# moabarar/nemar

Hardware: AMD Instinct MI355X
Metric: train images/sec (256x256 A/B pairs) (higher is better)
Workload: dtype f32

## Files before the change

### include/nemar_hip.h

```cpp
#ifndef NEMAR_HIP_H
#define NEMAR_HIP_H
#include <stddef.h>

#ifdef __cplusplus
extern "C" {
#endif

#define NEMAR_OK 0
#define NEMAR_EINVAL (-1)
#define NEMAR_ELAUNCH (-2)
#define NEMAR_EWORKSPACE (-3)

int nemar_version(void);
const char* nemar_last_error(void);

#define NEMAR_GRID_EXPLICIT 0
#define NEMAR_GRID_UNET 1
#define NEMAR_GRID_AFFINE 2
int nemar_grid_sample_fwd(const float* in, const float* grid_src, int grid_mode, float* out,
                          int N, int C, int H, int W, int Ho, int Wo, void* stream);
size_t nemar_grid_sample_bwd_workspace(int N, int C, int H, int W);
size_t nemar_grid_sample_bwd_zeroed_bytes(int N, int C, int H, int W);
int nemar_grid_sample_bwd(const float* in, const float* grid_src, int grid_mode, const float* gout,
                          float* gin, int accum_gin, float* ggrid, int accum_ggrid,
                          int N, int C, int H, int W, int Ho, int Wo, void* workspace, size_t ws_bytes, void* stream);

size_t nemar_smoothness_workspace(int N, int H, int W);
int nemar_smoothness_fwd(const float* d, const float* img, int Ci, float alpha, float factor,
                         float* loss, int accumulate, void* workspace, size_t ws_bytes,
                         int N, int H, int W, void* stream);
int nemar_smoothness_bwd(const float* d, const float* img, int Ci, float alpha, const float* gscale,
                         float factor, float* gd, int accumulate, int N, int H, int W, void* stream);

#define NEMAR_PAD_ZERO 0
#define NEMAR_PAD_REFLECT 1
#define NEMAR_ACT_NONE 0
#define NEMAR_ACT_RELU 1
#define NEMAR_ACT_LRELU 2
#define NEMAR_ACT_TANH 3
size_t nemar_conv2d_fwd_workspace(int N, int H, int W, int K, int C, int R, int S, int stride, int pad);
int nemar_conv2d_fwd(const float* x0, int C0, const float* x1, int C1, const float* w, const float* bias,
                     float* y, int N, int H, int W, int K, int R, int S, int stride, int pad, int pad_mode,
                     int act, float slope, void* workspace, size_t ws_bytes, int prepacked, void* stream);
size_t nemar_conv2d_bwd_data_workspace(int N, int C, int H, int W, int K, int R, int S, int stride, int pad,
                                       int pad_mode);
int nemar_conv2d_bwd_data(const float* gy, const float* w, const float* bias, int act, float slope,
                          float* gx0, int C0, float* gx1, int C1, int N, int H, int W, int K, int OH, int OW,
                          int R, int S, int stride, int pad, int pad_mode, void* workspace, size_t ws_bytes,
                          int prepacked, void* stream);
size_t nemar_conv2d_bwd_weight_workspace(int N, int C, int H, int W, int K, int OH, int OW, int R, int S, int stride,
                                         int pad);
int nemar_conv2d_bwd_weight(const float* x0, int C0, const float* x1, int C1, const float* gy, float* gw, float* gb,
                            int N, int H, int W, int K, int OH, int OW, int R, int S, int stride, int pad,
                            int pad_mode, void* workspace, size_t ws_bytes, void* stream);
typedef struct nemar_conv_extras {
    void* scratch;
    size_t scratch_bytes;
    const void* src_max_words;
    int src_max_count;
    const void* src2_max_words;
    int src2_max_count;
    const void* src_planes;
    void* gy_planes_out;
    size_t gy_planes_bytes;
    const void* src2_planes;
    const float* addend;
    void* out_max_words;
    const float* bias_partials;
} nemar_conv_extras;
int nemar_conv2d_bwd_data_fusable(int N, int C, int H, int W, int K, int R, int S, int stride, int pad, int pad_mode);
int nemar_conv2d_bwd_data_addend_ok(int N, int C, int H, int W, int K, int R, int S, int stride, int pad, int pad_mode);
size_t nemar_conv2d_x_planes_bytes(int N, int C, int H, int W, int KS);
size_t nemar_conv2d_gy_planes_bytes(int N, int C, int H, int W, int K, int R, int S, int stride, int pad, int pad_mode);
int nemar_last_gy_planes(void);
int nemar_conv2d_fwd_ex(const float* x0, int C0, const float* x1, int C1, const float* w, const float* bias, float* y, int N,
                        int H, int W, int K, int R, int S, int stride, int pad, int pad_mode, int act, float slope,
                        void* workspace, size_t ws_bytes, int prepacked, void* stream, const nemar_conv_extras* extras);
int nemar_conv2d_bwd_data_ex(const float* gy, const float* w, const float* bias, int act, float slope, float* gx0, int C0,
                             float* gx1, int C1, int N, int H, int W, int K, int OH, int OW, int R, int S, int stride, int pad,
                             int pad_mode, void* workspace, size_t ws_bytes, int prepacked, void* stream,
                             const nemar_conv_extras* extras);
int nemar_conv2d_bwd_weight_ex(const float* x0, int C0, const float* x1, int C1, const float* gy, float* gw, float* gb, int N,
                               int H, int W, int K, int OH, int OW, int R, int S, int stride, int pad, int pad_mode,
                               void* workspace, size_t ws_bytes, void* stream, const nemar_conv_extras* extras);
int nemar_pack_plan_record(int plan);
int nemar_pack_plan_jobs(int plan);
size_t nemar_pack_plan_bytes(int plan);
int nemar_pack_plan_dirty(int plan);
int nemar_pack_plan_commit(int plan, void* device_buffer, size_t bytes, void* stream);
int nemar_pack_plan_run(int plan, void* stream);
int nemar_pack_plan_reset(int plan);
int nemar_last_route(void);
int nemar_config_epoch(void);
int nemar_set_max_words_lazy(int on);
int nemar_max_words_finalize(void* max_words, int samples, void* stream);
size_t nemar_conv2d_scratch(int N, int H, int W, int K, int C, int R, int S, int stride, int pad);
int nemar_absmax(const float* t, long long n, void* out_word, void* stream);
int nemar_absmax_samples(const float* t, int samples, long long per_sample, void* out_words, void* stream);
int nemar_kernel_timer(int enable);
int nemar_kernel_timer_read(double* total_ms, double* total_flop, int* launches);
size_t nemar_bias_grad_workspace(int N, int C, int HW);
int nemar_bias_grad(const float* g, float* gb, int N, int C, int HW, void* workspace, size_t ws_bytes, void* stream);

int nemar_instnorm_fwd(const float* x, const float* residual, float* y, float* stats, int planes, int HW,
                       float eps, int act, float slope, void* stream);
int nemar_instnorm_bwd(const float* x, const float* stats, const float* gy, float* gx, int planes, int HW,
                       int act, float slope, void* stream);
#define NEMAR_MAX_PARTIALS 2048
#define NEMAR_MAX_WORDS(samples) ((size_t)(samples) * (1 + NEMAR_MAX_PARTIALS))
int nemar_instnorm_fwd_max(const float* x, const float* residual, float* y, float* stats, int planes, int HW,
                           float eps, int act, float slope, void* max_words, int planes_per_sample, void* stream);
int nemar_instnorm_bwd_max(const float* x, const float* stats, const float* gy, float* gx, int planes, int HW,
                           int act, float slope, void* max_words, int planes_per_sample, void* stream);

int nemar_instnorm_fwd_planes(const float* x, const float* residual, const void* residual_max_words, float* y, float* stats,
                              int N, int C, int H, int W, float eps, int act, float slope, float dropout_p,
                              unsigned long long seed, unsigned offset, void* planes, void* scale_words, void* max_words,
                              void* wgrad_planes, void* stream);
int nemar_instnorm_bwd_planes(const float* x, const float* stats, const float* gy, const void* gy_max_words, int N, int C,
                              int H, int W, int act, float slope, float dropout_p, unsigned long long seed, unsigned offset,
                              int pad_mode, float* gx, void* dgrad_planes, void* wgrad_planes, void* scale_words,
                              float* bias_partials, void* stream);
int nemar_bias_from_partials(const float* bias_partials, int N, int C, float* gb, void* stream);
size_t nemar_batchnorm_workspace(int N, int C, int HW, int segments);
int nemar_batchnorm_fwd_train(const float* x, const float* residual, float* y, const float* weight, const float* bias,
                              float* running_mean, float* running_var, long long* num_batches_tracked, float* saved,
                              int N, int C, int HW, int segments, float eps, float momentum, int act, float slope,
                              float dropout_p, unsigned long long seed, unsigned offset, void* max_words,
                              void* workspace, size_t workspace_bytes, void* stream);
int nemar_batchnorm_fwd_eval(const float* x, const float* residual, float* y, const float* weight, const float* bias,
                             const float* running_mean, const float* running_var, float* saved, int N, int C, int HW, float eps,
                             int act, float slope, float dropout_p, unsigned long long seed, unsigned offset, void* max_words,
                             void* stream);
int nemar_batchnorm_bwd(const float* x, const float* gy, float* gx, const float* weight, const float* bias, const float* saved,
                        float* grad_weight, float* grad_bias, int N, int C, int HW, int segments, int training, int act,
                        float slope, float dropout_p, unsigned long long seed, unsigned offset, void* workspace,
                        size_t workspace_bytes, void* stream);

int nemar_act_bwd(const float* gy, const float* y, float* gx, long long n, int act, float slope, void* stream);
int nemar_act_fwd(const float* x, float* y, long long n, int act, float slope, void* stream);
int nemar_concat_pieces(const float* const* pieces, const long long* counts, int k, float* dst, void* stream);
int nemar_add2(const float* a, const float* b, float* out, long long n, void* stream);
int nemar_maxpool2_fwd(const float* x, float* y, int planes, int H, int W, void* stream);
int nemar_maxpool2_bwd(const float* x, const float* gy, const float* addend, float* gx, int planes, int H, int W,
                       void* stream);
int nemar_bilinear_fwd(const float* x, float* y, int planes, int H, int W, int Ho, int Wo, void* stream);
int nemar_bilinear_bwd(const float* gy, float* gx, int planes, int H, int W, int Ho, int Wo, void* stream);
int nemar_dropout(const float* x, float* y, long long n, float p, unsigned long long seed, unsigned offset,
                  void* stream);
int nemar_dropout_max(const float* x, float* y, int samples, long long per_sample, float p, unsigned long long seed,
                      unsigned offset, void* max_words, void* stream);

int nemar_set_dropout_base(const void* device_word);
int nemar_store_words(void* dst, const void* host_words, int n, void* stream);
int nemar_adam_step_dev(float* p, const float* g, float* m, float* v, long long n, const float* hyper, double beta1,
                        double beta2, double eps, void* stream);

int nemar_crop_flip_normalize(const float* pool, const int* params, float* y, int M, int B, int C, int H, int W,
                              int Hc, int Wc, float scale, void* stream);

int nemar_deform_field(const float* params, float* g, int B, int Hc, int Wc, int gh, int gw, void* stream);
int nemar_crop_flip_deform_normalize(const float* pool, const int* params, const float* g, float* y, int M, int B, int C,
                                     int H, int W, int Hc, int Wc, float scale, void* stream);
size_t nemar_registration_error_workspace(int N, int H, int W);
int nemar_registration_error(const float* pred, int grid_mode, const float* g, float* out, void* workspace, size_t ws_bytes,
                             int N, int H, int W, void* stream);

#define NEMAR_SAMPLE_BILINEAR 0
#define NEMAR_SAMPLE_NEAREST 1
int nemar_warp_resampled_fwd(const float* in, const float* pred, int grid_mode, int sample_mode, float* out,
                             int N, int C, int Hs, int Ws, int hf, int wf, int Ho, int Wo, void* stream);

int nemar_label_overlap(const float* labels_moving, const float* labels_fixed, const float* pred, int grid_mode, unsigned* counts,
                        int N, int K, int Hs, int Ws, int hf, int wf, int Ho, int Wo, void* stream);
int nemar_map_points(const float* pts, const float* pred, int grid_mode, float* out, int N, int P, int Hs, int Ws, int hf, int wf,
                     int Ho, int Wo, void* stream);

int nemar_compose_pred(const float* first, int first_mode, int h1, int w1, const float* second, int second_mode, int h2, int w2,
                       float* out_field, const float* img, float* out_img, int C, int N, int H, int W, void* stream);

#define NEMAR_GAN_VANILLA 0
#define NEMAR_GAN_LSGAN 1
#define NEMAR_GAN_WGANGP 2
size_t nemar_loss_workspace(void);
int nemar_l1_loss_fwd(const float* a, const float* b, long long n, float weight, float* loss, int accumulate,
                      void* workspace, size_t ws_bytes, void* stream);
int nemar_l1_loss_bwd(const float* a, const float* b, long long n, const float* gscale, float weight, float* ga,
                      int accumulate, void* stream);
int nemar_gan_loss_fwd(const float* x, long long n, int mode, int target_is_real, float weight, float* loss,
                       int accumulate, void* workspace, size_t ws_bytes, void* stream);
int nemar_gan_loss_bwd(const float* x, long long n, int mode, int target_is_real, const float* gscale,
                       float weight, float* gx, void* stream);

int nemar_adam_step(float* p, const float* g, float* m, float* v, long long n, double lr, double beta1,
                    double beta2, double eps, int step, void* stream);

#ifdef __cplusplus
}
#endif
#endif
```

### nemar_amd/_lib.py

```python
import ctypes as C
import os

import torch

_HERE = os.path.dirname(os.path.abspath(__file__))
PRODUCT_PATH = os.path.join(_HERE, "lib", "libnemar_hip.so")
AB_PATH = os.path.join(_HERE, "lib", "libnemar_hip_ab.so")
DEFAULT_PATH = AB_PATH if (os.environ.get("NEMAR_AB_LIBRARY") == "1" or os.environ.get("NEMAR_TUNE")) else PRODUCT_PATH

_f = C.POINTER(C.c_float)
_vp = C.c_void_p
_i = C.c_int
_fl = C.c_float
_sz = C.c_size_t
_ll = C.c_longlong
_db = C.c_double
_u64 = C.c_ulonglong
_u32 = C.c_uint

SIGNATURES = {
    "nemar_version": (_i, []),
    "nemar_last_error": (C.c_char_p, []),
    "nemar_grid_sample_fwd": (_i, [_vp, _vp, _i, _vp, _i, _i, _i, _i, _i, _i, _vp]),
    "nemar_grid_sample_bwd_workspace": (_sz, [_i, _i, _i, _i]),
    "nemar_grid_sample_bwd_zeroed_bytes": (_sz, [_i, _i, _i, _i]),
    "nemar_grid_sample_bwd": (_i, [_vp, _vp, _i, _vp, _vp, _i, _vp, _i, _i, _i, _i, _i, _i, _i, _vp, _sz, _vp]),
    "nemar_smoothness_workspace": (_sz, [_i, _i, _i]),
    "nemar_smoothness_fwd": (_i, [_vp, _vp, _i, _fl, _fl, _vp, _i, _vp, _sz, _i, _i, _i, _vp]),
    "nemar_smoothness_bwd": (_i, [_vp, _vp, _i, _fl, _vp, _fl, _vp, _i, _i, _i, _i, _vp]),
    "nemar_conv2d_fwd_workspace": (_sz, [_i] * 9),
    "nemar_conv2d_fwd": (_i, [_vp, _i, _vp, _i, _vp, _vp, _vp, _i, _i, _i, _i, _i, _i, _i, _i, _i, _i, _fl, _vp, _sz, _i, _vp]),
    "nemar_conv2d_bwd_data_workspace": (_sz, [_i] * 10),
    "nemar_conv2d_bwd_data": (_i, [_vp, _vp, _vp, _i, _fl, _vp, _i, _vp, _i, _i, _i, _i, _i, _i, _i, _i, _i, _i, _i,
                                   _i, _vp, _sz, _i, _vp]),
    "nemar_conv2d_bwd_weight_workspace": (_sz, [_i] * 11),
    "nemar_conv2d_bwd_weight": (_i, [_vp, _i, _vp, _i, _vp, _vp, _vp, _i, _i, _i, _i, _i, _i, _i, _i, _i, _i, _i, _vp, _sz,
                                     _vp]),
    "nemar_conv2d_scratch": (_sz, [_i] * 9),
    "nemar_conv2d_gy_planes_bytes": (_sz, [_i] * 10),
    "nemar_absmax": (_i, [_vp, _ll, _vp, _vp]),
    "nemar_absmax_samples": (_i, [_vp, _i, _ll, _vp, _vp]),
    "nemar_kernel_timer": (_i, [_i]),
    "nemar_kernel_timer_read": (_i, [C.POINTER(C.c_double), C.POINTER(C.c_double), C.POINTER(_i)]),
    "nemar_bias_grad_workspace": (_sz, [_i, _i, _i]),
    "nemar_bias_grad": (_i, [_vp, _vp, _i, _i, _i, _vp, _sz, _vp]),
    "nemar_last_route": (_i, []),
    "nemar_last_gy_planes": (_i, []),
    "nemar_config_epoch": (_i, []),
    "nemar_set_max_words_lazy": (_i, [_i]),
    "nemar_instnorm_fwd": (_i, [_vp, _vp, _vp, _vp, _i, _i, _fl, _i, _fl, _vp]),
    "nemar_instnorm_bwd": (_i, [_vp, _vp, _vp, _vp, _i, _i, _i, _fl, _vp]),
    "nemar_instnorm_fwd_max": (_i, [_vp, _vp, _vp, _vp, _i, _i, _fl, _i, _fl, _vp, _i, _vp]),
    "nemar_instnorm_fwd_planes": (_i, [_vp, _vp, _vp, _vp, _vp, _i, _i, _i, _i, _fl, _i, _fl, _fl, _u64, _u32, _vp, _vp, _vp, _vp, _vp]),
    "nemar_instnorm_bwd_planes": (_i, [_vp, _vp, _vp, _vp, _i, _i, _i, _i, _i, _fl, _fl, _u64, _u32, _i, _vp, _vp, _vp, _vp, _vp, _vp]),
    "nemar_bias_from_partials": (_i, [_vp, _i, _i, _vp, _vp]),
    "nemar_conv2d_bwd_data_fusable": (_i, [_i] * 10),
    "nemar_conv2d_x_planes_bytes": (_sz, [_i] * 5),
    "nemar_set_dropout_base": (_i, [_vp]),
    "nemar_store_words": (_i, [_vp, _vp, _i, _vp]),
    "nemar_pack_plan_record": (_i, [_i]),
    "nemar_pack_plan_jobs": (_i, [_i]),
    "nemar_pack_plan_bytes": (_sz, [_i]),
    "nemar_pack_plan_dirty": (_i, [_i]),
    "nemar_pack_plan_commit": (_i, [_i, _vp, _sz, _vp]),
    "nemar_pack_plan_run": (_i, [_i, _vp]),
    "nemar_pack_plan_reset": (_i, [_i]),
    "nemar_adam_step_dev": (_i, [_vp, _vp, _vp, _vp, _ll, _vp, C.c_double, C.c_double, C.c_double, _vp]),
    "nemar_conv2d_fwd_ex": (_i, [_vp, _i, _vp, _i, _vp, _vp, _vp, _i, _i, _i, _i, _i, _i, _i, _i, _i, _i, _fl, _vp, _sz, _i, _vp, _vp]),
    "nemar_conv2d_bwd_data_ex": (_i, [_vp, _vp, _vp, _i, _fl, _vp, _i, _vp, _i, _i, _i, _i, _i, _i, _i, _i, _i, _i, _i, _i, _vp, _sz, _i, _vp, _vp]),
    "nemar_conv2d_bwd_weight_ex": (_i, [_vp, _i, _vp, _i, _vp, _vp, _vp, _i, _i, _i, _i, _i, _i, _i, _i, _i, _i, _i, _vp, _sz, _vp, _vp]),
    "nemar_instnorm_bwd_max": (_i, [_vp, _vp, _vp, _vp, _i, _i, _i, _fl, _vp, _i, _vp]),
    "nemar_act_bwd": (_i, [_vp, _vp, _vp, _ll, _i, _fl, _vp]),
    "nemar_act_fwd": (_i, [_vp, _vp, _ll, _i, _fl, _vp]),
    "nemar_conv2d_bwd_data_addend_ok": (_i, [_i] * 10),
    "nemar_max_words_finalize": (_i, [_vp, _i, _vp]),
    "nemar_concat_pieces": (_i, [_vp, _vp, _i, _vp, _vp]),
    "nemar_add2": (_i, [_vp, _vp, _vp, _ll, _vp]),
    "nemar_maxpool2_fwd": (_i, [_vp, _vp, _i, _i, _i, _vp]),
    "nemar_maxpool2_bwd": (_i, [_vp, _vp, _vp, _vp, _i, _i, _i, _vp]),
    "nemar_bilinear_fwd": (_i, [_vp, _vp, _i, _i, _i, _i, _i, _vp]),
    "nemar_bilinear_bwd": (_i, [_vp, _vp, _i, _i, _i, _i, _i, _vp]),
    "nemar_crop_flip_normalize": (_i, [_vp, _vp, _vp, _i, _i, _i, _i, _i, _i, _i, _fl, _vp]),
    "nemar_deform_field": (_i, [_vp, _vp, _i, _i, _i, _i, _i, _vp]),
    "nemar_crop_flip_deform_normalize": (_i, [_vp, _vp, _vp, _vp, _i, _i, _i, _i, _i, _i, _i, _fl, _vp]),
    "nemar_registration_error_workspace": (_sz, [_i, _i, _i]),
    "nemar_registration_error": (_i, [_vp, _i, _vp, _vp, _vp, _sz, _i, _i, _i, _vp]),
    "nemar_warp_resampled_fwd": (_i, [_vp, _vp, _i, _i, _vp, _i, _i, _i, _i, _i, _i, _i, _i, _vp]),
    "nemar_label_overlap": (_i, [_vp, _vp, _vp, _i, _vp, _i, _i, _i, _i, _i, _i, _i, _i, _vp]),
    "nemar_map_points": (_i, [_vp, _vp, _i, _vp, _i, _i, _i, _i, _i, _i, _i, _i, _vp]),
    "nemar_compose_pred": (_i, [_vp, _i, _i, _i, _vp, _i, _i, _i, _vp, _vp, _vp, _i, _i, _i, _i, _vp]),
    "nemar_dropout": (_i, [_vp, _vp, _ll, _fl, _u64, _u32, _vp]),
    "nemar_dropout_max": (_i, [_vp, _vp, _i, _ll, _fl, _u64, _u32, _vp, _vp]),
    "nemar_loss_workspace": (_sz, []),
    "nemar_l1_loss_fwd": (_i, [_vp, _vp, _ll, _fl, _vp, _i, _vp, _sz, _vp]),
    "nemar_l1_loss_bwd": (_i, [_vp, _vp, _ll, _vp, _fl, _vp, _i, _vp]),
    "nemar_gan_loss_fwd": (_i, [_vp, _ll, _i, _i, _fl, _vp, _i, _vp, _sz, _vp]),
    "nemar_gan_loss_bwd": (_i, [_vp, _ll, _i, _i, _vp, _fl, _vp, _vp]),
    "nemar_adam_step": (_i, [_vp, _vp, _vp, _vp, _ll, _db, _db, _db, _db, _i, _vp]),
    "nemar_batchnorm_workspace": (_sz, [_i, _i, _i, _i]),
    "nemar_batchnorm_fwd_train": (_i, [_vp, _vp, _vp, _vp, _vp, _vp, _vp, _vp, _vp, _i, _i, _i, _i, _fl, _fl, _i, _fl, _fl, _u64, _u32,
                                       _vp, _vp, _sz, _vp]),
    "nemar_batchnorm_fwd_eval": (_i, [_vp, _vp, _vp, _vp, _vp, _vp, _vp, _vp, _i, _i, _i, _fl, _i, _fl, _fl, _u64, _u32, _vp, _vp]),
    "nemar_batchnorm_bwd": (_i, [_vp, _vp, _vp, _vp, _vp, _vp, _vp, _vp, _i, _i, _i, _i, _i, _i, _fl, _fl, _u64, _u32, _vp, _sz, _vp]),
}


AB_SIGNATURES = {
    "nemar_tune": (_i, [_i, _i]),
    "nemar_grid_sample_tune": (_i, [_i]),
    "nemar_tune_ptr": (_i, [_vp]),
}


class NemarHipError(RuntimeError):
    pass


class ConvExtras(C.Structure):
    _fields_ = [("scratch", C.c_void_p), ("scratch_bytes", C.c_size_t), ("src_max_words", C.c_void_p), ("src_max_count", C.c_int),
                ("src2_max_words", C.c_void_p), ("src2_max_count", C.c_int), ("src_planes", C.c_void_p),
                ("gy_planes_out", C.c_void_p), ("gy_planes_bytes", C.c_size_t), ("src2_planes", C.c_void_p),
                ("addend", C.c_void_p), ("out_max_words", C.c_void_p), ("bias_partials", C.c_void_p)]


class Library:

    def __init__(self, path):
        if not os.path.exists(path):
            raise NemarHipError(
                "gfx950 operator library not found at %s — build it with `python -m nemar_amd.csrc.build` "
                "(there is no CPU/PyTorch fallback for the NeMAR hot path)" % path)
        self.path = path
        self._dll = C.CDLL(path)
        self._fns = {}
        for name, (res, args) in SIGNATURES.items():
            try:
                fn = getattr(self._dll, name)
            except AttributeError as e:
                raise NemarHipError("%s does not export %s" % (path, name)) from e
            fn.restype = res
            fn.argtypes = args
            self._fns[name] = fn
        self.has_switches = all(hasattr(self._dll, name) for name in AB_SIGNATURES)
        if self.has_switches:
            for name, (res, args) in AB_SIGNATURES.items():
                fn = getattr(self._dll, name)
                fn.restype = res
                fn.argtypes = args
                self._fns[name] = fn

    def raw(self, name):
        return self._fns[name]

    def last_error(self):
        return self._fns["nemar_last_error"]().decode("utf-8", "replace")

    def __getattr__(self, name):
        fns = self.__dict__.get("_fns", {})
        full = name if name.startswith("nemar_") else "nemar_" + name
        if full not in fns:
            if full in AB_SIGNATURES:
                raise NemarHipError("%s has no %s: the measurement switches exist only in the -DNEMAR_AB build "
                                    "(libnemar_hip_ab.so; set NEMAR_AB_LIBRARY=1 before nemar_amd is imported)" % (self.__dict__.get("path"), full))
            raise AttributeError(name)
        fn = fns[full]
        if {**SIGNATURES, **AB_SIGNATURES}[full][0] is not _i or full in ("nemar_version", "nemar_last_route", "nemar_last_gy_planes", "nemar_config_epoch", "nemar_set_max_words_lazy", "nemar_pack_plan_jobs", "nemar_pack_plan_dirty", "nemar_conv2d_bwd_data_fusable", "nemar_conv2d_bwd_data_addend_ok"):
            return fn

        if os.environ.get("NEMAR_DEBUG_SYNC"):
            def checked(*a):
                import sys
                sys.stderr.write("[nemar] %s %s\n" % (full, [x for x in a if isinstance(x, (int, float))]))
                sys.stderr.flush()
                rc = fn(*a)
                torch.cuda.synchronize()
                if rc != 0:
                    raise NemarHipError("%s failed (%d): %s" % (full, rc, self.last_error()))
                return rc
            checked.__name__ = full
            self.__dict__[name] = checked
            return checked

        def checked(*a):
            rc = fn(*a)
            if rc != 0:
                raise NemarHipError("%s failed (%d): %s" % (full, rc, self.last_error()))
            return rc

        checked.__name__ = full
        self.__dict__[name] = checked
        return checked


_default = None


def load(path=None):
    global _default
    if path is not None:
        return Library(path)
    if _default is None:
        _default = Library(DEFAULT_PATH)
        for kv in os.environ.get("NEMAR_TUNE", "").split(","):
            if "=" in kv:
                k, v = kv.split("=")
                _default.tune(int(k), int(v))
    return _default
```

### nemar_amd/csrc/common.h

```cpp
#pragma once
#include <hip/hip_runtime.h>
#include <stdint.h>
#include <stdio.h>

#define NEMAR_OK 0
#define NEMAR_EINVAL (-1)
#define NEMAR_ELAUNCH (-2)
#define NEMAR_EWORKSPACE (-3)

#define NEMAR_API extern "C" __attribute__((visibility("default")))

#ifdef NEMAR_AB
#define NEMAR_SWITCH(type, name, def) type name = def
#define NEMAR_AB_ONLY(...) __VA_ARGS__
#else
#define NEMAR_SWITCH(type, name, def) __attribute__((unused)) constexpr type name = def
#define NEMAR_AB_ONLY(...)
#endif

size_t nemar_lds_bytes(const void* kernel, size_t need, bool claim);
#define NEMAR_LDS_CLAIM_DEFAULT 1
#ifdef NEMAR_AB
extern int g_lds_claim;
#else
constexpr int g_lds_claim = NEMAR_LDS_CLAIM_DEFAULT;
#endif

struct nemar_conv_extras {
    void* scratch;
    size_t scratch_bytes;
    const void* src_max_words;
    int src_max_count;
    const void* src2_max_words;
    int src2_max_count;
    const void* src_planes;
    void* gy_planes_out;
    size_t gy_planes_bytes;
    const void* src2_planes;
    const float* addend;
    void* out_max_words;
    const float* bias_partials;
};

void nemar_set_error(const char* fmt, ...);

#define NEMAR_REQUIRE(cond, ...)                 \
    do {                                         \
        if (!(cond)) {                           \
            nemar_set_error(__VA_ARGS__);        \
            return NEMAR_EINVAL;                 \
        }                                        \
    } while (0)

#define NEMAR_CLEAR_HIP_ERROR() ((void)hipGetLastError())

#define NEMAR_CHECK_LAUNCH(what)                                              \
    do {                                                                      \
        hipError_t e__ = hipGetLastError();                                   \
        if (e__ != hipSuccess) {                                              \
            nemar_set_error("%s: %s", what, hipGetErrorString(e__));          \
            return NEMAR_ELAUNCH;                                             \
        }                                                                     \
    } while (0)

#define NEMAR_HIP_CALL(expr)                                                 \
    do {                                                                      \
        hipError_t e__ = (expr);                                              \
        if (e__ != hipSuccess) {                                              \
            nemar_set_error("%s: %s", #expr, hipGetErrorString(e__));         \
            return NEMAR_ELAUNCH;                                             \
        }                                                                     \
    } while (0)

static inline int nemar_cdiv(long long a, long long b) { return (int)((a + b - 1) / b); }

static inline int nemar_stream_grid(long long work_items, int per_block) {
    long long b = (work_items + per_block - 1) / per_block;
    if (b < 1) b = 1;
    if (b > 256 * 8) b = 256 * 8;
    return (int)b;
}

struct FastDiv {
    unsigned d;
    unsigned long long m;
};
static inline FastDiv make_fastdiv(unsigned d) {
    FastDiv f;
    f.d = d ? d : 1;
    f.m = ((1ull << 40) + f.d - 1) / f.d;
    return f;
}
__device__ __forceinline__ unsigned fd_div(unsigned n, const FastDiv& f) {
    return (unsigned)(((unsigned long long)n * f.m) >> 40);
}

__device__ __forceinline__ void glds_b128(const float* g, float* lds) {
    __builtin_amdgcn_global_load_lds((const __attribute__((address_space(1))) void*)g,
                                     (__attribute__((address_space(3))) void*)lds, 16, 0, 0);
}
__device__ __forceinline__ void glds_b32(const float* g, float* lds) {
    __builtin_amdgcn_global_load_lds((const __attribute__((address_space(1))) void*)g,
                                     (__attribute__((address_space(3))) void*)lds, 4, 0, 0);
}
__device__ __forceinline__ void wait_vmem() { __builtin_amdgcn_s_waitcnt(0x0F70); }

__device__ __forceinline__ float uniform_f(float v) {
#ifdef NEMAR_HOST_EMULATION
    return v;
#else
    return __builtin_bit_cast(float, __builtin_amdgcn_readfirstlane(__builtin_bit_cast(int, v)));
#endif
}

__device__ __forceinline__ float wave_sum(float v) {
#pragma unroll
    for (int o = 32; o > 0; o >>= 1) v += __shfl_xor(v, o, 64);
    return v;
}
__device__ __forceinline__ float wave_max(float v) {
#pragma unroll
    for (int o = 32; o > 0; o >>= 1) v = fmaxf(v, __shfl_xor(v, o, 64));
    return v;
}
// ... 12 lines not shown
```

### nemar_amd/csrc/conv.hip

```cpp
#define NEMAR_CONV_HIP
#include "common.h"
#include "conv_exact.h"
#include "conv_call.h"
#include "conv_route.h"
#include "pack_plan.h"

#ifdef NEMAR_AB
extern int g_split16_ring3;
extern int g_split16_ksplit_cap;
extern int g_narrow_fwd4;
extern int g_wg_xreg;
extern int g_register_vec4;
extern int g_overlap_per_lane;
void nemar_norm_planes_debug(int bits);
#endif

int nemar_narrow_fwd(const float* x, const float* w, const float* bias, float* y, int N, int C, int H, int W, int K, int R,
                     int pad, int border, int act, float slope, float* part, size_t part_floats, hipStream_t st);
int nemar_narrow_wgrad(const float* x, const float* gy, float* gw, int N, int C, int H, int W, int K, int R, int pad,
                       int border, float* part, hipStream_t st);
void nemar_wgrad2_launch(const float* x0, int C0, const float* x1, int C1, const float* gy, float* gw, float* gb, int N,
                         int H, int W, int K, int OH, int OW, int R, int S, int stride, int pad, int pad_mode,
                         int target_blocks, bool vec_ok, int dbg, float* part, hipStream_t st);
void nemar_sum_partials_pair(const float* part_a, long long stride_a, int splits_a, float* dst_a, long long n_a,
// ... 414 lines not shown
            v = at(y, x);
        } else {
            const int y0 = y + 3, x0 = x + 3;
            const int y1 = (y >= 1 && y <= 3) ? 3 - y : -1, y2 = (y <= H - 2 && y >= H - 4) ? 2 * (H - 1) - y + 3 : -1;
            const int x1 = (x >= 1 && x <= 3) ? 3 - x : -1, x2 = (x <= W - 2 && x >= W - 4) ? 2 * (W - 1) - x + 3 : -1;
            auto row = [&](int Y) {
                float s = at(Y, x0);
                if (x1 >= 0) s += at(Y, x1);
                if (x2 >= 0) s += at(Y, x2);
                return s;
            };
            v = row(y0);
            if (y1 >= 0) v += row(y1);
            if (y2 >= 0) v += row(y2);
        }
        if (bias) v += bias[k];
        out[idx] = apply_act(v, act, slope);
    }
}

void k7_mf_run(const K7MfPlan& m_, const float* src, const float* w, int Ks, int Cb, int dgrad, const float* bias, float* out, int N, int H, int W,
               int fold, int act, float slope, float* wsf, int prepacked, hipStream_t st) {
    K7MfPlan m = m_;
    float* wt = wsf + m.wt_off;
    void* packed = wsf + m.pack_off;
    float* P = wsf + m.p_off;
    if (!prepacked) {
        K7MfWtArgs a{w, wt, Ks, Cb, dgrad, nemar_stream_grid(32 * Cb * 7, 256), 1};
        if (nemar_pack_recording()) nemar_pack_record_job(PACK_FAM_PRE, &a, a.gx, 1);
        hipLaunchKernelGGL(k7_mf_weights_kernel, dim3(a.gx), dim3(256), 0, st, w, wt, Ks, Cb, dgrad);
        nemar_s16g_pack(m.q, m.pl, wt, (long long)Cb * 7, 7, packed, st);
    }
    m.q.src0 = src; m.q.src1 = nullptr; m.q.dst0 = P; m.q.dst1 = nullptr; m.q.bias = nullptr; m.q.dbg = 0; m.q.tl = nullptr;
    nemar_s16g_conv(m.q, m.pl, packed, st);
    const long long total = (long long)N * Ks * H * W;
    hipLaunchKernelGGL(k7_mf_sum_kernel, dim3(nemar_stream_grid(total, 256)), dim3(256), 0, st, (const float*)P, bias, out, Ks, H, W, m.PH, m.PW, fold,
                       act, slope, total);
}

__global__ __launch_bounds__(256) void pad_planes_kernel(const float* __restrict__ src, float* __restrict__ dst, int plane,
                                                         int plane_padded, long long total) {
    for (long long idx = (long long)blockIdx.x * blockDim.x + threadIdx.x; idx < total;
         idx += (long long)gridDim.x * blockDim.x) {
        const long long pl = idx / plane_padded;
        const int r = (int)(idx - pl * plane_padded);
        dst[idx] = r < plane ? src[pl * plane + r] : 0.f;
    }
}

}

static ConvFacts facts_of(const ConvCall& call, const float* bias, int act, float slope) {
    ConvFacts f;
    f.bias = bias != nullptr; f.act = act; f.slope = slope; f.scratch_bytes = call.scratch ? call.scratch_bytes : 0;
    return f;
}

NEMAR_API size_t nemar_conv2d_fwd_workspace(int N, int H, int W, int K, int C, int R, int S, int stride, int pad) {
    if (N <= 0 || H <= 0 || W <= 0 || K <= 0 || C <= 0 || R <= 0 || S <= 0 || stride < 1) return 0;
    return sizeof(float) * plan_fwd({N, C, 0, H, W, K, R, S, stride, pad, BORDER_ZERO}, ConvFacts::canonical()).total;
}

static int conv2d_fwd(ConvCall& call, const float* x0, int C0, const float* x1, int C1, const float* w, const float* bias,
                      float* y, int N, int H, int W, int K, int R, int S, int stride, int pad, int pad_mode,
                      int act, float slope, void* workspace, size_t ws_bytes, int prepacked, void* stream) {
    NEMAR_CLEAR_HIP_ERROR();
    NEMAR_REQUIRE(x0 && w && y && workspace, "conv2d_fwd: null pointer");
    NEMAR_REQUIRE(C0 > 0 && C1 >= 0 && (C1 == 0 || x1), "conv2d_fwd: bad channel split %d+%d", C0, C1);
    NEMAR_REQUIRE(N > 0 && H > 0 && W > 0 && K > 0 && R > 0 && S > 0 && R * S <= MAX_TAPS, "conv2d_fwd: bad shape");
    NEMAR_REQUIRE(stride >= 1 && pad >= 0 && pad < 32768, "conv2d_fwd: bad stride/pad");
    NEMAR_REQUIRE(pad_mode == BORDER_ZERO || (pad_mode == BORDER_REFLECT && pad < H && pad < W),
                  "conv2d_fwd: reflect pad %d needs pad < H,W (%d,%d)", pad, H, W);
    const int C = C0 + C1;
    const int OH = (H + 2 * pad - R) / stride + 1, OW = (W + 2 * pad - S) / stride + 1;
    NEMAR_REQUIRE(OH > 0 && OW > 0, "conv2d_fwd: empty output");
    NEMAR_REQUIRE((long long)N * OH * OW < (1ll << 31) && (long long)C * H * W < (1ll << 31) && (long long)C * R * S < (1 << 20),
                  "conv2d_fwd: problem too large for 32-bit tile indexing");
    ConvFacts f = facts_of(call, bias, act, slope);
    FwdPlan P = plan_fwd({N, C0, C1, H, W, K, R, S, stride, pad, pad_mode}, f);
    if (ws_bytes < sizeof(float) * P.total) {
        nemar_set_error("conv2d_fwd: workspace %zu < %zu", ws_bytes, sizeof(float) * P.total);
        return NEMAR_EWORKSPACE;
    }
    hipStream_t st = (hipStream_t)stream;
    const char* what = "conv2d_fwd";
    g_last_route = P.route;
    switch (P.route) {
    case ROUTE_K7:
        if (P.sub == FwdPlan::K7_MANY_FEW) {
            k7_mf_run(P.k7, x0, w, K, C, 0, bias, y, N, H, W, 0, act, slope, (float*)workspace, prepacked, st);
            what = "conv2d_fwd (7x7 many -> few, 16-bit pipe)";
        } else {
            if (!prepacked) nemar_k7_fm_pack(w, (long long)C * 49, 49, 0, K, C, workspace, st);
            nemar_k7_fm_conv(x0, C, H, W, 3, pad_mode == BORDER_REFLECT, workspace, bias, y, K, N, H, W, act, slope, 0, st);
            what = "conv2d_fwd (7x7, 16-bit pipe)";
        }
        break;
    case ROUTE_NARROW:
        nemar_narrow_fwd(x0, w, bias, y, N, C, H, W, K, R, pad, pad_mode, act, slope,
                         g_deterministic ? (float*)workspace : nullptr, ws_bytes / sizeof(float), st);
        what = "conv2d_fwd (narrow)";
        break;
    case ROUTE_SPLIT16: {
        const int mode = pad_mode == BORDER_REFLECT ? SPLIT16_REFLECT : SPLIT16_ZERO;
        if (!prepacked) nemar_split16_pack(w, workspace, K, C, R, 0, g_split16_variant, st);
        nemar_split16_conv(x0, workspace, bias, y, N, H, W, K, C, R, 1, H, W, OH, OW, mode, call.scratch, g_xcd_map, g_split16_variant,
                           g_tl, nullptr, call.src_max, call.src_planes, call.src_planes_kind, nullptr, nullptr, st);
        what = "conv2d_fwd (split-16)";
        break;
    }
    case ROUTE_S16G: {
        S16gProblem& q = P.q;
        q.src0 = x0; q.src1 = x1; q.dst0 = y; q.dst1 = nullptr; q.bias = bias; q.dbg = g_dbg; q.tl = g_tl;
        if (!prepacked) nemar_s16g_pack(q, P.pl, w, (long long)C * R * S, (long long)R * S, workspace, st);
        nemar_s16g_conv(q, P.pl, workspace, st);
        what = "conv2d_fwd (16-bit pipe, in-kernel split)";
        break;
    }
    default: {
        IgemmParams p;
        fwd_taps(p.taps, R, S, pad);
        if (!prepacked) launch_pack(w, (float*)workspace, K, C, C * R * S, R * S, p.taps, st);
        p.src0 = x0; p.src1 = x1; p.C0 = C0; p.C1 = C1; p.Hs = H; p.Ws = W;
        p.wp = (const float*)workspace; p.M = K; p.Mpad = igemm_mpad(K); p.Kred = C * R * S;
        p.zero = p.wp + packed_core_floats(K, C * R * S);
        p.dbg = g_dbg; p.tl = g_tl;
        p.ring_p = 0; p.ring_H = 0; p.ring_W = 0; p.ksplit = 1; p.part = nullptr; p.part_stride = 0;
        p.rf = 0; p.rf_row = nullptr; p.rf_col = nullptr; p.xcd = 0;
        p.bias = bias;
        p.dst0 = y; p.dst1 = nullptr; p.M0 = K;
        p.OH = OH; p.OW = OW; p.OHf = OH; p.OWf = OW; p.osy = 1; p.ooy = 0; p.osx = 1; p.oox = 0;
        p.N = N; p.P = N * OH * OW;
        p.sy = stride; p.sx = stride; p.border = pad_mode; p.act = act; p.slope = slope; p.pad = pad;
        p.fd_ohw = make_fastdiv(OH * OW); p.fd_ow = make_fastdiv(OW); p.fd_cs = make_fastdiv(C);
        if (P.sub != FwdPlan::PLAIN) {
            p.ksplit = P.ksplit;
            p.part = (float*)workspace + P.slab_off;
            p.part_stride = (long long)N * K * OH * OW;
            p.act = ACT_NONE;
        }
        launch_igemm(p, st);
        if (P.sub == FwdPlan::SPLIT_ACT) nemar_sum_partials_act(p.part, p.part_stride, p.ksplit, y, p.part_stride, act == ACT_RELU ? 1 : 2, slope, st);
        else if (P.sub == FwdPlan::SPLIT) nemar_sum_partials(p.part, p.part_stride, p.ksplit, y, p.part_stride, false, st);
    }
    }
    NEMAR_CHECK_LAUNCH(what);
    return NEMAR_OK;
}

NEMAR_API size_t nemar_conv2d_bwd_data_workspace(int N, int C, int H, int W, int K, int R, int S, int stride, int pad, int pad_mode) {
    if (N <= 0 || C <= 0 || K <= 0 || R <= 0 || S <= 0 || stride < 1) return 0;
    return sizeof(float) * plan_dgrad({N, C, 0, H, W, K, R, S, stride, pad, pad_mode}, ConvFacts::canonical()).total;
}

static int conv2d_bwd_data(ConvCall& call, const float* gy, const float* w, const float* bias, int act, float slope,
                           float* gx0, int C0, float* gx1, int C1, int N, int H, int W, int K, int OH, int OW,
                           int R, int S, int stride, int pad, int pad_mode, void* workspace, size_t ws_bytes,
                           int prepacked, void* stream) {
    NEMAR_CLEAR_HIP_ERROR();
    NEMAR_REQUIRE(gy && w && workspace && (gx0 || gx1), "conv2d_bwd_data: null pointer");
    NEMAR_REQUIRE(C0 >= 0 && C1 >= 0 && C0 + C1 > 0 && (C1 == 0 || gx1), "conv2d_bwd_data: bad channel split");
    NEMAR_REQUIRE(N > 0 && H > 0 && W > 0 && K > 0 && OH > 0 && OW > 0 && R * S <= MAX_TAPS && R > 0 && S > 0,
                  "conv2d_bwd_data: bad shape");
    NEMAR_REQUIRE(stride >= 1 && stride <= 4 && pad >= 0, "conv2d_bwd_data: bad stride/pad");
    NEMAR_REQUIRE((H + 2 * pad - R) / stride + 1 == OH && (W + 2 * pad - S) / stride + 1 == OW,
                  "conv2d_bwd_data: gy %dx%d inconsistent with x %dx%d k%d s%d p%d", OH, OW, H, W, R, stride, pad);
    const int C = C0 + C1;
    const bool refl = pad_mode == BORDER_REFLECT && pad > 0;
    NEMAR_REQUIRE(pad_mode != BORDER_REFLECT || (pad < H && pad < W), "conv2d_bwd_data: reflect pad too large");
    NEMAR_REQUIRE(!refl || (!bias && act == ACT_NONE && gx1 == nullptr),
                  "conv2d_bwd_data: reflect mode supports a single destination without bias/activation");
    NEMAR_REQUIRE(!refl || stride > 1 || pad <= 4, "conv2d_bwd_data: reflect pad %d > 4 unsupported", pad);
    ConvFacts f = facts_of(call, bias, act, slope);
    f.gx0 = gx0 != nullptr; f.gx1 = gx1 != nullptr;
    f.gy_planes_bytes = call.gy_planes_out ? call.gy_planes_bytes : 0;
    DgradPlan L = plan_dgrad({N, C0, C1, H, W, K, R, S, stride, pad, pad_mode}, f);
    if (ws_bytes < sizeof(float) * L.total) {
        nemar_set_error("conv2d_bwd_data: workspace %zu < %zu", ws_bytes, sizeof(float) * L.total);
        return NEMAR_EWORKSPACE;
    }
    NEMAR_REQUIRE((long long)N * (H + 2 * pad) * (W + 2 * pad) < (1ll << 31) && (long long)K * OH * OW < (1ll << 31) && (long long)K * R * S < (1 << 20),
                  "conv2d_bwd_data: problem too large for 32-bit tile indexing");
    hipStream_t st = (hipStream_t)stream;
    float* wsf = (float*)workspace;
    const long long total = (long long)N * C * H * W;
    const int mskip = L.mskip;
    const char* what = "conv2d_bwd_data";
    g_last_route = L.route;
    switch (L.sub) {
    case DgradPlan::K7_MANY_FEW:
        k7_mf_run(L.k7, gy, w, C, K, 1, nullptr, gx0, N, H, W, L.k7_fold, ACT_NONE, 0.f, wsf, prepacked, st);
        what = "conv2d_bwd_data (7x7 many -> few, 16-bit pipe)";
        break;
    case DgradPlan::K7_FEW_MANY:
        if (!prepacked) nemar_k7_fm_pack(w, 49, (long long)C * 49, 1, C, K, workspace, st);
        if (L.k7_fold == 2) {
            float* padded = wsf + ((nemar_k7_fm_pack_floats(C) + 3) & ~(size_t)3);
            nemar_k7_fm_conv(gy, K, OH, OW, 6, 0, workspace, nullptr, padded, C, N, H + 6, W + 6, ACT_NONE, 0.f, 0, st);
            fold_padded(padded, gx0, H, W, pad, total, nullptr, st);
        } else {
            nemar_k7_fm_conv(gy, K, OH, OW, L.k7_fold ? 6 : 3, 0, workspace, nullptr, gx0, C, N, H, W, ACT_NONE, 0.f, L.k7_fold, st);
        }
        what = "conv2d_bwd_data (7x7, 16-bit pipe)";
        break;
    case DgradPlan::SPLIT16: {
        if (!prepacked) nemar_split16_pack(w, workspace, K, C, R, 1, g_split16_variant, st);
        const Split16Done done = nemar_split16_conv(gy, workspace, nullptr, gx0, N, H, W, C, K, R, R - 1 - pad, OH, OW, H, W,
                                                    refl ? SPLIT16_DGRAD_REFLECT : SPLIT16_ZERO, call.scratch, g_xcd_map, g_split16_variant, g_tl,
                                                    L.want_gy_planes ? call.gy_planes_out : nullptr, call.src_max, call.src_planes,
                                                    call.src_planes_kind, call.addend, call.out_max, st);
        call.gy_planes_written = done.dual_written;
        call.epilogue_fused = done.epilogue_fused;
        what = "conv2d_bwd_data (split-16)";
        break;
    }
    case DgradPlan::S16G:
    case DgradPlan::S16G_FOLD: {
        const bool fold16 = L.sub == DgradPlan::S16G_FOLD;
        S16gProblem& q = L.q;
        q.src0 = gy; q.src1 = nullptr; q.bias = bias ? bias + mskip : nullptr;
        if (fold16) { q.dst0 = wsf + L.padded_off; q.dst1 = nullptr; q.M0 = q.M; }
        else if (mskip) { q.dst0 = gx1; q.dst1 = nullptr; q.M0 = q.M; }
        else { q.dst0 = gx0; q.dst1 = gx1; q.M0 = C0; }
        if (!prepacked) nemar_s16g_pack(q, L.pl, w + (size_t)mskip * R * S, (long long)R * S, (long long)C * R * S, workspace, st);
        nemar_s16g_conv(q, L.pl, workspace, st);
        if (fold16) fold_padded(q.dst0, gx0, H, W, pad, total, call.addend, st);
        if (fold16 && call.addend) call.addend_done = true;
        what = fold16 ? "conv2d_bwd_data (16-bit pipe on the padded domain + fold)" : "conv2d_bwd_data (16-bit pipe, in-kernel split)";
        break;
    }
    case DgradPlan::EXACT: {
    const bool ring = L.ring, fold = L.fold;
    bool folded = false;
    const int Hd = fold ? H + 2 * pad : H, Wd = fold ? W + 2 * pad : W;
    const int padd = fold ? 0 : pad;
    float* padded = fold ? wsf + L.padded_off : nullptr;
    int cls = 0;
    for (int ph = 0; ph < stride; ++ph)
        for (int pw = 0; pw < stride; ++pw, ++cls) {
            IgemmParams p;
            dgrad_taps(p.taps, R, S, padd, stride, ph, pw);
            const int OHc = (Hd - ph + stride - 1) / stride, OWc = (Wd - pw + stride - 1) / stride;
            if (OHc <= 0 || OWc <= 0) continue;
            const int Mc = C - mskip;
            p.src0 = gy; p.src1 = nullptr; p.C0 = K; p.C1 = 0; p.Hs = OH; p.Ws = OW;
            p.M = Mc; p.Mpad = igemm_mpad(Mc); p.Kred = p.taps.n * K;
            p.bias = bias ? bias + mskip : nullptr;
            if (fold) { p.dst0 = padded; p.dst1 = nullptr; p.M0 = Mc; }
            else if (mskip) { p.dst0 = gx1; p.dst1 = nullptr; p.M0 = Mc; }
            else { p.dst0 = gx0; p.dst1 = gx1; p.M0 = C0; }
            p.OH = OHc; p.OW = OWc; p.OHf = Hd; p.OWf = Wd; p.osy = stride; p.ooy = ph; p.osx = stride; p.oox = pw;
            p.N = N; p.P = N * OHc * OWc;
            p.sy = 1; p.sx = 1; p.border = BORDER_ZERO; p.act = act; p.slope = slope;
            p.pad = pad;
            p.ring_p = 0; p.ring_H = 0; p.ring_W = 0; p.ksplit = 1; p.part = nullptr; p.part_stride = 0;
            p.rf = 0; p.rf_row = nullptr; p.rf_col = nullptr; p.xcd = 0;
            p.fd_ohw = make_fastdiv(OHc * OWc); p.fd_ow = make_fastdiv(OWc); p.fd_cs = make_fastdiv(K);
            float* wp = wsf + L.pack_stride * (size_t)cls;
            p.wp = wp;
            p.zero = wp + packed_core_floats(Mc, K * (p.taps.n > 0 ? p.taps.n : 1));
            p.dbg = g_dbg; p.tl = nullptr;
            if (p.taps.n == 0) {
                p.taps.n = 1; p.taps.dy[0] = -32000; p.taps.dx[0] = -32000; p.taps.wofs[0] = 0; p.Kred = K;
                p.taps.dyx[0] = (int)(((unsigned)-32000 << 16) | ((unsigned)-32000 & 0xffffu));
            }
            if (!prepacked) launch_pack(w + (size_t)mskip * R * S, wp, Mc, K, R * S, C * R * S, p.taps, st);
            bool ring_done = false;
            if (L.narrow) {
                float* w2 = wsf + L.w2_off;
                if (!prepacked) {
                    if (nemar_pack_recording()) {
                        FlipTArgs a{w, w2, K, C, R, S, nemar_stream_grid((long long)K * C * R * S, 256), 1};
                        nemar_pack_record_job(PACK_FAM_FLIPT, &a, a.gx, 1);
                    }
                    hipLaunchKernelGGL(flip_transpose_kernel, dim3(nemar_stream_grid((long long)K * C * R * S, 256)),
                                       dim3(256), 0, st, w, w2, K, C, R, S);
                }
                nemar_narrow_fwd(gy, w2, nullptr, gx0, N, K, OH, OW, C, R, R - 1 - pad, BORDER_ZERO, ACT_NONE, 0.f, nullptr, 0, st);
            } else {
                if (L.split) {
                    p.ksplit = L.ksplit;
                    p.part = wsf + L.slab_off;
                    p.part_stride = (long long)N * C * Hd * Wd;
                    if (gx1) { p.M0 = C; p.dst1 = nullptr; }
                }
                bool vec = false;
                if (L.aux_rows && route_ws2(p, &vec) && vec) {
                    float* rows = wsf + L.aux_rows_off, * cols = wsf + L.aux_cols_off;
                    hipLaunchKernelGGL(reflect_aux_kernel, dim3(nemar_stream_grid(6ll * N * K * W + 8ll * N * K * H, 256)),
                                       dim3(256), 0, st, gy, rows, cols, N, K, H, W);
                    p.rf = 1; p.rf_row = rows; p.rf_col = cols;
                    ring_done = true;
                }
// ... 124 lines not shown
        p.dbg = g_dbg;
        p.pix_per_split = P.pix_per_split;
        p.part = part;
        p.partb = part ? part + P.bias_off : nullptr;
        const bool wide = K > 32;
        dim3 grid(nemar_cdiv(K, wide ? 128 : 32), nemar_cdiv(J, wide ? 128 : 256), P.splits), block(256);
        if (wide) hipLaunchKernelGGL((wgrad_kernel<2, 2, 2, 2>), grid, block, 0, st, p);
        else hipLaunchKernelGGL((wgrad_kernel<1, 4, 1, 2>), grid, block, 0, st, p);
        if (part) nemar_sum_partials_pair(part, (long long)K * J, P.splits, gw, (long long)K * J, gb ? p.partb : nullptr, K, P.splits, gb, K, true, st);
    }
    }
    NEMAR_CHECK_LAUNCH(what);
    return NEMAR_OK;
}

NEMAR_API int nemar_last_route(void) { return g_last_route; }
NEMAR_API int nemar_config_epoch(void) { return g_config_epoch; }

#ifdef NEMAR_AB
NEMAR_API int nemar_tune_ptr(void* p) { g_tl = (long long*)p; return NEMAR_OK; }

NEMAR_API int nemar_tune(int key, int value) {
    ++g_config_epoch;
    if (key == 0) { g_cfg128 = value; return NEMAR_OK; }
    if (key == 1) { g_lds_pad = value; return NEMAR_OK; }
    if (key == 2) { g_dbg = value; return NEMAR_OK; }
    if (key == 3) { g_narrow = value; return NEMAR_OK; }
    if (key == 4) { g_wgrad = value; return NEMAR_OK; }
    if (key == 6) { g_min_blocks = value > 0 ? value : 384; return NEMAR_OK; }
    if (key == 14) { g_deterministic = value != 0; return NEMAR_OK; }
    if (key == 8) { g_reflect_aux = value != 0; return NEMAR_OK; }
    if (key == 15) { g_xcd_map = value != 0; return NEMAR_OK; }
    if (key == 20) { g_split16 = value != 0; return NEMAR_OK; }
    if (key == 24) { g_s16g = value != 0; return NEMAR_OK; }
    if (key == 25) { g_s16g_min_mmac = value < 0 ? 0 : value; return NEMAR_OK; }
    if (key == 26) { g_s16g_wgrad_first = value != 0; return NEMAR_OK; }
    if (key == 27) { nemar_s16g_tune(0, value); return NEMAR_OK; }
    if (key == 29) { g_s16g_wgrad = value != 0; return NEMAR_OK; }
    if (key == 31) { nemar_norm_planes_debug(value); return NEMAR_OK; }
    if (key == 32) { g_split16_ring3 = value != 0; return NEMAR_OK; }
    if (key == 33) { g_k7 = value != 0; return NEMAR_OK; }
    if (key == 36) { g_split_act = value != 0; return NEMAR_OK; }
    if (key == 43) { g_fold_small = value != 0; return NEMAR_OK; }
    if (key == 37) { g_lds_claim = value; return NEMAR_OK; }
    if (key == 38) { g_wg_xreg = value != 0; return NEMAR_OK; }
    if (key == 39) { g_split16_ksplit_cap = value < 1 ? 1 : (value > 8 ? 8 : value); return NEMAR_OK; }
    if (key == 45) { g_overlap_per_lane = value != 0; return NEMAR_OK; }
    if (key == 44) { g_register_vec4 = value != 0; return NEMAR_OK; }
    if (key == 35) { g_dual_gy = value != 0; return NEMAR_OK; }
    if (key == 34) { nemar_split16_wgrad_tune(value); return NEMAR_OK; }
    if (key == 30) { g_s16g_fold = value != 0; return NEMAR_OK; }
    if (key == 28) { nemar_s16g_tune(1, value); return NEMAR_OK; }
    if (key == 40) { nemar_s16g_tune(2, value); return NEMAR_OK; }
    if (key == 42) { nemar_s16g_tune(4, value); return NEMAR_OK; }
    if (key == 41) { nemar_s16g_tune(3, value); return NEMAR_OK; }
    if (key == 23) { g_split16_min_mmac = value < 0 ? 0 : value; return NEMAR_OK; }
    if (key == 21) { g_split16_variant = value == 3 ? 3 : 4; return NEMAR_OK; }
    if (key == 16) { g_adir = value != 0; return NEMAR_OK; }
    if (key == 17) { g_mt8 = value; return NEMAR_OK; }
    if (key == 19) { g_narrow_fwd4 = value != 0; return NEMAR_OK; }
    if (key == 18) { g_ring = (value == 4 || value == 5) ? value : 3; return NEMAR_OK; }
    if (key == 12) { g_ksplit = value != 0; return NEMAR_OK; }
    if (key == 11) { g_nl4_scalar = value != 0; return NEMAR_OK; }
    if (key == 10) { g_deep64 = value != 0; return NEMAR_OK; }
    if (key == 7) { g_ws2_mt = (value == 1 || value == 2 || value == 4) ? value : 0; return NEMAR_OK; }
    if (key == 5) { g_wgrad_blocks = value > 0 ? value : 512; return NEMAR_OK; }
    nemar_set_error("nemar_tune: unknown key %d", key);
    return NEMAR_EINVAL;
}
#endif

static DgradPlan usual_dgrad(int N, int C, int H, int W, int K, int R, int S, int stride, int pad, int pad_mode) {
    DgradPlan P{};
    if (N <= 0 || C <= 0 || H <= 0 || W <= 0 || K <= 0 || R <= 0 || S <= 0 || stride < 1) return P;
    return plan_dgrad({N, C, 0, H, W, K, R, S, stride, pad, pad_mode}, ConvFacts::canonical());
}
static bool fusable(const DgradPlan& P) { return P.gy_planes_need != 0 && P.split16_ksplit == 1; }

NEMAR_API size_t nemar_conv2d_scratch(int N, int H, int W, int K, int C, int R, int S, int stride, int pad) {
    if (N <= 0 || H <= 0 || W <= 0 || K <= 0 || C <= 0) return 0;
    return plan_arena_bytes({N, C, 0, H, W, K, R, S, stride, pad, BORDER_ZERO});
}

NEMAR_API size_t nemar_conv2d_gy_planes_bytes(int N, int C, int H, int W, int K, int R, int S, int stride, int pad, int pad_mode) {
    return usual_dgrad(N, C, H, W, K, R, S, stride, pad, pad_mode).gy_planes_need;
}

NEMAR_API int nemar_conv2d_bwd_data_fusable(int N, int C, int H, int W, int K, int R, int S, int stride, int pad, int pad_mode) {
    return fusable(usual_dgrad(N, C, H, W, K, R, S, stride, pad, pad_mode)) ? 1 : 0;
}

NEMAR_API int nemar_conv2d_bwd_data_addend_ok(int N, int C, int H, int W, int K, int R, int S, int stride, int pad, int pad_mode) {
    const DgradPlan P = usual_dgrad(N, C, H, W, K, R, S, stride, pad, pad_mode);
    if (fusable(P)) return 1;
    if (pad_mode != BORDER_REFLECT || pad <= 0 || stride != 1 || pad >= H || pad >= W || R != S || R == 7) return 0;
    return (P.fold16 || P.fold) && plan_arena_bytes({N, C, 0, H, W, K, R, S, stride, pad, BORDER_ZERO}) == 0 ? 1 : 0;
}

NEMAR_API int nemar_last_gy_planes(void) { return g_last_gy_planes; }

namespace {
ConvCall call_from(const nemar_conv_extras* ex) {
    ConvCall call;
    if (!ex) return call;
    if (ex->scratch && ex->scratch_bytes) { call.scratch = ex->scratch; call.scratch_bytes = ex->scratch_bytes; }
    if (ex->src_max_words && ex->src_max_count > 0) call.src_max = {(const unsigned*)ex->src_max_words, ex->src_max_count};
    return call;
}
}

NEMAR_API int nemar_conv2d_fwd(const float* x0, int C0, const float* x1, int C1, const float* w, const float* bias,
                               float* y, int N, int H, int W, int K, int R, int S, int stride, int pad, int pad_mode,
                               int act, float slope, void* workspace, size_t ws_bytes, int prepacked, void* stream) {
    ConvCall call;
    return conv2d_fwd(call, x0, C0, x1, C1, w, bias, y, N, H, W, K, R, S, stride, pad, pad_mode, act, slope, workspace, ws_bytes, prepacked, stream);
}

NEMAR_API int nemar_conv2d_fwd_ex(const float* x0, int C0, const float* x1, int C1, const float* w, const float* bias, float* y, int N,
                                  int H, int W, int K, int R, int S, int stride, int pad, int pad_mode, int act, float slope,
                                  void* workspace, size_t ws_bytes, int prepacked, void* stream, const nemar_conv_extras* extras) {
    ConvCall call = call_from(extras);
    if (extras) { call.src_planes = extras->src_planes; call.src_planes_kind = SPLIT16_REFLECT; }
    return conv2d_fwd(call, x0, C0, x1, C1, w, bias, y, N, H, W, K, R, S, stride, pad, pad_mode, act, slope, workspace, ws_bytes, prepacked, stream);
}

NEMAR_API int nemar_conv2d_bwd_data(const float* gy, const float* w, const float* bias, int act, float slope,
                                    float* gx0, int C0, float* gx1, int C1, int N, int H, int W, int K, int OH, int OW,
                                    int R, int S, int stride, int pad, int pad_mode, void* workspace, size_t ws_bytes,
                                    int prepacked, void* stream) {
    ConvCall call;
    return conv2d_bwd_data(call, gy, w, bias, act, slope, gx0, C0, gx1, C1, N, H, W, K, OH, OW, R, S, stride, pad, pad_mode, workspace, ws_bytes,
                           prepacked, stream);
}

NEMAR_API int nemar_conv2d_bwd_data_ex(const float* gy, const float* w, const float* bias, int act, float slope, float* gx0, int C0,
                                       float* gx1, int C1, int N, int H, int W, int K, int OH, int OW, int R, int S, int stride, int pad,
                                       int pad_mode, void* workspace, size_t ws_bytes, int prepacked, void* stream,
                                       const nemar_conv_extras* extras) {
    ConvCall call = call_from(extras);
    if (extras) {
        call.src_planes = extras->src_planes;
        call.src_planes_kind = pad_mode == BORDER_REFLECT ? SPLIT16_DGRAD_REFLECT : SPLIT16_ZERO;
        call.gy_planes_out = extras->gy_planes_out; call.gy_planes_bytes = extras->gy_planes_bytes;
        call.addend = extras->addend; call.out_max = extras->out_max_words;
    }
    const int rc = conv2d_bwd_data(call, gy, w, bias, act, slope, gx0, C0, gx1, C1, N, H, W, K, OH, OW, R, S, stride, pad, pad_mode, workspace,
                                   ws_bytes, prepacked, stream);
    g_last_gy_planes = call.gy_planes_written ? 1 : 0;
    if (rc == NEMAR_OK && ((call.addend && !call.epilogue_fused && !call.addend_done) || (call.out_max && !call.epilogue_fused))) {
        nemar_set_error("conv2d_bwd_data_ex: this layer's route has no fused epilogue (addend / out_max_words): ask nemar_conv2d_bwd_data_fusable / "
                        "nemar_conv2d_bwd_data_addend_ok first");
        return NEMAR_EINVAL;
    }
    return rc;
}

NEMAR_API int nemar_conv2d_bwd_weight(const float* x0, int C0, const float* x1, int C1, const float* gy, float* gw,
                                      float* gb, int N, int H, int W, int K, int OH, int OW, int R, int S, int stride,
                                      int pad, int pad_mode, void* workspace, size_t ws_bytes, void* stream) {
    ConvCall call;
    return conv2d_bwd_weight(call, x0, C0, x1, C1, gy, gw, gb, N, H, W, K, OH, OW, R, S, stride, pad, pad_mode, workspace, ws_bytes, stream);
}

NEMAR_API int nemar_conv2d_bwd_weight_ex(const float* x0, int C0, const float* x1, int C1, const float* gy, float* gw, float* gb, int N,
                                         int H, int W, int K, int OH, int OW, int R, int S, int stride, int pad, int pad_mode,
                                         void* workspace, size_t ws_bytes, void* stream, const nemar_conv_extras* extras) {
    ConvCall call = call_from(extras);
    if (extras) {
        if (extras->src2_max_words && extras->src2_max_count > 0) call.src2_max = {(const unsigned*)extras->src2_max_words, extras->src2_max_count};
        call.x_planes = extras->src_planes;
        call.src2_planes = extras->src2_planes;
        call.bias_partials = extras->bias_partials;
    }
    const int rc = conv2d_bwd_weight(call, x0, C0, x1, C1, gy, gw, gb, N, H, W, K, OH, OW, R, S, stride, pad, pad_mode, workspace, ws_bytes, stream);
    if (rc == NEMAR_OK && call.bias_partials && gb && !call.bias_rode) {
        nemar_set_error("conv2d_bwd_weight_ex: bias_partials are only taken on the wide route (nemar_conv2d_bwd_data_fusable); gb was reduced from gy");
        return NEMAR_EINVAL;
    }
    return rc;
}

NEMAR_API int nemar_absmax(const float* t, long long n, void* out_word, void* stream) {
    NEMAR_CLEAR_HIP_ERROR();
    NEMAR_REQUIRE(t && out_word && n > 0, "absmax: null pointer");
    nemar_split16_absmax(t, 1, n, out_word, (hipStream_t)stream);
    NEMAR_CHECK_LAUNCH("absmax");
    return NEMAR_OK;
}

NEMAR_API int nemar_absmax_samples(const float* t, int samples, long long per_sample, void* out_words, void* stream) {
    NEMAR_CLEAR_HIP_ERROR();
    NEMAR_REQUIRE(t && out_words && samples > 0 && samples <= 65535 && per_sample > 0, "absmax_samples: bad arguments");
    nemar_split16_absmax(t, samples, per_sample, out_words, (hipStream_t)stream);
    NEMAR_CHECK_LAUNCH("absmax_samples");
    return NEMAR_OK;
}

NEMAR_API int nemar_kernel_timer(int enable) {
    nemar_split16_timer(enable);
    return NEMAR_OK;
}

NEMAR_API int nemar_kernel_timer_read(double* total_ms, double* total_flop, int* launches) {
    NEMAR_REQUIRE(total_ms && total_flop && launches, "kernel_timer_read: null pointer");
    *launches = nemar_split16_timer_read(total_ms, total_flop);
// ... 21 lines not shown
```

### nemar_amd/csrc/conv_call.h

```cpp
#pragma once
#include <stddef.h>

struct MaxWords {
    const unsigned* words = nullptr;
    int count = 0;
};

struct ConvCall {
    void* scratch = nullptr;
    size_t scratch_bytes = 0;
    MaxWords src_max;
    MaxWords src2_max;
    const void* src_planes = nullptr;
    int src_planes_kind = -1;
    const void* x_planes = nullptr;
    void* gy_planes_out = nullptr;
    size_t gy_planes_bytes = 0;
    const void* src2_planes = nullptr;
    const float* addend = nullptr;
    void* out_max = nullptr;
    const float* bias_partials = nullptr;
    bool gy_planes_written = false;
    bool epilogue_fused = false;
    bool addend_done = false;
    bool bias_rode = false;
};
```

### nemar_amd/csrc/conv_route.h

```cpp
#pragma once
#ifndef NEMAR_CONV_HIP
#error "conv_route.h holds conv.hip's own switches: include it from conv.hip only"
#endif
#include "common.h"
#include "conv_exact.h"
#include "conv_split16.h"
#include "conv_s16g.h"
#include "conv_k7.h"

bool nemar_narrow_eligible(int K, int C1, int R, int S, int stride, int N, int OH, int OW);
int nemar_narrow_wgrad_splits(int N, int C, int OH, int OW);
bool nemar_wgrad2_eligible(int K, int OH, int OW, bool gy_aligned16);
void nemar_wgrad2_plan(int K, int J, int P, int target_blocks, int* splits_out, int* pix_per_split_out);

using namespace nemar_exact;

namespace {

static NEMAR_SWITCH(int, g_split16, 1);
static NEMAR_SWITCH(long long, g_split16_min_mmac, 2000);
static NEMAR_SWITCH(int, g_split16_variant, 4);
static NEMAR_SWITCH(int, g_k7, 1);
static NEMAR_SWITCH(int, g_s16g, 1);
static NEMAR_SWITCH(long long, g_s16g_min_mmac, 30);
// ... 94 lines not shown
void s16g_set_class(S16gProblem& q, int c, const TapTable& t, int OHc, int OWc, int ooy, int oox) {
    q.ntaps[c] = t.n;
    for (int i = 0; i < t.n && i < S16G_MAX_TAPS; ++i) { q.dy[c][i] = t.dy[i]; q.dx[c][i] = t.dx[i]; q.wofs[c][i] = t.wofs[i]; }
    q.OH[c] = OHc; q.OW[c] = OWc; q.ooy[c] = ooy; q.oox[c] = oox;
}
bool s16g_worth_it(long long macs) { return g_s16g && macs >= g_s16g_min_mmac * 1000000ll; }

bool s16g_fwd_problem(S16gProblem& q, S16gPlan& pl, int N, int C0, int C1, int H, int W, int K, int R, int S, int stride, int pad,
                      int pad_mode, int act, float slope) {
    const int C = C0 + C1;
    if (R * S > S16G_MAX_TAPS || stride > 2 || stride < 1) return false;
    const int OH = (H + 2 * pad - R) / stride + 1, OW = (W + 2 * pad - S) / stride + 1;
    if (OH <= 0 || OW <= 0 || !s16g_worth_it((long long)N * OH * OW * K * C * R * S)) return false;
    q = S16gProblem();
    q.C0 = C0; q.C1 = C1; q.Hs = H; q.Ws = W; q.N = N; q.M = K; q.M0 = K;
    q.act = act; q.slope = slope; q.border = pad_mode; q.sstride = stride;
    q.OHf = OH; q.OWf = OW; q.osy = 1; q.osx = 1; q.ncls = 1;
    TapTable t;
    fwd_taps(t, R, S, pad);
    s16g_set_class(q, 0, t, OH, OW, 0, 0);
    pl = nemar_s16g_plan(q);
    return pl.ok != 0;
}

bool s16g_dgrad_problem(S16gProblem& q, S16gPlan& pl, int N, int C, int mskip, int H, int W, int K, int OH, int OW, int R, int S,
                        int stride, int pad, int act, float slope) {
    if (R * S > S16G_MAX_TAPS || stride > 2 || stride < 1) return false;
    if (!s16g_worth_it((long long)N * OH * OW * K * (C - mskip) * R * S)) return false;
    q = S16gProblem();
    q.C0 = K; q.C1 = 0; q.Hs = OH; q.Ws = OW; q.N = N; q.M = C - mskip;
    q.act = act; q.slope = slope; q.border = BORDER_ZERO; q.sstride = 1;
    q.OHf = H; q.OWf = W; q.osy = stride; q.osx = stride; q.ncls = 0;
    for (int ph = 0; ph < stride; ++ph)
        for (int pw = 0; pw < stride; ++pw) {
            TapTable t;
            dgrad_taps(t, R, S, pad, stride, ph, pw);
            const int OHc = (H - ph + stride - 1) / stride, OWc = (W - pw + stride - 1) / stride;
            if (t.n == 0 || OHc <= 0 || OWc <= 0 || t.n > (stride > 1 ? S16G_CLS_TAPS : S16G_MAX_TAPS)) return false;
            s16g_set_class(q, q.ncls++, t, OHc, OWc, ph, pw);
        }
    pl = nemar_s16g_plan(q);
    return pl.ok != 0;
}

struct K7MfPlan {
    S16gProblem q;
    S16gPlan pl;
    size_t wt_off, pack_off, p_off, total;
    int PH, PW;
    bool ok;
};
K7MfPlan k7_mf_plan(int N, int Cb, int Hs, int Ws, int spad, int border) {
    K7MfPlan m;
    m.ok = false;
    m.PH = Hs + 2 * spad - 6;
    m.PW = Ws + 2 * spad;
    S16gProblem& q = m.q;
    q = S16gProblem();
    q.C0 = Cb; q.C1 = 0; q.Hs = Hs; q.Ws = Ws; q.N = N; q.M = 32; q.M0 = 32;
    q.act = ACT_NONE; q.slope = 0.f; q.border = border; q.sstride = 1;
    q.OHf = m.PH; q.OWf = m.PW; q.osy = 1; q.osx = 1; q.ncls = 1;
    TapTable t;
    t.n = 7;
    for (int i = 0; i < 7; ++i) { t.dy[i] = (short)(i - spad); t.dx[i] = (short)(-spad); t.dyx[i] = ((i - spad) << 16) | ((-spad) & 0xffff); t.wofs[i] = i; }
    s16g_set_class(q, 0, t, m.PH, m.PW, 0, 0);
    m.pl = nemar_s16g_plan(q);
    if (!m.pl.ok) return m;
    m.wt_off = 0;
    m.pack_off = ((size_t)32 * Cb * 7 + 3) & ~(size_t)3;
    m.p_off = (m.pack_off + (nemar_s16g_pack_bytes(q, m.pl) + 3) / 4 + 3) & ~(size_t)3;
    m.total = m.p_off + (size_t)N * 32 * m.PH * m.PW;
    m.ok = true;
    return m;
}
bool k7_mf_eligible(int Cb, int Ks, int R, int S, int stride, int pad) {
    return g_k7 && R == 7 && S == 7 && stride == 1 && pad == 3 && Ks >= 1 && Ks <= 4 && Cb >= 16 && Cb % 16 == 0;
}

struct FwdPlan {
    int route;
    enum Sub { PLAIN, K7_MANY_FEW, K7_FEW_MANY, SPLIT, SPLIT_ACT } sub;
    size_t pack, slab_off, total;
    int ksplit;
    K7MfPlan k7;
    S16gProblem q; S16gPlan pl;
};
FwdPlan plan_fwd(const ConvShape& s, const ConvFacts& f) {
    FwdPlan P;
    const int N = s.N, H = s.H, W = s.W, K = s.K, C = s.C(), R = s.R, S = s.S, stride = s.stride, pad = s.pad, OH = s.OH(), OW = s.OW();
    P.pack = packed_floats(K, C * R * S);
    if (wide_candidates(s).fwd)
        grow(P.pack, (nemar_split16_pack_bytes(K, C, R) + 3) / 4);
    if (s16g_fwd_problem(P.q, P.pl, N, C, 0, H, W, K, R, S, stride, pad, BORDER_ZERO, ACT_NONE, 0.f))
        grow(P.pack, (nemar_s16g_pack_bytes(P.q, P.pl) + 3) / 4);
    const bool k7_fm = nemar_k7_fm_eligible(C, K, R, S, stride, pad);
    if (k7_fm) grow(P.pack, nemar_k7_fm_pack_floats(K));
    P.ksplit = 1;
    if (g_ksplit && OH > 0 && OW > 0 && K > 4) P.ksplit = normalize_ksplit(C * R * S, small_problem_split(K, N * OH * OW, C * R * S));
    P.slab_off = (P.pack + 3) & ~(size_t)3;
    P.total = P.slab_off + (P.ksplit > 1 ? (size_t)P.ksplit * N * K * OH * OW : 0);
    P.k7.ok = false;
    if (k7_mf_eligible(C, K, R, S, stride, pad)) {
        P.k7 = k7_mf_plan(N, C, H, W, 3, BORDER_ZERO);
        if (P.k7.ok) grow(P.total, P.k7.total);
        if (s.pad_mode != BORDER_ZERO) P.k7 = k7_mf_plan(N, C, H, W, 3, s.pad_mode);
    }
    const int mode = s.pad_mode == BORDER_REFLECT ? SPLIT16_REFLECT : SPLIT16_ZERO;
    P.sub = FwdPlan::PLAIN;
    if (s.C1 == 0 && P.k7.ok) { P.route = ROUTE_K7; P.sub = FwdPlan::K7_MANY_FEW; }
    else if (g_k7 && s.C1 == 0 && f.act != ACT_TANH && k7_fm) { P.route = ROUTE_K7; P.sub = FwdPlan::K7_FEW_MANY; }
    else if (nemar_narrow_eligible(K, s.C1, R, S, stride, N, OH, OW) && g_narrow) P.route = ROUTE_NARROW;
    else if (g_split16 && s.C1 == 0 && f.act == ACT_NONE && split16_worth_it(N, OH, OW, K, C, R, S) &&
             nemar_split16_eligible(N, H, W, K, C, R, S, stride, pad, mode, g_split16_variant) &&
             f.scratch_bytes && f.scratch_bytes >= nemar_split16_scratch_total(N, H, W, K, C, OH, OW)) P.route = ROUTE_SPLIT16;
    else if (s16g_fwd_problem(P.q, P.pl, N, s.C0, s.C1, H, W, K, R, S, stride, pad, s.pad_mode, f.act, f.slope)) P.route = ROUTE_S16G;
    else {
        const bool split_act = g_split_act && (f.act == ACT_RELU || f.act == ACT_LRELU);
        P.route = ROUTE_EXACT;
        if (P.ksplit > 1 && (f.act == ACT_NONE || split_act)) P.sub = split_act ? FwdPlan::SPLIT_ACT : FwdPlan::SPLIT;
    }
    return P;
}

struct DgradPlan {
    int route;
    enum Sub { K7_MANY_FEW, K7_FEW_MANY, SPLIT16, S16G, S16G_FOLD, EXACT } sub;
    size_t pack_stride, padded_off, w2_off, ring_off, ring_slab_off, slab_off, aux_rows_off, aux_cols_off, total;
    int ring_len, ksplit, ring_ksplit;
    bool ring, fold, fold16, fold_small;
    int k7_fold;
    bool want_gy_planes;
    size_t gy_planes_need;
    int split16_ksplit;
    int mskip;
    bool narrow;
    bool split;
    bool aux_rows;
    K7MfPlan k7;
    S16gProblem q; S16gPlan pl;
};
DgradPlan plan_dgrad(const ConvShape& s, const ConvFacts& f) {
    DgradPlan L;
    const int N = s.N, C = s.C(), H = s.H, W = s.W, K = s.K, R = s.R, S = s.S, stride = s.stride, pad = s.pad, OH = s.OH(), OW = s.OW();
    const bool refl = s.refl();
    L.ring = refl && stride == 1;
    L.fold = refl && !L.ring;
    L.pack_stride = packed_floats(C, K * R * S);
    if (wide_candidates(s).dgrad)
        grow(L.pack_stride, (nemar_split16_pack_bytes(C, K, R) + 3) / 4);
    bool s16g = false;
    L.fold16 = false;
    if (!refl && OH > 0 && OW > 0 && s16g_dgrad_problem(L.q, L.pl, N, C, 0, H, W, K, OH, OW, R, S, stride, pad, ACT_NONE, 0.f)) {
        s16g = true;
        grow(L.pack_stride, ((nemar_s16g_pack_bytes(L.q, L.pl) + 3) / 4 + stride * stride - 1) / (stride * stride));
    } else if (L.ring && g_s16g_fold && R * S <= 9 && OH > 0 && OW > 0 &&
               s16g_dgrad_problem(L.q, L.pl, N, C, 0, H + 2 * pad, W + 2 * pad, K, OH, OW, R, S, 1, 0, ACT_NONE, 0.f)) {
        L.fold16 = true;
        grow(L.pack_stride, (nemar_s16g_pack_bytes(L.q, L.pl) + 3) / 4);
    }
    L.fold_small = L.ring && !L.fold16 && g_fold_small && g_ksplit && C > 4 && (H + 2 * pad) * (W + 2 * pad) <= 1296;
    if (L.fold_small) { L.ring = false; L.fold = true; }
    size_t o = L.pack_stride * (size_t)(stride * stride);
    L.padded_off = o;
    if (L.fold || L.fold16) o += (size_t)N * C * (H + 2 * pad) * (W + 2 * pad);
    L.w2_off = o;
    if (C <= 4) o += (size_t)C * K * R * S;
    L.ring_off = o;
    L.ring_len = L.ring ? 2 * pad * (W + 2 * pad) + 2 * pad * H : 0;
    o += (size_t)N * C * L.ring_len;
    L.ring_ksplit = 1;
    L.ring_slab_off = o;
    if (L.ring) {
        const int tiles = nemar_cdiv(N * L.ring_len, 64) * nemar_cdiv(C, 64), stages = nemar_cdiv(K * R * S, BK);
        int ks = nemar_cdiv(384, tiles);
        if (ks > nemar_cdiv(stages, 8)) ks = nemar_cdiv(stages, 8);
        L.ring_ksplit = normalize_ksplit(K * R * S, ks < 1 ? 1 : ks);
        if (L.ring_ksplit > 1) o += (size_t)L.ring_ksplit * N * C * L.ring_len;
    }
    L.ksplit = 1;
    const int Hs = L.fold_small ? H + 2 * pad : H, Wsl = L.fold_small ? W + 2 * pad : W;
    if (g_ksplit && stride == 1 && (!L.fold || L.fold_small) && C > 4) {
        const int P = N * Hs * Wsl, Kred = K * R * S, stages = nemar_cdiv(Kred, BK);
        if (g_cfg128 == 0 && C > 64 && K % BK == 0) {
            const long long tiles = (long long)nemar_cdiv(C, 128) * nemar_cdiv(P, 128);
            if (tiles < 200 && stages >= 256) {
                int ks = nemar_cdiv(256, (int)tiles);
                if (ks > stages / 128) ks = stages / 128;
                if (ks > 1) L.ksplit = ks;
            }
        }
        if (L.ksplit == 1) L.ksplit = small_problem_split(C, P, Kred);
        L.ksplit = normalize_ksplit(Kred, L.ksplit);
    }
    L.slab_off = o;
    if (L.ksplit > 1) o += (size_t)L.ksplit * N * C * Hs * Wsl;
    const bool aux = L.ring && pad == 1 && R == 3 && S == 3;
    L.aux_rows_off = o;
    if (aux) o += 6ull * N * K * W;
    L.aux_cols_off = o;
    if (aux) o += 8ull * N * K * H;
    L.total = o;
    L.k7.ok = false;
    if (k7_mf_eligible(K, C, R, S, stride, pad)) {
// ... 123 lines not shown
```

### nemar_amd/csrc/conv_split16.h

```cpp
#pragma once
#include <hip/hip_runtime.h>
#include <stddef.h>
#include "conv_call.h"

enum { SPLIT16_ZERO = 0, SPLIT16_REFLECT = 1, SPLIT16_DGRAD_REFLECT = 2 };

bool nemar_split16_eligible(int N, int H, int W, int M, int Cred, int R, int S, int stride, int pad, int mode, int variant);
size_t nemar_split16_scratch_bytes(int N, int Cred, int H, int W);
int nemar_split16_ksplit(int N, int H, int W, int M, int Cred);
size_t nemar_split16_scratch_total(int N, int H, int W, int M, int Cred, int OH, int OW);
size_t nemar_split16_pack_bytes(int M, int Cred, int KS);
void nemar_split16_pack(const float* w, void* packed, int K, int C, int KS, int dgrad, int variant, hipStream_t st);
struct Split16Done {
    bool dual_written;
    bool epilogue_fused;
};
Split16Done nemar_split16_conv(const float* src, const void* packed, const float* bias, float* dst, int N, int H, int W, int M, int Cred,
                               int KS, int src_pad, int Hs, int Ws_src, int OH, int OW, int mode, void* scratch, int xcd_map, int variant,
                               long long* tl, void* dual_g_out, MaxWords src_max, const void* ready_planes, int ready_kind,
                               const float* addend, void* out_max, hipStream_t st);

bool nemar_split16_wgrad_eligible(int N, int C, int H, int W, int K, int R, int S, int stride, int pad);
size_t nemar_split16_wgrad_scratch_bytes(int N, int C, int H, int W, int K, int KS);
int nemar_split16_wgrad_splits(int N, int C, int H, int W, int K, int KS);
#ifdef NEMAR_AB
void nemar_split16_wgrad_tune(int one_copy);
#endif
void nemar_sum_partials_pair(const float* part_a, long long stride_a, int splits_a, float* dst_a, long long n_a,
                             const float* part_b, long long stride_b, int splits_b, float* dst_b, long long n_b, bool accumulate, hipStream_t st);
void nemar_split16_wgrad(const float* x, const float* gy, float* gw, int N, int C, int H, int W, int K, int KS, int reflect,
                         void* scratch, float* part, int xcd_map, const void* g_planes, const void* x_planes, MaxWords x_max,
                         MaxWords gy_max, const float* bias_partials, float* gb, hipStream_t st);
size_t nemar_split16_wgrad_g_bytes(int N, int H, int W, int K, int KS);
void nemar_split16_dual_split(const float* gy, void* dplanes, void* gplanes, int N, int K, int H, int W, int mode, const unsigned* maxbits,
                              int mstride, hipStream_t st);
void nemar_sum_partials(const float* part, long long stride, int splits, float* dst, long long n, bool accumulate, hipStream_t st);
void nemar_sum_partials_two(const float* part, long long stride, int splits, float* d0, float* d1, int N, int C0, int C1, int HW, hipStream_t st);
void nemar_sum_partials_act(const float* part, long long stride, int splits, float* dst, long long n, int act, float slope, hipStream_t st);

void nemar_split16_absmax(const float* x, int samples, long long per, void* out, hipStream_t st);
const unsigned* nemar_split16_source_max(const float* src, int N, long long per, MaxWords hint, unsigned* own, int* stride, hipStream_t st);

void nemar_split16_timer(int on);
int nemar_split16_timer_read(double* total_ms, double* total_flop);
```

### nemar_amd/csrc/conv_split16.hip

```cpp
#include "common.h"
#include "conv_split16.h"
#include "pack_plan.h"
#include "max_words.h"

namespace {

typedef float f32x16 __attribute__((ext_vector_type(16)));
typedef __bf16 bf16x8 __attribute__((ext_vector_type(8)));
typedef unsigned u32x4 __attribute__((ext_vector_type(4)));
typedef unsigned short u16x8 __attribute__((ext_vector_type(8)));

__device__ __forceinline__ unsigned short bf16_rn(float v) {
    const __bf16 h = (__bf16)v;
    return __builtin_bit_cast(unsigned short, h);
}
__device__ __forceinline__ float bf16_val(unsigned short b) { return __builtin_bit_cast(float, (unsigned)b << 16); }

__device__ __forceinline__ void split3(float v, unsigned short& b0, unsigned short& b1, unsigned short& b2) {
    b0 = bf16_rn(v);
    const float r1 = v - bf16_val(b0);
    b1 = bf16_rn(r1);
    const float r2 = r1 - bf16_val(b1);
    b2 = bf16_rn(r2);
}
// ... 126 lines not shown
        const int tap = (int)(q % NT), chunk = (int)(q / NT);
        const int mg = mblk * 128 + m;
        unsigned short b0[8], b1[8], b2[8];
#pragma unroll
        for (int j = 0; j < 8; ++j) {
            const int cr = chunk * 16 + kg * 8 + j;
            const float v = dgrad ? w[((size_t)cr * M + mg) * NT + (NT - 1 - tap)] : w[((size_t)mg * Cred + cr) * NT + tap];
            if (NPL == 3) split3(v, b0[j], b1[j], b2[j]);
            else split2_f16(v * scale, b0[j], b1[j]);
        }
        u32x4* o = out + (((size_t)(chunk * NT + tap) * mblks + mblk) * NPL) * 256 + kg * 128 + m;
        o[0] = pack8(b0);
        o[256] = pack8(b1);
        if (NPL == 3) o[512] = pack8(b2);
    }
}

struct Split16PackArgs {
    const float* w; u32x4* out;
    int M, Cred, dgrad, NT;
    const unsigned* parts; unsigned* maxword;
    int gx, gy;
};
__device__ __forceinline__ void split16_pack_body(const Split16PackArgs& a, int bx, int, int gx) {
    unsigned mb = 0;
#pragma unroll
    for (int i = 0; i < NEMAR_PACK_MAX_PARTS; ++i) mb = max(mb, a.parts[i]);
    if (bx == 0 && threadIdx.x == 0) *a.maxword = mb;
    const int mblks = a.M >> 7, NT = a.NT, M = a.M, Cred = a.Cred;
    const long long total = (long long)(Cred >> 4) * NT * mblks * 256;
    const float scale = pow2_scale(mb);
    for (long long t = (long long)bx * 256 + threadIdx.x; t < total; t += (long long)gx * 256) {
        const int m = (int)(t & 127), kg = (int)((t >> 7) & 1);
        long long q = t >> 8;
        const int mblk = (int)(q % mblks);
        q /= mblks;
        const int tap = (int)(q % NT), chunk = (int)(q / NT);
        const int mg = mblk * 128 + m;
        unsigned short b0[8], b1[8];
#pragma unroll
        for (int j = 0; j < 8; ++j) {
            const int cr = chunk * 16 + kg * 8 + j;
            const float v = a.dgrad ? a.w[((size_t)cr * M + mg) * NT + (NT - 1 - tap)] : a.w[((size_t)mg * Cred + cr) * NT + tap];
            split2_f16(v * scale, b0[j], b1[j]);
        }
        u32x4* o = a.out + (((size_t)(chunk * NT + tap) * mblks + mblk) * 2) * 256 + kg * 128 + m;
        o[0] = pack8(b0);
        o[256] = pack8(b1);
    }
}
NEMAR_PACK_MULTI(split16_pack_multi_kernel, Split16PackArgs, split16_pack_body, 256)
void split16_pack_multi(const void* jobs, int njobs, int gx, int gy, hipStream_t st) {
    hipLaunchKernelGGL(split16_pack_multi_kernel, dim3(gx, gy, njobs), dim3(256), 0, st, (const Split16PackArgs*)jobs);
}
struct RegSplit16Pack {
    RegSplit16Pack() { nemar_pack_register(PACK_FAM_SPLIT16, sizeof(Split16PackArgs), split16_pack_multi); }
} g_reg_split16_pack;

struct Split16Params {
    const u32x4* planes;
    const u32x4* wp;
    const float* bias;
    int bias_al;
    float* dst;
    int N, H, W, M, Cred;
    int Ws, HpWs;
    int wshift, RT;
    int tiles_per_img, mblks;
    int halo_instr, aux_instr;
    int halo16, aux16;
    int fold;
    int xcd;
    long long plane16;
    int ksplit;
    long long slab_stride;
    int OH, OW;
    const unsigned* xmax;
    const unsigned* wmax;
    int xstride;
    long long* tl;
    const float* addend;
    unsigned* maxw;
    int maxw_lazy;
};

__device__ __forceinline__ void glds16(const u32x4* g, u32x4* lds) {
    __builtin_amdgcn_global_load_lds((const __attribute__((address_space(1))) void*)g,
                                     (__attribute__((address_space(3))) void*)lds, 16, 0, 0);
}

__device__ __forceinline__ void glds16u(const u32x4* ubase, unsigned lane_bytes, u32x4* lds) {
    glds16(reinterpret_cast<const u32x4*>(reinterpret_cast<const char*>(ubase) + lane_bytes), lds);
}

template <int NBW, int NPL, int KS = 3, int RING = 4, int EPI = 0>
__global__ __launch_bounds__(256) void igemm_split16_kernel(Split16Params p) {
    constexpr int NT = KS * KS;
    constexpr int ASTAGE16 = 256 * NPL, KB = (NT - 3) * NBW, NREG = 2 * NPL, NP = NPL == 3 ? 6 : 3, NMFMA = 8 * NP;
    constexpr int ACOPY = NPL;
    static_assert(RING == 4 || (RING == 3 && NT % 3 == 0), "ring slot of a tap must be a compile-time constant");
#define S16_SLOTOF(stage_, tap_) (RING == 4 ? ((stage_) & 3) : ((tap_) % 3))
#ifdef NEMAR_HOST_EMULATION
    __shared__ __attribute__((aligned(16))) u32x4 smem[9728];
#else
    extern __shared__ __attribute__((aligned(16))) u32x4 smem[];
#endif
    u32x4* const As = smem;
    u32x4* const Bs = smem + RING * ASTAGE16;
    const int region16 = p.halo16 + p.aux16, bbuf16 = NREG * region16;

    const int tid = threadIdx.x, wid = __builtin_amdgcn_readfirstlane(tid >> 6), lane = tid & 63;
    int t = blockIdx.x;
    if (p.xcd) t = (t & 7) * ((int)gridDim.x >> 3) + (t >> 3);
    const int zsplit = t % p.ksplit;
    t /= p.ksplit;
    const int ptile = t / p.mblks, mblk = t - ptile * p.mblks;
    const int n = ptile / p.tiles_per_img, y0 = (ptile - n * p.tiles_per_img) * p.RT;
    const int nchunks = (p.Cred >> 4) / p.ksplit, nstage = nchunks * NT;
    const int chunk0 = zsplit * nchunks;
    const int CG = p.Cred >> 3;

    const int hi = (p.halo16 + 63) >> 6, ai = (p.aux16 + 63) >> 6, ipr = hi + ai, ncopies = NREG * ipr;
    const size_t wstage = (size_t)p.mblks * ASTAGE16;
    const u32x4* const wsrc0 = p.wp + (size_t)mblk * ASTAGE16 + wid * (64 * ACOPY) + (size_t)chunk0 * NT * wstage;
    const u32x4* const bsrc0 = p.planes + ((size_t)n * CG + 2 * chunk0) * p.HpWs;
    const int halo_off = y0 * p.Ws, aux_off = (p.H + 2) * p.Ws;
    unsigned goff[KB], blds[KB];
    int blim[KB];
    int share = 0;
    {
        int breg = 0, bin = wid;
        while (bin >= ipr) { bin -= ipr; ++breg; }
        unsigned g = 0, l = 0;
        int lim = 0;
#pragma unroll
        for (int k = 0; k < KB; ++k) {
            if (wid + 4 * k < ncopies) {
                const bool aux = bin >= hi;
                const int j = aux ? bin - hi : bin;
                const int pl = breg >> 1, kg = breg & 1;
                g = (unsigned)((size_t)pl * p.plane16 + (size_t)kg * p.HpWs + (aux ? aux_off : halo_off) + j * 64);
                l = (unsigned)(breg * region16 + (aux ? p.halo16 : 0) + j * 64);
                lim = (aux ? p.aux16 : p.halo16) - j * 64;
                share = k + 1;
                bin += 4;
                while (bin >= ipr) { bin -= ipr; ++breg; }
            }
            goff[k] = g + lane;
            blds[k] = l;
            blim[k] = lim;
        }
    }
#define S16_COPIES(stage_, ti_, ci_)                                                                                   \
    {                                                                                                                   \
        const int st_ = min((stage_), nstage - 1);                      \
        const u32x4* const a_ = wsrc0 + (size_t)st_ * wstage + lane;                                                    \
        u32x4* const ad_ = As + S16_SLOTOF(stage_, ti_) * ASTAGE16 + wid * (64 * ACOPY);                                \
        _Pragma("unroll") for (int q = 0; q < ACOPY; ++q) glds16(a_ + 64 * q, ad_ + 64 * q);                            \
        if ((ti_) >= 3) {                                                                                               \
            const int hc_ = min((ci_) + 1, nchunks - 1);                  \
            const u32x4* const bb_ = bsrc0 + (size_t)(2 * hc_) * p.HpWs;                                                \
            u32x4* const bd_ = Bs + (((ci_) + 1) & 1) * bbuf16;                                                         \
            _Pragma("unroll") for (int q = 0; q < NBW; ++q) {                                                           \
                const int k_ = ((ti_) - 3) * NBW + q;                                                                   \
                if (lane < blim[k_]) glds16(bb_ + goff[k_], bd_ + blds[k_]);                                            \
            }                                                                                                           \
        }                                                                                                               \
// ... 97 lines not shown
                    else                                                                                                \
                        acc[mt_][nt_] = __builtin_amdgcn_mfma_f32_32x32x16_f16(__builtin_bit_cast(f16x8, af[cur][mt_][PA[q_]]), \
                                                                               __builtin_bit_cast(f16x8, bf[cur][nt_][PB[q_]]), \
                                                                               acc[mt_][nt_], 0, 0, 0);                 \
                }                                                                                                       \
                __builtin_amdgcn_sched_barrier(0);
                constexpr int NSLOT = 1 + 6 * NPL + ACOPY + NBW;
#define S16_SLOT(i_) S16_MFMAS((i_) * NMFMA / NSLOT, ((i_) + 1) * NMFMA / NSLOT)
                int baddr[2];
#pragma unroll
                for (int nt = 0; nt < 2; ++nt) {
                    int ra_ = (row[nt] + nr + z) * p.Ws;
                    if (KS == 3 && nr == 2) ra_ = top[nt] ? auxoff : ra_;
                    if (KS == 3 && nr == 0) ra_ = bot[nt] ? auxoff + p.Ws : ra_;
                    int sl_ = col[nt] + nsx;
                    if (KS == 3 && nsx == 2) sl_ = lft[nt] ? p.W + 2 : sl_;
                    if (KS == 3 && nsx == 0) sl_ = rgt[nt] ? p.W + 3 : sl_;
                    baddr[nt] = ra_ + sl_;
                }
                const u32x4* const Bn_ = Bs + nhb * bbuf16 + lhi * region16;
                const u32x4* const An_ = As + S16_SLOTOF(T + 1, tap + 1) * ASTAGE16 + lhi * 128 + l31;
                S16_SLOT(0)
#pragma unroll
                for (int i = 0; i < 2 * NPL; ++i) {
                    bf[nxt][i / NPL][i % NPL] = Bn_[(i % NPL) * 2 * region16 + baddr[i / NPL]];
                    S16_SLOT(1 + i)
                }
#pragma unroll
                for (int i = 0; i < 4 * NPL; ++i) {
                    af[nxt][i / NPL][i % NPL] = An_[(i % NPL) * 256 + (i / NPL) * 32];
                    S16_SLOT(1 + 2 * NPL + i)
                }
                {
                    const int st_ = min(T + RING, nstage - 1);
                    const u32x4* const a_ = wsrc0 + (size_t)st_ * wstage + lane;
                    u32x4* const ad_ = As + S16_SLOTOF(T, tap) * ASTAGE16 + wid * (64 * ACOPY);
#pragma unroll
                    for (int q = 0; q < ACOPY; ++q) {
                        glds16(a_ + 64 * q, ad_ + 64 * q);
                        S16_SLOT(1 + 6 * NPL + q)
                    }
                    if (iti >= 3) {
                        const int hc_ = min(ici + 1, nchunks - 1);
                        const u32x4* const bb_ = bsrc0 + (size_t)(2 * hc_) * p.HpWs;
                        u32x4* const bd_ = Bs + ((ici + 1) & 1) * bbuf16;
#pragma unroll
                        for (int q = 0; q < NBW; ++q) {
                            const int k_ = (iti - 3) * NBW + q;
                            if (lane < blim[k_]) glds16(bb_ + goff[k_], bd_ + blds[k_]);
                            S16_SLOT(1 + 6 * NPL + ACOPY + q)
                        }
                    } else {
                        S16_MFMAS((1 + 6 * NPL + ACOPY) * NMFMA / NSLOT, NMFMA)
                    }
                }
#undef S16_SLOT
#undef S16_MFMAS
                const int t3 = tap + 3 >= NT ? tap + 3 - NT : tap + 3;
                const int nfl = RING == 4 ? S16_COUNT(t3) + S16_COUNT(iti) : S16_COUNT(iti);
                S16_STAMP(1)
                if (nfl == ACOPY) S16_VMCNT(ACOPY)
                else if (nfl == ACOPY + NBW) S16_VMCNT(ACOPY + NBW)
                else if (nfl == 2 * ACOPY) S16_VMCNT(2 * ACOPY)
                else if (nfl == 2 * ACOPY + NBW) S16_VMCNT(2 * ACOPY + NBW)
                else S16_VMCNT(2 * ACOPY + 2 * NBW)
                S16_STAMP(2)
                __builtin_amdgcn_s_waitcnt(0xC07F);
                S16_STAMP(3)
                __builtin_amdgcn_s_barrier();
                S16_STAMP(4)
#undef S16_STAMP
            }
        }
    }
    wait_vmem();
#undef S16_READ
#undef S16_VMCNT
#undef S16_COUNT
#undef S16_COPIES
#undef S16_SLOTOF

    const size_t HW = (size_t)p.OH * p.OW;
    const float unscale = NPL == 2 ? 1.f / (pow2_scale(p.xmax[n * p.xstride]) * pow2_scale(*p.wmax)) : 1.f;
    if (!EPI) {
        const bool with_bias = p.bias != nullptr && zsplit == 0;
        float* d0[2];
        bool ok[2];
#pragma unroll
        for (int nt = 0; nt < 2; ++nt) {
            ok[nt] = KS == 3 || (y0 + row[nt] < p.OH && col[nt] < p.OW);
            d0[nt] = p.dst + (size_t)zsplit * p.slab_stride + (size_t)n * p.M * HW + (size_t)(y0 + row[nt]) * p.OW + col[nt] +
                     (size_t)(mblk * 128 + 4 * lhi) * HW;
        }
#pragma unroll
        for (int mt = 0; mt < 4; ++mt) {
            float bv[16];
#pragma unroll
            for (int q = 0; q < 4; ++q) {
                float4 b4 = make_float4(0.f, 0.f, 0.f, 0.f);
                if (with_bias) {
                    const float* const bp = p.bias + mblk * 128 + 4 * lhi + mt * 32 + 8 * q;
                    b4 = p.bias_al ? *reinterpret_cast<const float4*>(bp) : make_float4(bp[0], bp[1], bp[2], bp[3]);
                }
                bv[4 * q] = b4.x; bv[4 * q + 1] = b4.y; bv[4 * q + 2] = b4.z; bv[4 * q + 3] = b4.w;
            }
#pragma unroll
            for (int r = 0; r < 16; ++r) {
#pragma unroll
                for (int nt = 0; nt < 2; ++nt) {
                    float v = acc[mt][nt][r];
                    if (NPL == 2) v *= unscale;
                    v += bv[r];
                    if (ok[nt]) d0[nt][(size_t)(mt * 32 + (r & 3) + 8 * (r >> 2)) * HW] = v;
                }
            }
            __builtin_amdgcn_sched_barrier(0);
        }
        return;
    }
    unsigned omax = 0;
    size_t o0[2];
#pragma unroll
    for (int nt = 0; nt < 2; ++nt)
        o0[nt] = (size_t)n * p.M * HW + (size_t)(y0 + row[nt]) * p.OW + col[nt] + (size_t)(mblk * 128 + 4 * lhi) * HW;
#pragma unroll
    for (int mt = 0; mt < 4; ++mt) {
        float ad[2][16];
        if (EPI == 2) {
#pragma unroll
            for (int r = 0; r < 16; ++r)
#pragma unroll
                for (int nt = 0; nt < 2; ++nt) ad[nt][r] = p.addend[o0[nt] + (size_t)(mt * 32 + (r & 3) + 8 * (r >> 2)) * HW];
            __builtin_amdgcn_sched_barrier(0);
        }
#pragma unroll
        for (int r = 0; r < 16; ++r)
#pragma unroll
            for (int nt = 0; nt < 2; ++nt) {
                float v = acc[mt][nt][r] * unscale;
                if (EPI == 2) v += ad[nt][r];
                p.dst[o0[nt] + (size_t)(mt * 32 + (r & 3) + 8 * (r >> 2)) * HW] = v;
                omax = max(omax, finite_bits(__builtin_bit_cast(unsigned, v)));
            }
        __builtin_amdgcn_sched_barrier(0);
    }
    if (p.maxw) {
        __shared__ unsigned mred[4];
#pragma unroll
        for (int o = 32; o > 0; o >>= 1) omax = max(omax, (unsigned)__shfl_xor((int)omax, o, 64));
        if (lane == 0) mred[wid] = omax;
        __syncthreads();
        if (tid == 0) {
            const int parts = p.tiles_per_img * p.mblks;
            p.maxw[p.N + (size_t)n * parts + (ptile - n * p.tiles_per_img) * p.mblks + mblk] = max(max(mred[0], mred[1]), max(mred[2], mred[3]));
            if (p.maxw_lazy && ptile == n * p.tiles_per_img && mblk == 0) p.maxw[n] = NEMAR_MAX_LAZY_MARK | (unsigned)parts;
        }
    }
}

int ilog2(int v) {
    int s = 0;
    while ((1 << s) < v) ++s;
    return s;
}

}

bool nemar_split16_eligible(int N, int H, int W, int M, int Cred, int R, int S, int stride, int pad, int mode, int variant) {
    if (R != S || (R != 3 && R != 4) || stride != 1 || pad != 1) return false;
    if (M % 128 != 0 || Cred % 16 != 0 || M <= 0 || Cred <= 0) return false;
    if (!(W == 32 || W == 64 || W == 128 || W == 256)) return false;
    const int RT = 256 / W;
    if (H % RT != 0 || H < 4) return false;
    if ((long long)N * Cred * (H + 4) * (W + 4) >= (1ll << 31) || N > 256) return false;
    if (R == 4 && (mode != SPLIT16_ZERO || variant == 0)) return false;
    if (variant == 0) return false;
    const int npl = variant == 3 ? 3 : 2;
    const int region16 = (RT + R - 1) * (W + 4) + (mode == SPLIT16_DGRAD_REFLECT ? 2 * (W + 4) : 0);
    return 2 * 2 * npl * region16 + 4 * 256 * npl <= 9728;
}

NEMAR_SWITCH(int, g_split16_ksplit_cap, 8);
int nemar_split16_ksplit(int N, int H, int W, int M, int Cred) {
    const int tiles = N * (H / (256 / W)) * (M / 128), nchunks = Cred / 16;
    int ks = 1;
    while (tiles * ks * 2 <= 256 && nchunks % (ks * 2) == 0 && nchunks / (ks * 2) >= 4 && ks < g_split16_ksplit_cap) ks *= 2;
    return ks;
}

size_t nemar_split16_scratch_total(int N, int H, int W, int M, int Cred, int OH, int OW) {
    const int ks = nemar_split16_ksplit(N, H, W, M, Cred);
    return nemar_split16_scratch_bytes(N, Cred, H, W) + (ks > 1 ? (size_t)ks * N * M * OH * OW * sizeof(float) : 0);
}

size_t nemar_split16_scratch_bytes(int N, int Cred, int H, int W) {
    return (size_t)3 * N * (Cred / 8) * (H + 4) * (W + 4) * 16 + 16384;
}

size_t nemar_split16_pack_bytes(int M, int Cred, int KS) { return (size_t)(Cred / 16) * KS * KS * (M / 128) * 768 * 16 + 16384; }

namespace {
unsigned* scratch_max_word(void* scratch, int N, int Cred, int H, int W) {
    return (unsigned*)((char*)scratch + nemar_split16_scratch_bytes(N, Cred, H, W) - 1024);
}
unsigned* pack_max_word(void* packed, int M, int Cred, int KS) {
    return (unsigned*)((char*)packed + nemar_split16_pack_bytes(M, Cred, KS) - 64);
}

}

void nemar_split16_absmax(const float* x, int samples, long long per, void* out, hipStream_t st) {
    int grid = nemar_stream_grid(per, 256 * 16);
    if (grid * samples > 2048) grid = (2048 + samples - 1) / samples;
    hipLaunchKernelGGL(absmax_kernel, dim3(grid, samples), dim3(256), 0, st, x, per, (unsigned*)out);
}

const unsigned* nemar_split16_source_max(const float* src, int N, long long per, MaxWords hint, unsigned* own, int* stride, hipStream_t st) {
    if (hint.words && (hint.count == N || hint.count == 1)) {
        *stride = hint.count == N && N > 1 ? 1 : 0;
        return hint.words;
    }
    (void)hipMemsetAsync(own, 0, sizeof(unsigned) * N, st);
    nemar_split16_absmax(src, N, per, own, st);
    *stride = N > 1 ? 1 : 0;
    return own;
}

namespace {
constexpr int MAX_TIMED = 1024;
hipEvent_t g_tev[MAX_TIMED][2];
int g_tev_made = 0, g_tev_used = 0;
double g_tev_flop = 0.0;
bool g_timing = false;
}

void nemar_split16_timer(int on) {
    g_timing = on != 0;
    if (on) { g_tev_used = 0; g_tev_flop = 0.0; }
}

int nemar_split16_timer_read(double* total_ms, double* total_flop) {
    double t = 0.0;
    for (int i = 0; i < g_tev_used; ++i) {
        float ms = 0.f;
        (void)hipEventSynchronize(g_tev[i][1]);
        (void)hipEventElapsedTime(&ms, g_tev[i][0], g_tev[i][1]);
        t += ms;
    }
    *total_ms = t;
    *total_flop = g_tev_flop;
    const int n = g_tev_used;
    g_tev_used = 0;
    g_tev_flop = 0.0;
    return n;
}

#define S16_TIMED_LAUNCH(launch_)                                              \
    {                                                                          \
        const bool tm_ = g_timing && KS == 3 && g_tev_used < MAX_TIMED;        \
        if (tm_) {                                                             \
            while (g_tev_made <= g_tev_used) {                                 \
                (void)hipEventCreate(&g_tev[g_tev_made][0]);                   \
                (void)hipEventCreate(&g_tev[g_tev_made][1]);                   \
                ++g_tev_made;                                                  \
            }                                                                  \
            (void)hipEventRecord(g_tev[g_tev_used][0], st);                    \
        }                                                                      \
        launch_;                                                               \
        if (tm_) {                                                             \
            (void)hipEventRecord(g_tev[g_tev_used++][1], st);                  \
            g_tev_flop += 2.0 * N * OH * OW * (double)M * Cred * KS * KS;      \
        }                                                                      \
    }

void nemar_split16_pack(const float* w, void* packed, int K, int C, int KS, int dgrad, int variant, hipStream_t st) {
    const int M = dgrad ? C : K, Cred = dgrad ? K : C, NT = KS * KS;
    const long long total = (long long)(Cred / 16) * NT * (M / 128) * 256;
    if (variant == 4) {
        unsigned* mw = pack_max_word(packed, M, Cred, KS);
        if (nemar_pack_recording()) {
            unsigned* parts = (unsigned*)((char*)packed + nemar_split16_pack_bytes(M, Cred, KS) - 1024);
            NemarPackMaxArgs ma{w, (long long)K * C * NT, parts, NEMAR_PACK_MAX_PARTS, 1};
            nemar_pack_record_job(PACK_FAM_MAX, &ma, ma.gx, 1);
            Split16PackArgs a{w, (u32x4*)packed, M, Cred, dgrad, NT, parts, mw, nemar_stream_grid(total, 256), 1};
            nemar_pack_record_job(PACK_FAM_SPLIT16, &a, a.gx, 1);
        }
        (void)hipMemsetAsync(mw, 0, sizeof(unsigned), st);
        nemar_split16_absmax(w, 1, (long long)K * C * NT, mw, st);
        hipLaunchKernelGGL((split16_pack_kernel<2>), dim3(nemar_stream_grid(total, 256)), dim3(256), 0, st, w, (u32x4*)packed, M, Cred, dgrad, mw,
                           NT);
        return;
    }
    hipLaunchKernelGGL((split16_pack_kernel<3>), dim3(nemar_stream_grid(total, 256)), dim3(256), 0, st, w, (u32x4*)packed, M, Cred, dgrad,
                       (const unsigned*)nullptr, NT);
}

NEMAR_SWITCH(int, g_split16_ring3, 0);

Split16Done nemar_split16_conv(const float* src, const void* packed, const float* bias, float* dst, int N, int H, int W, int M, int Cred,
                               int KS, int src_pad, int Hs, int Ws_src, int OH, int OW, int mode, void* scratch, int xcd_map, int variant,
                               long long* tl, void* dual_g_out, MaxWords src_max, const void* ready_planes, int ready_kind,
                               const float* addend, void* out_max, hipStream_t st) {
    bool dual_written = false;
    const long long total = (long long)N * (Cred / 8) * (H + 4) * (W + 4);
    unsigned* const xmw = scratch_max_word(scratch, N, Cred, H, W);
    const unsigned* xmax = xmw;
    int xstride = 0;
    const void* const ready = (variant == 4 && KS == 3 && src_pad == 1 && Hs == H && Ws_src == W && ready_kind == mode &&
                               src_max.words && src_max.count == N) ? ready_planes : nullptr;
    if (variant == 4) {
        xmax = nemar_split16_source_max(src, N, (long long)Cred * Hs * Ws_src, src_max, xmw, &xstride, st);
        if (!ready && dual_g_out && KS == 3 && src_pad == 1 && Hs == H && Ws_src == W && Cred % 64 == 0 &&
            (mode == SPLIT16_DGRAD_REFLECT || mode == SPLIT16_ZERO))
        {
            nemar_split16_dual_split(src, scratch, dual_g_out, N, Cred, H, W, mode, xmax, xstride, st);
            dual_written = true;
        } else if (!ready)
            hipLaunchKernelGGL((split_planes_kernel<2>), dim3(nemar_cdiv(total, 256)), dim3(256), 0, st, src, (u32x4*)scratch, N, Cred, H, W,
                               mode, total, xmax, xstride, src_pad, Hs, Ws_src);
    } else {
        hipLaunchKernelGGL((split_planes_kernel<3>), dim3(nemar_cdiv(total, 256)), dim3(256), 0, st, src, (u32x4*)scratch, N, Cred, H, W,
                           mode, total, (const unsigned*)nullptr, 0, src_pad, Hs, Ws_src);
    }
    Split16Params p;
    p.planes = ready ? (const u32x4*)ready : (const u32x4*)scratch;
    p.wp = (const u32x4*)packed;
    p.bias = bias;
    p.bias_al = (((uintptr_t)bias) & 15) == 0 ? 1 : 0;
    p.dst = dst;
    p.N = N; p.H = H; p.W = W; p.M = M; p.Cred = Cred;
    p.Ws = W + 4;
    p.HpWs = (H + 4) * (W + 4);
    p.wshift = ilog2(W);
    p.RT = 256 / W;
    p.tiles_per_img = H / p.RT;
    p.mblks = M / 128;
    p.halo_instr = nemar_cdiv((long long)(p.RT + KS - 1) * p.Ws * 16, 1024);
    p.fold = mode == SPLIT16_DGRAD_REFLECT;
    p.aux_instr = p.fold ? nemar_cdiv((long long)2 * p.Ws * 16, 1024) : 0;
    p.plane16 = total;
    p.tl = tl;
    p.xmax = xmax;
    p.xstride = xstride;
    p.wmax = pack_max_word(const_cast<void*>(packed), M, Cred, KS);
    p.OH = OH; p.OW = OW;
    p.halo16 = (p.RT + KS - 1) * p.Ws;
    p.aux16 = p.fold ? 2 * p.Ws : 0;
    const int tiles = N * p.tiles_per_img * p.mblks;
    p.ksplit = nemar_split16_ksplit(N, H, W, M, Cred);
    p.slab_stride = (long long)N * M * OH * OW;
    const bool fuse = p.ksplit == 1 && variant == 4 && KS == 3 && !bias && (addend || out_max);
    p.addend = fuse ? addend : nullptr;
    p.maxw = fuse ? (unsigned*)out_max : nullptr;
    p.maxw_lazy = (p.maxw && nemar_max_words_lazy() && p.tiles_per_img * p.mblks <= 0xFFFF) ? 1 : 0;
    float* const final_dst = dst;
    if (p.ksplit > 1) p.dst = (float*)((char*)scratch + nemar_split16_scratch_bytes(N, Cred, H, W));
    const int grid = tiles * p.ksplit;
    p.xcd = (xcd_map && grid % 8 == 0 && (grid / 8) % (p.mblks * p.ksplit) == 0) ? 1 : 0;
    const int region = p.halo_instr + p.aux_instr;
    const dim3 g(grid);
#ifdef NEMAR_HOST_EMULATION
#define S16_GO_(NBW_, NPL_, KS_, RING_, EPI_) { hipLaunchKernelGGL((igemm_split16_kernel<NBW_, NPL_, KS_, RING_, EPI_>), g, dim3(256), 0, st, p); }
#else
#define S16_GO_(NBW_, NPL_, KS_, RING_, EPI_)                                                                           \
    {                                                                                                                   \
        const size_t need_ = ((size_t)(RING_) * 256 * (NPL_) + (size_t)2 * 2 * (NPL_) * (p.halo16 + p.aux16)) * 16;     \
        const size_t lds_ = nemar_lds_bytes(reinterpret_cast<const void*>(&igemm_split16_kernel<NBW_, NPL_, KS_, RING_, EPI_>), need_,      \
                                            (g_lds_claim & 2) != 0);                    \
        hipLaunchKernelGGL((igemm_split16_kernel<NBW_, NPL_, KS_, RING_, EPI_>), g, dim3(256), lds_, st, p);            \
    }
#endif
#define S16_GO(NBW_, NPL_, KS_, RING_) S16_GO_(NBW_, NPL_, KS_, RING_, 0)
    if (variant == 4) {
        const int ipr = nemar_cdiv(p.halo16, 64) + nemar_cdiv(p.aux16, 64);
        const int nbw = nemar_cdiv(nemar_cdiv(4 * ipr, 4), KS * KS - 3);
        NEMAR_AB_ONLY(const bool ring3 = g_split16_ring3 && KS == 3 && ((size_t)3 * 512 + (size_t)8 * (p.halo16 + p.aux16)) * 16 <= 80 * 1024 - 512;)
        S16_TIMED_LAUNCH(
            if (KS == 4) {
                if (nbw <= 1) S16_GO(1, 2, 4, 4)
                else S16_GO(2, 2, 4, 4)
            }
            NEMAR_AB_ONLY(else if (ring3) {
                if (nbw <= 1) S16_GO(1, 2, 3, 3)
                else if (nbw == 2) S16_GO(2, 2, 3, 3)
                else S16_GO(3, 2, 3, 3)
            })
            else if (fuse && p.addend && nbw <= 1) S16_GO_(1, 2, 3, 4, 2)
            else if (fuse && p.addend && nbw == 2) S16_GO_(2, 2, 3, 4, 2)
            else if (fuse && p.addend) S16_GO_(3, 2, 3, 4, 2)
            else if (fuse && nbw <= 1) S16_GO_(1, 2, 3, 4, 1)
            else if (fuse && nbw == 2) S16_GO_(2, 2, 3, 4, 1)
            else if (fuse) S16_GO_(3, 2, 3, 4, 1)
            else if (nbw <= 1) S16_GO(1, 2, 3, 4)
            else if (nbw == 2) S16_GO(2, 2, 3, 4)
            else S16_GO(3, 2, 3, 4))
        if (p.ksplit > 1) nemar_sum_partials(p.dst, p.slab_stride, p.ksplit, final_dst, p.slab_stride, false, st);
        if (p.maxw && !p.maxw_lazy) max_words_finalize(p.maxw, N, p.tiles_per_img * p.mblks, st);
        return {dual_written, fuse};
    }
#ifdef NEMAR_AB
    if (variant == 3) {
        const int ipr = nemar_cdiv(p.halo16, 64) + nemar_cdiv(p.aux16, 64);
        const int nbw = nemar_cdiv(nemar_cdiv(6 * ipr, 4), KS * KS - 3);
        if (KS == 4) {
            if (nbw <= 1) S16_GO(1, 3, 4, 4)
            else S16_GO(2, 3, 4, 4)
        } else if (nbw <= 2) S16_GO(2, 3, 3, 4)
        else S16_GO(3, 3, 3, 4)
        if (p.ksplit > 1) nemar_sum_partials(p.dst, p.slab_stride, p.ksplit, final_dst, p.slab_stride, false, st);
        return {dual_written, fuse};
    }
#endif
#undef S16_GO
#undef S16_GO_
    (void)region;
    return {dual_written, fuse};
}
```

### nemar_amd/csrc/core.hip

```cpp
#include "common.h"
#include <stdarg.h>
#include <mutex>
#include <unordered_map>

#ifdef NEMAR_AB
int g_lds_claim = NEMAR_LDS_CLAIM_DEFAULT;
#endif

size_t nemar_lds_bytes(const void* kernel, size_t need, bool claim) {
#ifdef NEMAR_HOST_EMULATION
    (void)kernel; (void)claim;
    return need;
#else
    static std::mutex mu;
    static std::unordered_map<unsigned long long, size_t> fill_of;
    size_t fill;
    {
        std::lock_guard<std::mutex> lock(mu);
        int dev = 0;
        (void)hipGetDevice(&dev);
        const unsigned long long key = (unsigned long long)(uintptr_t)kernel ^ ((unsigned long long)(dev + 1) << 56);
        auto it = fill_of.find(key);
        if (it == fill_of.end()) {
            hipFuncAttributes fa;
            size_t stat = 0;
            if (hipFuncGetAttributes(&fa, kernel) == hipSuccess) stat = fa.sharedSizeBytes;
            int cu = 0;
            if (hipDeviceGetAttribute(&cu, hipDeviceAttributeMaxSharedMemoryPerMultiprocessor, dev) != hipSuccess || cu < 160 * 1024) cu = 160 * 1024;
            fill = (size_t)cu > stat ? (size_t)cu - stat : 0;
            if (fill < need) fill = need;
            const hipError_t e = hipFuncSetAttribute(kernel, hipFuncAttributeMaxDynamicSharedMemorySize, (int)fill);
            if (e != hipSuccess) nemar_set_error("hipFuncSetAttribute(MaxDynamicSharedMemorySize = %zu): %s", fill, hipGetErrorString(e));
            (void)hipGetLastError();
            it = fill_of.emplace(key, fill).first;
        } else if (it->second < need) {
            const hipError_t e = hipFuncSetAttribute(kernel, hipFuncAttributeMaxDynamicSharedMemorySize, (int)need);
            if (e != hipSuccess) nemar_set_error("hipFuncSetAttribute(MaxDynamicSharedMemorySize = %zu): %s", need, hipGetErrorString(e));
            (void)hipGetLastError();
            it->second = need;
        }
        fill = it->second;
    }
    return (claim && fill > need) ? fill : need;
#endif
}

#define NEMAR_HIP_VERSION 607

static thread_local char g_err[512] = "";
static thread_local int g_max_words_lazy = 0;
bool nemar_max_words_lazy() { return g_max_words_lazy != 0; }
NEMAR_API int nemar_set_max_words_lazy(int on) {
    const int prev = g_max_words_lazy;
    g_max_words_lazy = on ? 1 : 0;
    return prev;
}

void nemar_set_error(const char* fmt, ...) {
    va_list ap;
    va_start(ap, fmt);
    vsnprintf(g_err, sizeof(g_err), fmt, ap);
    va_end(ap);
}

NEMAR_API int nemar_version(void) { return NEMAR_HIP_VERSION; }

NEMAR_API const char* nemar_last_error(void) { return g_err; }
```

### nemar_amd/csrc/norm_planes.hip

```cpp
#include "common.h"
#include "max_words.h"
#include "conv_split16.h"

namespace {

typedef unsigned u32x4 __attribute__((ext_vector_type(4)));
typedef _Float16 f16x2 __attribute__((ext_vector_type(2)));
constexpr int ACT_NONE = 0, ACT_RELU = 1, ACT_LRELU = 2;

__device__ __forceinline__ float np_act(float v, int act, float slope) {
    if (act == ACT_RELU) return fmaxf(v, 0.f);
    if (act == ACT_LRELU) return v > 0.f ? v : v * slope;
    return v;
}
__device__ __forceinline__ float np_pow2_scale(unsigned maxbits) {
    const int e = (int)((maxbits >> 23) & 255u);
    if (e == 0 || e == 255) return 1.f;
    const int se = 127 + 11 - (e - 127);
    if (se < 1 || se > 254) return 1.f;
    return __builtin_bit_cast(float, (unsigned)se << 23);
}
__device__ __forceinline__ unsigned np_f16(float v) {
    const _Float16 h = (_Float16)v;
    return (unsigned)__builtin_bit_cast(unsigned short, h);
}
__device__ __forceinline__ void np_split(float v, unsigned& h, unsigned& l) {
    h = np_f16(v);
    l = np_f16(v - (float)__builtin_bit_cast(_Float16, (unsigned short)h));
}
__device__ __forceinline__ unsigned np_finite_mag(float v) {
    const unsigned u = __builtin_bit_cast(unsigned, v) & 0x7fffffffu;
    return u < 0x7f800000u ? u : 0u;
}
__device__ __forceinline__ void np_philox(unsigned c0, unsigned c1, unsigned c2, unsigned c3, unsigned k0, unsigned k1, unsigned* out) {
#pragma unroll
    for (int r = 0; r < 10; ++r) {
        const unsigned hi0 = __umulhi(0xD2511F53u, c0), lo0 = 0xD2511F53u * c0;
        const unsigned hi1 = __umulhi(0xCD9E8D57u, c2), lo1 = 0xCD9E8D57u * c2;
        const unsigned n0 = hi1 ^ c1 ^ k0, n1 = lo1, n2 = hi0 ^ c3 ^ k1, n3 = lo0;
        c0 = n0; c1 = n1; c2 = n2; c3 = n3;
        k0 += 0x9E3779B9u;
        k1 += 0xBB67AE85u;
    }
    out[0] = c0; out[1] = c1; out[2] = c2; out[3] = c3;
}

struct NormPlanesParams {
    const float* x;
    const float* residual;
    const unsigned* resmax;
    float* y;
    float* stats;
    u32x4* planes;
    unsigned* scale_words;
    unsigned* maxw;
    long long plane16;
    int N, C, H, W;
    float eps, slope, bound0;
    int act;
    int dropout;
    unsigned thresh;
    float dscale;
    unsigned seed_lo, seed_hi, offset;
    const unsigned* obase;
    int lazy;
    int dbg;
    u32x4* xw;
    long long xplane16;
    int CPR, Hx;
};

constexpr int XT_MAX = 64 * 72;
constexpr int NP_LDS_BYTES = 8 * (XT_MAX + 8) * 2 > 16 * 256 * 16 ? 8 * (XT_MAX + 8) * 2 : 16 * 256 * 16;

__device__ __forceinline__ void block_sum8(float* s, float* red, float* tot) {
    const int lane = threadIdx.x & 63, wid = threadIdx.x >> 6;
#pragma unroll
    for (int j = 0; j < 8; ++j) s[j] = wave_sum(s[j]);
    __syncthreads();
    if (lane == 0) {
#pragma unroll
        for (int j = 0; j < 8; ++j) red[wid * 8 + j] = s[j];
    }
    __syncthreads();
    if (threadIdx.x < 8) {
        float t = 0.f;
        for (int w = 0; w < 16; ++w) t += red[w * 8 + threadIdx.x];
        red[128 + threadIdx.x] = t;
    }
    __syncthreads();
#pragma unroll
    for (int j = 0; j < 8; ++j) tot[j] = uniform_f(red[128 + j]);
}

__device__ __forceinline__ int np_unit_of_block(int b, int total) {
    if (total & 63) return b;
    const int x = b & 7, r = b >> 3;
    return (((r >> 3) << 3) + x) * 8 + (r & 7);
}

#ifdef NEMAR_NP_FWD_OCC2
__global__ __launch_bounds__(1024, 8) void instnorm_planes_kernel(NormPlanesParams p) {
#else
__global__ __launch_bounds__(1024) void instnorm_planes_kernel(NormPlanesParams p) {
#endif
    __shared__ float red[136];
    __shared__ unsigned mred[16];
    __shared__ __attribute__((aligned(16))) unsigned char np_lds[NP_LDS_BYTES];
    u32x4 (*const xpose)[256] = reinterpret_cast<u32x4 (*)[256]>(np_lds);
    const int CG = p.C >> 3;
    const int unit = np_unit_of_block((int)blockIdx.x, (int)gridDim.x);
    const int n = unit / CG, cg = unit - n * CG;
    const int HW = p.H * p.W, W = p.W, H = p.H;
    const int t = threadIdx.x;
    const bool active = 4 * t < HW;
    const size_t cbase = ((size_t)n * p.C + (size_t)cg * 8) * HW;
    float v[8][4];
    float s[8], tot[8], mean[8], rstd[8];
#pragma unroll
    for (int j = 0; j < 8; ++j) {
        float4 q = make_float4(0.f, 0.f, 0.f, 0.f);
        if (active) q = *reinterpret_cast<const float4*>(p.x + cbase + (size_t)j * HW + 4 * t);
        v[j][0] = q.x; v[j][1] = q.y; v[j][2] = q.z; v[j][3] = q.w;
        s[j] = (q.x + q.y) + (q.z + q.w);
    }
    const float inv = 1.f / (float)HW;
    if (!(p.dbg & 4)) block_sum8(s, red, tot); else { for (int j = 0; j < 8; ++j) tot[j] = s[j] * 1024.f; }
#pragma unroll
    for (int j = 0; j < 8; ++j) {
        mean[j] = tot[j] * inv;
        float q = 0.f;
#pragma unroll
        for (int e = 0; e < 4; ++e) {
            const float d = active ? v[j][e] - mean[j] : 0.f;
            v[j][e] = d;
            q += d * d;
        }
        s[j] = q;
    }
    if (!(p.dbg & 4)) block_sum8(s, red, tot); else { for (int j = 0; j < 8; ++j) tot[j] = s[j] * 1024.f; }
    float corr[8];
#pragma unroll
    for (int j = 0; j < 8; ++j) s[j] = (v[j][0] + v[j][1]) + (v[j][2] + v[j][3]);
    if (!(p.dbg & 4)) block_sum8(s, red, corr); else { for (int j = 0; j < 8; ++j) corr[j] = s[j] * 1024.f; }
#pragma unroll
    for (int j = 0; j < 8; ++j) {
        const float c = corr[j] * inv;
        rstd[j] = 1.f / sqrtf(tot[j] * inv + p.eps);
        if (fabsf(c) * rstd[j] > 7.62939453125e-6f) {
            mean[j] += c;
            rstd[j] = 1.f / sqrtf(fmaxf(tot[j] * inv - c * c, 0.f) + p.eps);
#pragma unroll
// ... 58 lines not shown
#pragma unroll
        for (int pl = 0; pl < 2; ++pl) {
            if (p.dbg & 1) break;
            __syncthreads();
#pragma unroll
            for (int e = 0; e < 4; ++e) xpose[wid][(p.dbg & 2) ? e * 64 + lane : lane * 4 + e] = pl ? lw[e] : hw[e];
            __syncthreads();
            u32x4* const dst = hp + (pl ? p.plane16 : 0);
#pragma unroll
            for (int e = 0; e < 4; ++e) {
                const int P = wid * 256 + e * 64 + lane;
                if (P >= HW) continue;
                const u32x4 word = xpose[wid][e * 64 + lane];
                const int row = P / W, col = P - row * W;
                auto put = [&](int prow) {
                    u32x4* const r = dst + (size_t)prow * Ws;
                    r[col + 1] = word;
                    if (col == 1) r[0] = word;
                    if (col == W - 2) r[W + 1] = word;
                    if (col == W - 1) { r[W + 2] = z; r[W + 3] = z; }
                };
                put(row + 1);
                if (row == 1) put(0);
                if (row == H - 2) put(H + 1);
                if (row == 0 || row == H - 1) {
                    u32x4* const r = dst + (size_t)(row == 0 ? H + 2 : H + 3) * Ws;
                    r[col + 1] = z;
                    if (col == 0) r[0] = z;
                    if (col == W - 1) { r[W + 1] = z; r[W + 2] = z; r[W + 3] = z; }
                }
            }
        }
    }
    if (p.xw) {
        unsigned short* const xt = reinterpret_cast<unsigned short*>(np_lds);
        const int RS = p.CPR * 8, CS = H * RS + 8;
        const int row = (4 * t) / W, c0 = 4 * t - row * W;
        const int CBLK = p.C >> 6, FX = p.Hx * p.CPR;
        const int nwords = 8 * FX;
#pragma unroll
        for (int pl = 0; pl < 2; ++pl) {
            __syncthreads();
            if (active) {
#pragma unroll
                for (int j = 0; j < 8; ++j) {
                    unsigned short u[4];
#pragma unroll
                    for (int e = 0; e < 4; ++e) u[e] = (unsigned short)(((pl ? lw[e][j >> 1] : hw[e][j >> 1]) >> (16 * (j & 1))) & 0xffffu);
                    unsigned short* const r = xt + j * CS + row * RS + c0 + 1;
                    r[0] = u[0];
                    *reinterpret_cast<unsigned*>(r + 1) = (unsigned)u[1] | ((unsigned)u[2] << 16);
                    r[3] = u[3];
                    if (c0 == 0) r[-1] = u[1];
                    if (c0 == W - 4) {
                        r[4] = u[2];
                        for (int z = W + 2; z < RS; ++z) xt[j * CS + row * RS + z] = 0;
                    }
                }
            }
            __syncthreads();
            u32x4* const dst = p.xw + (pl ? p.xplane16 : 0) + (((size_t)n * CBLK + (cg >> 3)) * FX) * 64 + (cg & 7) * 8;
            for (int i = t; i < nwords; i += 1024) {
                const int cc = i & 7, f = i >> 3;
                const int yp = f / p.CPR, q = f - yp * p.CPR;
                u32x4 word = u32x4{0u, 0u, 0u, 0u};
                if (yp <= H + 1) {
                    const int sr = yp == 0 ? 1 : (yp == H + 1 ? H - 2 : yp - 1);
                    word = *reinterpret_cast<const u32x4*>(xt + cc * CS + sr * RS + q * 8);
                }
                dst[(size_t)f * 64 + cc] = word;
            }
        }
    }
    if (p.maxw) {
#pragma unroll
        for (int o = 32; o > 0; o >>= 1) omax = max(omax, (unsigned)__shfl_xor((int)omax, o, 64));
        if ((t & 63) == 0) mred[t >> 6] = omax;
        __syncthreads();
        if (t == 0) {
            unsigned m = mred[0];
            for (int i = 1; i < 16; ++i) m = max(m, mred[i]);
            p.maxw[p.N + unit] = m;
            if (p.lazy && cg == 0) p.maxw[n] = NEMAR_MAX_LAZY_MARK | (unsigned)CG;
        }
    }
}


struct NormBwdPlanesParams {
    const float* x;
    const float* stats;
    const float* gy;
    const unsigned* gymax;
    float* gx;
    u32x4* dpl;
    u32x4* gpl;
    unsigned* scale_words;
    float* bsum;
    long long dplane16, gplane16;
    int N, C, H, W;
    int CPR, Hg;
    int reflect;
    int act;
    float slope, bmul;
    int dropout;
    unsigned thresh;
    float dscale;
    unsigned seed_lo, seed_hi, offset;
    const unsigned* obase;
};

__device__ __forceinline__ float np_act_df(float xhat, int act, float slope) {
    if (act == ACT_RELU) return xhat > 0.f ? 1.f : 0.f;
    if (act == ACT_LRELU) return xhat > 0.f ? 1.f : slope;
    return 1.f;
}

static size_t np_bwd_lds_bytes(int H, int W) {
    const size_t tile = (size_t)8 * (H * W + 8) * 2, side = (size_t)4 * 8 * (W + H) * sizeof(float);
    return tile > side ? tile : side;
}

__device__ __forceinline__ unsigned np_t4() {
#ifdef NEMAR_HOST_EMULATION
    return 4u * threadIdx.x;
#else
    unsigned v;
    asm volatile("v_lshlrev_b32 %0, 2, %1" : "=v"(v) : "v"((unsigned)threadIdx.x));
    return v;
#endif
}

__global__ __launch_bounds__(1024, 8) void instnorm_bwd_planes_kernel(NormBwdPlanesParams p) {
#ifdef NEMAR_HOST_EMULATION
    __shared__ __attribute__((aligned(16))) unsigned short tile16[8 * (4096 + 8)];
#else
    extern __shared__ __attribute__((aligned(16))) unsigned short tile16[];
#endif
    __shared__ float red[16 * 16 + 16];
    __shared__ float rmax[16];
    const int CG = p.C >> 3;
    const int unit = np_unit_of_block((int)blockIdx.x, (int)gridDim.x);
    const int n = unit / CG, cg = unit - n * CG;
    const int HW = p.H * p.W, W = p.W, H = p.H;
    const int t = threadIdx.x, lane = t & 63, wid = t >> 6;
    const bool active = 4 * t < HW;
    const size_t cbase = ((size_t)n * p.C + (size_t)cg * 8) * HW;
    #define NP_TOFF (active ? np_t4() : 0u)
    float g[8][4];
    {
        float m = 0.f;
        for (int c = t; c < p.C; c += 1024) m = fmaxf(m, p.stats[2 * ((size_t)n * p.C + c) + 1]);
        m = wave_max(m);
        if (lane == 0) rmax[wid] = m;
    }
    const float dneg = p.act == ACT_RELU ? 0.f : (p.act == ACT_LRELU ? p.slope : 1.f);
#pragma unroll
    for (int j = 0; j < 8; ++j) {
        const size_t pl = (size_t)n * p.C + (size_t)cg * 8 + j;
        const float mean = p.stats[2 * pl], rstd = p.stats[2 * pl + 1];
        const float4 a = *reinterpret_cast<const float4*>(p.x + cbase + (size_t)j * HW + NP_TOFF);
        const float4 b = *reinterpret_cast<const float4*>(p.gy + cbase + (size_t)j * HW + NP_TOFF);
        g[j][0] = b.x; g[j][1] = b.y; g[j][2] = b.z; g[j][3] = b.w;
        if (p.dropout) {
            const unsigned long long q = ((unsigned long long)n * p.C + (unsigned long long)cg * 8 + j) * (unsigned long long)(HW >> 2) + t;
            unsigned r[4];
// ... 129 lines not shown
                    }
                    vv[z] = v;
                }
                f16x2 h, l;
                h[0] = (_Float16)vv[0];
                h[1] = (_Float16)vv[1];
                l[0] = (_Float16)(vv[0] - (float)h[0]);
                l[1] = (_Float16)(vv[1] - (float)h[1]);
                hwd[k] = __builtin_bit_cast(unsigned, h);
                lwd[k] = __builtin_bit_cast(unsigned, l);
            }
            hp[(size_t)prow * Ws + pslot] = hwd;
            hp[p.dplane16 + (size_t)prow * Ws + pslot] = lwd;
        }
    }
    auto halves = [&](int pl, int j, int k) -> unsigned {
        f16x2 h;
        h[0] = (_Float16)g[j][2 * k];
        h[1] = (_Float16)g[j][2 * k + 1];
        if (pl) {
            f16x2 l;
            l[0] = (_Float16)(g[j][2 * k] - (float)h[0]);
            l[1] = (_Float16)(g[j][2 * k + 1] - (float)h[1]);
            return __builtin_bit_cast(unsigned, l);
        }
        return __builtin_bit_cast(unsigned, h);
    };
    const int TS = HW + 8;
    const int KBLK = p.C >> 6, F = p.Hg * p.CPR;
    u32x4* const gdst = p.gpl ? p.gpl + (((size_t)n * KBLK + (cg >> 3)) * F) * 64 + (cg & 7) * 8 : nullptr;
#pragma unroll 1
    for (int pl = 0; pl < 2; ++pl) {
        __syncthreads();
        if (active) {
#pragma unroll
            for (int j = 0; j < 8; ++j) *reinterpret_cast<uint2*>(tile16 + j * TS + np_t4()) = make_uint2(halves(pl, j, 0), halves(pl, j, 1));
        }
        __syncthreads();
        if (p.dpl) {
            u32x4* const dst = hp + (pl ? p.dplane16 : 0);
            for (int i = t; i < Hp * Ws; i += 1024) {
                const int prow = i / Ws, pslot = i - prow * Ws;
                const bool inner = prow >= 1 && prow <= H && pslot >= 1 && pslot <= W;
                if (!inner && p.reflect && (prow >= H + 2 ? (pslot >= 1 && pslot != W + 1) : (prow >= 1 && prow <= H && pslot >= W + 2))) continue;
                u32x4 word = u32x4{0u, 0u, 0u, 0u};
                if (inner) {
                    const unsigned short* const src = tile16 + (prow - 1) * W + (pslot - 1);
#pragma unroll
                    for (int k = 0; k < 4; ++k) word[k] = (unsigned)src[(2 * k) * TS] | ((unsigned)src[(2 * k + 1) * TS] << 16);
                }
                dst[i] = word;
            }
        }
        if (p.gpl) {
            u32x4* const dst = gdst + (pl ? p.gplane16 : 0);
            for (int i = t; i < 8 * F; i += 1024) {
                const int cc = i & 7, f = i >> 3;
                const int y = f / p.CPR, q = f - y * p.CPR;
                u32x4 word = u32x4{0u, 0u, 0u, 0u};
                if (y < H && q * 8 < W) word = *reinterpret_cast<const u32x4*>(tile16 + cc * TS + y * W + q * 8);
                dst[(size_t)f * 64 + cc] = word;
            }
        }
    }
}
#undef NP_TOFF

NEMAR_SWITCH(int, g_norm_planes_dbg, 0);
}

extern const unsigned* g_dropout_base;

#ifdef NEMAR_AB
void nemar_norm_planes_debug(int bits) { g_norm_planes_dbg = bits; }
#endif

NEMAR_API size_t nemar_conv2d_x_planes_bytes(int N, int C, int H, int W, int KS) {
    if (KS != 3 || N <= 0 || N > 256 || C <= 0 || C % 64 || H < 4 || W < 8 || W % 8 || H * W > 4096) return 0;
    const int CPR = (W + 2 + 7) / 8, Hg = (H + 3) / 4 * 4;
    if (H * CPR * 8 > XT_MAX) return 0;
    return (size_t)2 * N * C * (Hg + 2) * CPR * 16;
}

NEMAR_API int nemar_instnorm_fwd_planes(const float* x, const float* residual, const void* residual_max_words, float* y, float* stats,
                                        int N, int C, int H, int W, float eps, int act, float slope, float dropout_p,
                                        unsigned long long seed, unsigned offset, void* planes, void* scale_words, void* max_words,
                                        void* wgrad_planes, void* stream) {
    NEMAR_CLEAR_HIP_ERROR();
    NEMAR_REQUIRE(x && stats && planes && scale_words, "instnorm_fwd_planes: null pointer");
    NEMAR_REQUIRE(N > 0 && N <= 256 && C > 0 && C % 8 == 0 && C / 8 <= NEMAR_MAX_PARTIALS, "instnorm_fwd_planes: bad N=%d C=%d", N, C);
    NEMAR_REQUIRE(H >= 4 && W >= 4 && W % 4 == 0 && H * W <= 4096, "instnorm_fwd_planes: unsupported plane %dx%d (W %% 4 == 0, HW <= 4096)", H, W);
    NEMAR_REQUIRE(act == ACT_NONE || act == ACT_RELU || act == ACT_LRELU, "instnorm_fwd_planes: unsupported act %d", act);
    NEMAR_REQUIRE(!residual || residual_max_words, "instnorm_fwd_planes: a residual needs its per-sample max words (the bound of the sum)");
    NEMAR_REQUIRE(dropout_p >= 0.f && dropout_p < 1.f, "instnorm_fwd_planes: bad dropout p");
    NEMAR_REQUIRE((((uintptr_t)x | (uintptr_t)residual | (uintptr_t)y | (uintptr_t)planes) & 15) == 0, "instnorm_fwd_planes: pointers must be 16-byte aligned");
    NormPlanesParams p;
    p.x = x; p.residual = residual; p.resmax = (const unsigned*)residual_max_words; p.y = y; p.stats = stats;
    p.planes = (u32x4*)planes; p.scale_words = (unsigned*)scale_words; p.maxw = (unsigned*)max_words;
    p.plane16 = (long long)N * (C / 8) * (H + 4) * (W + 4);
    p.N = N; p.C = C; p.H = H; p.W = W;
    p.eps = eps; p.slope = slope; p.act = act;
    p.bound0 = sqrtf((float)(H * W)) * (dropout_p > 0.f ? 1.f / (1.f - dropout_p) : 1.f);
    const double t = (double)dropout_p * 4294967296.0;
    p.dropout = dropout_p > 0.f ? 1 : 0;
    p.thresh = t >= 4294967295.0 ? 4294967295u : (unsigned)t;
    p.dscale = dropout_p > 0.f ? 1.f / (1.f - dropout_p) : 1.f;
    p.dbg = g_norm_planes_dbg;
    p.lazy = (max_words && nemar_max_words_lazy() && C / 8 <= 0xFFFF) ? 1 : 0;
    p.obase = g_dropout_base;
    p.seed_lo = (unsigned)(seed & 0xffffffffu); p.seed_hi = (unsigned)(seed >> 32); p.offset = offset;
    p.xw = (u32x4*)wgrad_planes;
    p.CPR = (W + 2 + 7) / 8;
    p.Hx = (H + 3) / 4 * 4 + 2;
    p.xplane16 = (long long)N * C * p.Hx * p.CPR;
    NEMAR_REQUIRE(!wgrad_planes || (nemar_conv2d_x_planes_bytes(N, C, H, W, 3) > 0 && ((uintptr_t)wgrad_planes & 15) == 0),
                  "instnorm_fwd_planes: this shape has no weight-gradient planes (N=%d C=%d %dx%d)", N, C, H, W);
    hipStream_t st = (hipStream_t)stream;
    hipLaunchKernelGGL(instnorm_planes_kernel, dim3(N * (C / 8)), dim3(1024), 0, st, p);
    if (max_words && !p.lazy) max_words_finalize((unsigned*)max_words, N, C / 8, st);
    NEMAR_CHECK_LAUNCH("instnorm_fwd_planes");
    return NEMAR_OK;
}

NEMAR_API int nemar_instnorm_bwd_planes(const float* x, const float* stats, const float* gy, const void* gy_max_words, int N, int C,
                                        int H, int W, int act, float slope, float dropout_p, unsigned long long seed, unsigned offset,
                                        int pad_mode, float* gx, void* dgrad_planes, void* wgrad_planes, void* scale_words,
                                        float* bias_partials, void* stream) {
    NEMAR_CLEAR_HIP_ERROR();
    NEMAR_REQUIRE(x && stats && gy && gy_max_words && scale_words, "instnorm_bwd_planes: null pointer");
    NEMAR_REQUIRE(dgrad_planes || wgrad_planes, "instnorm_bwd_planes: no planes requested (use nemar_instnorm_bwd)");
    NEMAR_REQUIRE(N > 0 && N <= 256 && C > 0 && C % 8 == 0, "instnorm_bwd_planes: bad N=%d C=%d", N, C);
    NEMAR_REQUIRE(H >= 4 && W >= 4 && W % 4 == 0 && H * W <= 4096, "instnorm_bwd_planes: unsupported plane %dx%d (W %% 4 == 0, HW <= 4096)", H, W);
    NEMAR_REQUIRE(!wgrad_planes || (C % 64 == 0 && W % 8 == 0), "instnorm_bwd_planes: weight-gradient planes need C %% 64 == 0 and W %% 8 == 0");
    NEMAR_REQUIRE(act == ACT_NONE || act == ACT_RELU || act == ACT_LRELU, "instnorm_bwd_planes: unsupported act %d", act);
    NEMAR_REQUIRE(dropout_p >= 0.f && dropout_p < 1.f, "instnorm_bwd_planes: bad dropout p");
    NEMAR_REQUIRE(pad_mode == 0 || pad_mode == 1, "instnorm_bwd_planes: bad pad_mode %d", pad_mode);
    NEMAR_REQUIRE((((uintptr_t)x | (uintptr_t)gy | (uintptr_t)gx | (uintptr_t)dgrad_planes | (uintptr_t)wgrad_planes) & 15) == 0,
                  "instnorm_bwd_planes: pointers must be 16-byte aligned");
    NormBwdPlanesParams p;
    p.x = x; p.stats = stats; p.gy = gy; p.gymax = (const unsigned*)gy_max_words; p.gx = gx;
    p.dpl = (u32x4*)dgrad_planes; p.gpl = (u32x4*)wgrad_planes; p.scale_words = (unsigned*)scale_words; p.bsum = bias_partials;
    p.N = N; p.C = C; p.H = H; p.W = W;
    p.CPR = (W + 2 + 7) / 8;
    p.Hg = (H + 3) / 4 * 4;
    p.dplane16 = (long long)N * (C / 8) * (H + 4) * (W + 4);
    p.gplane16 = (long long)N * C * p.Hg * p.CPR;
    p.reflect = pad_mode;
    p.act = act; p.slope = slope;
    p.dscale = dropout_p > 0.f ? 1.f / (1.f - dropout_p) : 1.f;
    p.bmul = (2.f + sqrtf((float)(H * W))) * p.dscale;
    const double t = (double)dropout_p * 4294967296.0;
    p.dropout = dropout_p > 0.f ? 1 : 0;
    p.thresh = t >= 4294967295.0 ? 4294967295u : (unsigned)t;
    p.obase = g_dropout_base;
    p.seed_lo = (unsigned)(seed & 0xffffffffu); p.seed_hi = (unsigned)(seed >> 32); p.offset = offset;
    const size_t lds = nemar_lds_bytes(reinterpret_cast<const void*>(&instnorm_bwd_planes_kernel), np_bwd_lds_bytes(H, W), false);
#ifdef NEMAR_HOST_EMULATION
    hipLaunchKernelGGL(instnorm_bwd_planes_kernel, dim3(N * (C / 8)), dim3(1024), 0, (hipStream_t)stream, p);
    (void)lds;
#else
    hipLaunchKernelGGL(instnorm_bwd_planes_kernel, dim3(N * (C / 8)), dim3(1024), lds, (hipStream_t)stream, p);
#endif
    NEMAR_CHECK_LAUNCH("instnorm_bwd_planes");
    return NEMAR_OK;
}

NEMAR_API int nemar_bias_from_partials(const float* bias_partials, int N, int C, float* gb, void* stream) {
    NEMAR_CLEAR_HIP_ERROR();
    NEMAR_REQUIRE(bias_partials && gb && N > 0 && C > 0, "bias_from_partials: bad arguments");
    nemar_sum_partials(bias_partials, C, N, gb, C, true, (hipStream_t)stream);
    NEMAR_CHECK_LAUNCH("bias_from_partials");
    return NEMAR_OK;
}
```

### nemar_amd/ops.py

```python
import ctypes
import os
import weakref

import torch
from torch.autograd import Function
from torch.autograd.function import once_differentiable

from . import _lib

L = _lib.load()



class _SizeQueries:

    def __init__(self, lib):
        self._lib, self._memo = lib, {}

    def __getattr__(self, name):
        fn = getattr(self._lib, name)
        memo = self._memo

        def q(*a):
            key = (name, a)
# ... 117 lines not shown
        if not _side_on[0]:
            self.ctx = None
            return self
        side = _side_stream_of(self.device)
        main = torch.cuda.current_stream(self.device)
        _main_streams[self.device] = main
        side.wait_stream(main)
        if not torch.cuda.is_current_stream_capturing() and not _KEEP_ALL:
            while _side_keep and _side_keep[0][0] is not None and _side_keep[0][0].query():
                _event_pool.append(_side_keep.popleft()[0])
        self.kept = [t for t in self.keep if t is not None]
        _side_busy[0] = True
        if not _side_cb[0]:
            torch.autograd.Variable._execution_engine.queue_callback(join_side)
            _side_cb[0] = True
        self.ctx = torch.cuda.stream(side)
        self.ctx.__enter__()
        _lane[0] = 1
        return self

    def __exit__(self, *a):
        if self.ctx is not None:
            ev = None
            if not torch.cuda.is_current_stream_capturing():
                ev = _event_pool.pop() if _event_pool else torch.cuda.Event()
                ev.record(torch.cuda.current_stream(self.device))
            _side_keep.append((ev, self.kept))
            _lane[0] = 0
            self.ctx.__exit__(*a)


def _main_lane_grad(buf, device):
    if _side_busy[0] and id(buf) in _side_touched:
        side = _side_streams.get(device)
        if side is not None:
            torch.cuda.current_stream(device).wait_stream(side)


def order_current_after_both(device):
    if not _side_busy[0]:
        return
    side = _side_streams.get(device)
    main = _main_streams.get(device)
    if side is None or main is None:
        return
    cur = torch.cuda.current_stream(device)
    other = main if cur == side else side
    cur.wait_stream(other)


def join_side():
    if _side_busy[0]:
        for dev, side in _side_streams.items():
            torch.cuda.current_stream(dev).wait_stream(side)
        _side_busy[0] = False
        for ring in _garena.values():
            for slot in ring:
                slot[1] = None
    _side_cb[0] = False
    _side_keep.clear()
    _side_touched.clear()


_scratch_need = {}
_arena = {}


def _conv_scratch(N, H, W, K, C, R, S, stride, pad, device):
    key = (N, H, W, K, C, R, S, stride, pad)
    need = _scratch_need.get(key)
    if need is None:
        need = _scratch_need[key] = L.conv2d_scratch(N, H, W, K, C, R, S, stride, pad)
    if not need:
        return None
    akey = (device, _lane[0])
    buf = _arena.get(akey)
    if buf is None or buf.numel() * 4 < need:
        _retire(buf)
        buf = torch.empty(int(need) // 4 + 64, dtype=torch.float32, device=device)
        _arena[akey] = buf
    return buf


_garena = {}
_garena_next = {}
_gplanes_need = {}
GY_RING = int(os.environ.get("NEMAR_GY_RING", "4"))
_GY_HANDOVER = os.environ.get("NEMAR_GY_HANDOVER", "1") == "1"


def _gy_planes(N, C, H, W, K, R, S, stride, pad, pad_mode, device):
    if _side_on[0] and not _GY_HANDOVER:
        return None, None
    key = (N, C, H, W, K, R, S, stride, pad, pad_mode)
    need = _gplanes_need.get(key)
    if need is None:
        need = _gplanes_need[key] = L.conv2d_gy_planes_bytes(N, C, H, W, K, R, S, stride, pad, pad_mode)
    if not need:
        return None, None
    ring = _garena.setdefault(device, [[None, None] for _ in range(GY_RING)])
    k = _garena_next.get(device, 0)
    _garena_next[device] = (k + 1) % GY_RING
    slot = ring[k]
    if slot[1] is not None:
        torch.cuda.current_stream(device).wait_event(slot[1])
        slot[1] = None
    if slot[0] is None or slot[0].numel() * 4 < need:
        _retire(slot[0])
        slot[0] = torch.empty(int(need) // 4 + 64, dtype=torch.float32, device=device)
    return slot[0], slot


def _extras(arena=None, src_max=None, src2_max=None, planes=None, gy_out=None, src2_planes=None, addend=None, out_max=None, bias_partials=None):
    if arena is None and src_max is None and src2_max is None and planes is None and addend is None:
        return None
    e = _lib.ConvExtras()
    if addend is not None:
        e.addend = addend.data_ptr()
    if bias_partials is not None:
        e.bias_partials = bias_partials.data_ptr()
    if out_max is not None:
        e.out_max_words = out_max.data_ptr()
    if arena is not None:
        e.scratch, e.scratch_bytes = arena.data_ptr(), arena.numel() * 4
    if src_max is not None:
        e.src_max_words, e.src_max_count = src_max.data_ptr(), src_max.numel()
    if src2_max is not None:
        e.src2_max_words, e.src2_max_count = src2_max.data_ptr(), src2_max.numel()
    if planes is not None:
        e.src_planes = planes.data_ptr()
    if gy_out is not None:
        e.gy_planes_out, e.gy_planes_bytes = gy_out.data_ptr(), gy_out.numel() * 4
    if src2_planes is not None:
        e.src2_planes = src2_planes.data_ptr()
    return ctypes.byref(e)


_absmax_pool = {}


MAX_PARTIALS = 2048


def _max_words(n, device):
    return torch.empty(n * (1 + MAX_PARTIALS), dtype=torch.int32, device=device)


def _wants_max(t):
    return t.dim() == 4 and 128 <= t.shape[1] <= MAX_PARTIALS and t.shape[1] % 16 == 0 and t.shape[0] <= 256


def _tag_max(t, words, lazy=False):
    if lazy:
        t._nemar_absmax_lazy = (words[:t.shape[0]], t._version)
    else:
        t._nemar_absmax = (words[:t.shape[0]], t._version)


def _absmax_word(t, lazy_ok=False):
    lazy = getattr(t, '_nemar_absmax_lazy', None)
    if lazy is not None and not (lazy[1] == t._version and lazy[0].numel() == t.shape[0]):
        lazy = None
    if lazy_ok and lazy is not None:
        return lazy[0]
    have = getattr(t, '_nemar_absmax', None)
    if have is not None and have[1] == t._version and have[0].numel() == t.shape[0]:
        return have[0]
    if lazy is not None:
        L.max_words_finalize(_p(lazy[0]), int(t.shape[0]), _stream())
        t._nemar_absmax = lazy
        return lazy[0]
    return _absmax_word_compute(t)


_LAZY_MAX = os.environ.get("NEMAR_LAZY_MAX", "1") != "0"


class _lazy_max:

    def __init__(self, on=True):
        self.on = on and _LAZY_MAX

    def __enter__(self):
        if self.on:
            L.set_max_words_lazy(1)
        return self

    def __exit__(self, *a):
        if self.on:
            L.set_max_words_lazy(0)


def _absmax_word_compute(t):
    n = int(t.shape[0])
    if _step_params["on"]:
        word = torch.zeros(n, dtype=torch.int32, device=t.device)
        L.absmax_samples(_p(t), n, t.numel() // n, _p(word), _stream())
        return word
    pool = _absmax_pool.get(t.device)
# ... 78 lines not shown
            L.pack_plan_record(self.plan)

    def __exit__(self, *a):
        if self.plan is not None:
            L.pack_plan_record(-1)


def _packed(weight, kind, nbytes):
    key = (id(weight), kind)
    own = getattr(weight, '_pack_epoch', None)
    static = (_param_epoch.n, weight._version, weight.data_ptr(), tuple(weight.shape), L.config_epoch())
    token = (static, own.n if own is not None else 0)
    ent = _pack_cache.get(key)
    mine = ent is not None and ent.ref() is weight and ent.buf.numel() * 4 >= nbytes
    if mine and ent.token == token:
        return ent.buf, 1, None
    if mine and ent.plan_gen == _plan_gen[0] and ent.token[0] == static:
        return ent.buf, 1, None
    buf = ent.buf if mine else torch.empty(int(nbytes) // 4 + 64, dtype=torch.float32, device=weight.device)
    new = _PackEntry(buf, token, weakref.ref(weight, lambda _r, k=key: _pack_cache.pop(k, None)))
    plan = None
    if _plans_on[0] and own is not None and own.plan is not None and not _pinned[0]:
        if mine and ent.plan_gen == _plan_gen[0]:
            new.plan_gen = ent.plan_gen
        else:
            plan = own.plan
            new.plan_gen = _plan_gen[0]
    _pack_cache[key] = new
    return buf, 0, plan


def grad_ready(param):
    gs = getattr(param, '_grad_sync', None)
    if gs is not None:
        gs.ready(param)


def _note_use(param):
    gs = getattr(param, '_grad_sync', None)
    if gs is not None and param is not None:
        gs.note_use(param)


def _grad_buffer(param):
    view = getattr(param, '_flat_grad', None)
    if view is not None:
        g = param.grad
        if g is None or g.data_ptr() != view.data_ptr():
            if g is not None:
                view.add_(g)
            param.grad = view
        return view
    if param.grad is None:
        param.grad = torch.zeros_like(param, memory_format=torch.contiguous_format)
    return param.grad


class _Conv2d(Function):
    @staticmethod
    def forward(ctx, x, x2, weight, bias, stride, pad, pad_mode, act, slope, wshape, with_skip=False):
        x, x2, w, b = _c(x), _c(x2), _c(weight), _c(bias)
        ctx.with_skip = bool(with_skip)
        if with_skip:
            ctx.set_materialize_grads(False)
        if wshape is not None:
            w = w.view(wshape)
        N, C0, H, W = x.shape
        C1 = 0 if x2 is None else x2.shape[1]
        K, C, R, S = w.shape
        if C != C0 + C1:
            raise ValueError("conv2d: weight expects %d input channels, got %d+%d" % (C, C0, C1))
        OH = (H + 2 * pad - R) // stride + 1
        OW = (W + 2 * pad - S) // stride + 1
        y = torch.empty((N, K, OH, OW), dtype=torch.float32, device=x.device)
        wsb = Q.conv2d_fwd_workspace(N, H, W, K, C, R, S, stride, pad)
        ws, hit, plan = _packed(weight, ('fwd', stride, pad, N, H, W), wsb)
        arena = _conv_scratch(N, H, W, K, C, R, S, stride, pad, x.device) if x2 is None else None
        tag = 'igemm_fwd_resblock' if (K == 256 and C == 256 and R == 3 and pad_mode == PAD_REFLECT) else None
        with (_span(tag) if tag else contextlib.nullcontext()):
            xmax = ready = None
            if arena is not None:
                ready = _planes_of(x) if (pad_mode == PAD_REFLECT and R == 3 and S == 3 and stride == 1 and pad == 1) else None
                xmax = ready[1] if ready is not None else _absmax_word(x)
            with _record(plan):
                L.conv2d_fwd_ex(_p(x), C0, _p(x2), C1, _p(w), _p(b), _p(y), N, H, W, K, R, S, stride, pad, pad_mode, act,
                                slope, _p(ws), wsb, hit, _stream(), _extras(arena, xmax, None, ready[0] if ready is not None else None))
        ctx.xmax = xmax
        xp = _xplanes_of(x) if ready is not None else None
        ctx.xplanes = xp[0] if (xp is not None and xp[1] is ready[1]) else None
        ctx.grad_from = int(getattr(x, '_nemar_grad_from', 0)) if x2 is None else 0
        ctx.save_for_backward(x, x2, w, y if act != ACT_NONE else None)
        ctx.weight, ctx.bias = weight, bias
        _note_use(weight)
        if bias is not None:
            _note_use(bias)
        ctx.cfg = (stride, pad, pad_mode, act, slope)
        if with_skip:
            return y, x.view_as(x)
        return y

    @staticmethod
    @once_differentiable
    def backward(ctx, gy, gskip=None):
        x, x2, w, y = ctx.saved_tensors
        stride, pad, pad_mode, act, slope = ctx.cfg
        ctx.gskip = _c(gskip) if (ctx.with_skip and ctx.needs_input_grad[0]) else None
        if gy is None:
            return (ctx.gskip,) + (None,) * 10
        gy = _c(gy)
        N, C0, H, W = x.shape
        C1 = 0 if x2 is None else x2.shape[1]
        K, C, R, S = w.shape
        OH, OW = gy.shape[2:]
        st = _stream()
        if act != ACT_NONE:
            g = torch.empty_like(gy)
            L.act_bwd(_p(gy), _p(y), _p(g), gy.numel(), act, slope, st)
        else:
            g = gy
        need_x, need_x2, need_w, need_b = ctx.needs_input_grad[0], ctx.needs_input_grad[1], \
            ctx.needs_input_grad[2], ctx.needs_input_grad[3]
        gmax = _absmax_word(g) if ctx.xmax is not None else None
        return _Conv2d._backward_body(ctx, x, x2, w, g, N, C0, C1, H, W, K, C, R, S, OH, OW, stride, pad, pad_mode, st,
                                      need_x, need_x2, need_w, need_b, gmax)

    @staticmethod
    def _backward_body(ctx, x, x2, w, g, N, C0, C1, H, W, K, C, R, S, OH, OW, stride, pad, pad_mode, st, need_x, need_x2, need_w,
                       need_b, gmax):
        gx = gx2 = gpl = gslot = None
        if need_x or need_x2:
            gx = torch.empty_like(x) if need_x else None
            gx2 = torch.empty_like(x2) if (need_x2 and x2 is not None) else None
            if x2 is not None and gx2 is None:
                gx2 = torch.empty_like(x2)
            wsb = Q.conv2d_bwd_data_workspace(N, C, H, W, K, R, S, stride, pad, pad_mode)
            if pad_mode == PAD_REFLECT and pad > 0 and x2 is not None:
                raise NotImplementedError("reflect-padded conv over a concatenated input has no data-gradient kernel")
            n0 = getattr(ctx, 'grad_from', 0)
            if 0 < n0 < N:
                _zero(gx[:n0])
                Nd, gd, gxd = N - n0, g[n0:], gx[n0:]
            else:
                Nd, gd, gxd = N, g, gx
            wsb = Q.conv2d_bwd_data_workspace(Nd, C, H, W, K, R, S, stride, pad, pad_mode)
            ws, hit, plan = _packed(ctx.weight, ('dgrad', stride, pad, pad_mode, need_x, Nd, H, W), wsb)
            arena = _conv_scratch(Nd, H, W, K, C, R, S, stride, pad, g.device)
            if arena is not None and need_w and Nd == N and gmax is not None and x2 is None:
                gpl, gslot = _gy_planes(N, C, H, W, K, R, S, stride, pad, pad_mode, g.device)
            rb = K == 256 and C == 256 and R == 3 and pad_mode == PAD_REFLECT
            gskip = getattr(ctx, 'gskip', None)
            ride = (gskip is not None and gx is not None and gx2 is None and Nd == N and arena is None
                    and Q.conv2d_scratch(N, H, W, K, C, R, S, stride, pad) == 0
                    and Q.conv2d_bwd_data_addend_ok(N, C, H, W, K, R, S, stride, pad, pad_mode) == 1)
            with _record(plan), (_span('dgrad_resblock') if rb else contextlib.nullcontext()):
                L.conv2d_bwd_data_ex(_p(gd), _p(w), None, ACT_NONE, 0.0, _p(gxd), C0, _p(gx2), C1, Nd, H, W, K, OH, OW, R, S,
                                     stride, pad, pad_mode, _p(ws), wsb, hit, st,
                                     _extras(arena, gmax[n0:] if (gmax is not None and Nd != N) else gmax, gy_out=gpl,
                                             addend=gskip if ride else None))
            if gskip is not None and gx is not None and not ride:
                L.add2(_p(gx), _p(gskip), _p(gx), gx.numel(), st)
            if gpl is not None and not L.last_gy_planes():
                gpl = None
            if not need_x2:
                gx2 = None
        want_b = need_b and ctx.bias is not None
        if need_w:
            _use = R != 7 or _SIDE_K7
            if not (need_x or need_x2):
                _use = False
# ... 121 lines not shown

    @staticmethod
    def forward(ctx, x, act, slope):
        x = _c(x)
        y = torch.empty_like(x)
        L.act_fwd(_p(x), _p(y), x.numel(), act, slope, _stream())
        ctx.save_for_backward(y)
        ctx.act, ctx.slope = act, slope
        return y

    @staticmethod
    def backward(ctx, gy):
        (y,) = ctx.saved_tensors
        gy = _c(gy)
        gx = torch.empty_like(gy)
        L.act_bwd(_p(gy), _p(y), _p(gx), gy.numel(), ctx.act, ctx.slope, _stream())
        return gx, None, None


def activation(x, act, slope=0.2):
    return x if act == ACT_NONE else _Activation.apply(x, act, slope)


def conv_transpose2d(x, weight, bias=None, stride=2, pad=1, out_pad=1, act=ACT_NONE, slope=0.2):
    return _ConvTranspose2d.apply(x, weight, bias, stride, pad, out_pad, act, slope)


def _planes_ok(x, residual):
    N, C, H, W = x.shape
    return _planes_on[0] and _wants_max(x) and W % 4 == 0 and H >= 4 and H * W <= 4096 and _conv_scratch(N, H, W, C, C, 3, 3, 1, 1, x.device) is not None


_planes_on = [os.environ.get("NEMAR_PLANES", "1") != "0"]


def tune_planes(on):
    _planes_on[0] = bool(on)


def _planes_of(t):
    have = getattr(t, '_nemar_planes', None)
    return have if have is not None and have[2] == t._version else None


def _xplanes_of(t):
    have = getattr(t, '_nemar_xplanes', None)
    return have if have is not None and have[2] == t._version else None


_xplanes_on = [os.environ.get("NEMAR_XPLANES", "1") != "0"]
_xplanes_need = {}


def _x_planes_buffer(N, C, H, W, device):
    if not _xplanes_on[0]:
        return None
    key = (N, C, H, W)
    need = _xplanes_need.get(key)
    if need is None:
        need = _xplanes_need[key] = L.conv2d_x_planes_bytes(N, C, H, W, 3)
    if not need:
        return None
    return torch.empty(int(need), dtype=torch.uint8, device=device)


class _InstanceNorm(Function):
    @staticmethod
    def forward(ctx, x, residual, act, slope, eps, planes, drop_p):
        x, residual = _c(x), _c(residual)
        N, C, H, W = x.shape
        y = torch.empty_like(x)
        stats = torch.empty((N * C, 2), dtype=torch.float32, device=x.device)
        ctx.drop = None
        if planes and _planes_ok(x, residual):
            words = _max_words(N, x.device)
            scale_words = torch.empty(N, dtype=torch.int32, device=x.device)
            buf = torch.empty(2 * N * (C // 8) * (H + 4) * (W + 4) * 16, dtype=torch.uint8, device=x.device)
            seed = off = 0
            if drop_p > 0.0:
                _dropout_state["offset"] = (_dropout_state["offset"] + 1) & 0xFFFFFFFF
                seed, off = _dropout_state["seed"], _dropout_state["offset"]
                ctx.drop = (drop_p, seed, off)
            xbuf = _x_planes_buffer(N, C, H, W, x.device) if any(ctx.needs_input_grad[:2]) else None
            L.instnorm_fwd_planes(_p(x), _p(residual), _p(_absmax_word(residual)) if residual is not None else None, _p(y), _p(stats),
                                  N, C, H, W, eps, act, slope, drop_p, seed, off, _p(buf), _p(scale_words), _p(words), _p(xbuf), _stream())
            _tag_max(y, words)
            y._nemar_planes = (buf, scale_words, y._version)
            if xbuf is not None:
                y._nemar_xplanes = (xbuf, scale_words, y._version)
        else:
            if _wants_max(x) and drop_p <= 0.0:
                words = _max_words(N, x.device)
                with _lazy_max():
                    L.instnorm_fwd_max(_p(x), _p(residual), _p(y), _p(stats), N * C, H * W, eps, act, slope, _p(words), C, _stream())
                _tag_max(y, words, lazy=_LAZY_MAX)
            else:
                L.instnorm_fwd(_p(x), _p(residual), _p(y), _p(stats), N * C, H * W, eps, act, slope, _stream())
            if drop_p > 0.0:
                _dropout_state["offset"] = (_dropout_state["offset"] + 1) & 0xFFFFFFFF
                ctx.drop = (drop_p, _dropout_state["seed"], _dropout_state["offset"])
                _dropout_launch(y, y, *ctx.drop)
        ctx.save_for_backward(x, stats)
        ctx.cfg = (act, slope)
        return y

    @staticmethod
    @once_differentiable
    def backward(ctx, gy):
        x, stats = ctx.saved_tensors
        act, slope = ctx.cfg
        gy = _c(gy)
        N, C, H, W = x.shape
        gx = None
        if ctx.needs_input_grad[0]:
            g = gy
            if ctx.drop is not None:
                if ctx.needs_input_grad[1]:
                    raise RuntimeError("instance_norm: dropout and a residual cannot be fused in one call")
                g = torch.empty_like(gy)
                L.dropout(_p(gy), _p(g), gy.numel(), ctx.drop[0], ctx.drop[1], ctx.drop[2], _stream())
            gx = torch.empty_like(x)
            if _wants_max(x):
                words = _max_words(N, x.device)
                with _lazy_max():
                    L.instnorm_bwd_max(_p(x), _p(stats), _p(g), _p(gx), N * C, H * W, act, slope, _p(words), C, _stream())
                _tag_max(gx, words, lazy=_LAZY_MAX)
            else:
                L.instnorm_bwd(_p(x), _p(stats), _p(g), _p(gx), N * C, H * W, act, slope, _stream())
        gres = gy if ctx.needs_input_grad[1] else None
        return gx, gres, None, None, None, None, None


def grad_from(x, n0):
    x._nemar_grad_from = int(n0)
    return x


def instance_norm(x, act=ACT_NONE, slope=0.2, residual=None, eps=1e-5, planes=False, dropout_p=0.0):
    return _InstanceNorm.apply(x, residual, act, slope, eps, bool(planes), float(dropout_p))


_norm_segments = [1]


@contextlib.contextmanager
def norm_segments(k):
    prev = _norm_segments[0]
    _norm_segments[0] = int(k)
    try:
        yield
    finally:
        _norm_segments[0] = prev


class _BatchNorm(Function):
    @staticmethod
    def forward(ctx, x, residual, weight, bias, running_mean, running_var, num_batches_tracked, training, act, slope, eps, momentum,
                drop_p, segments):
        x, residual = _c(x), _c(residual)
        N, C, H, W = x.shape
        HW = H * W
        S = int(segments) if training else 1
        if N % S:
            raise ValueError("batch_norm: %d segments do not divide a batch of %d" % (S, N))
        if training and (N // S) * HW == 1:
            raise ValueError("Expected more than 1 value per channel when training, got input size %s" % (list(x.shape),))
        y = torch.empty_like(x)
        ctx.drop = None
# ... 15 lines not shown
                                 N, C, HW, eps, act, slope, drop_p, seed, off, _p(words), _stream())
        if words is not None:
            _tag_max(y, words)
        ctx.save_for_backward(x, saved, weight, bias)
        ctx.weight, ctx.bias = weight, bias
        _note_use(weight)
        _note_use(bias)
        ctx.cfg = (S, bool(training), act, slope)
        return y

    @staticmethod
    @once_differentiable
    def backward(ctx, gy):
        x, saved, w, b = ctx.saved_tensors
        S, training, act, slope = ctx.cfg
        gy = _c(gy)
        N, C, H, W = x.shape
        need_x, need_res, need_w, need_b = ctx.needs_input_grad[:4]
        gx = torch.empty_like(x) if need_x else None
        gw = _grad_buffer(ctx.weight) if need_w else None
        gb = _grad_buffer(ctx.bias) if need_b else None
        if gx is not None or gw is not None or gb is not None:
            p, seed, off = ctx.drop if ctx.drop is not None else (0.0, 0, 0)
            wsb = Q.batchnorm_workspace(N, C, H * W, S)
            L.batchnorm_bwd(_p(x), _p(gy), _p(gx), _p(w), _p(b), _p(saved), _p(gw), _p(gb), N, C, H * W, S, int(training), act, slope,
                            p, seed, off, _p(_workspace(wsb, x.device)), wsb, _stream())
        if gw is not None:
            grad_ready(ctx.weight)
        if gb is not None:
            grad_ready(ctx.bias)
        return gx, (gy if need_res else None), None, None, None, None, None, None, None, None, None, None, None, None


def batch_norm(x, weight, bias, running_mean, running_var, num_batches_tracked, training, act=ACT_NONE, slope=0.2, residual=None, eps=1e-5,
               momentum=0.1, dropout_p=0.0):
    if running_mean.dtype != torch.float32 or running_var.dtype != torch.float32 or num_batches_tracked.dtype != torch.int64:
        raise TypeError("batch_norm: running statistics must be fp32 and the counter int64")
    return _BatchNorm.apply(x, residual, weight, bias, running_mean, running_var, num_batches_tracked, bool(training), act, slope, float(eps),
                            float(momentum), float(dropout_p), _norm_segments[0])


_fused_block_on = [os.environ.get("NEMAR_FUSED_BLOCK", "1") != "0"]
_fusable = {}


def fused_blocks(on=None):
    prev = _fused_block_on[0]
    if on is not None:
        _fused_block_on[0] = bool(on)
    return prev


def _block_fusable(x, C):
    if not (_fused_block_on[0] and _planes_on[0] and _xplanes_on[0] and x.is_cuda and x.dim() == 4 and x.dtype == torch.float32):
        return False
    N, Cx, H, W = x.shape
    if Cx != C:
        return False
    key = (N, C, H, W, L.config_epoch())
    ok = _fusable.get(key)
    if ok is None:
        ok = (_wants_max(x) and W % 8 == 0 and H >= 4 and H * W <= 4096
              and L.conv2d_bwd_data_fusable(N, C, H, W, C, 3, 3, 1, 1, PAD_REFLECT) == 1
              and L.conv2d_x_planes_bytes(N, C, H, W, 3) > 0
              and L.conv2d_scratch(N, H, W, C, C, 3, 3, 1, 1) > 0)
        _fusable[key] = bool(ok)
    return ok


def _chan_planes_buffer(N, C, H, W, device):
    return torch.empty(2 * N * (C // 8) * (H + 4) * (W + 4) * 16, dtype=torch.uint8, device=device)


class _ResBlock(Function):
    @staticmethod
    def forward(ctx, x, w1, b1, w2, b2, drop_p, feeds_block, eps):
        x = _c(x)
        N, C, H, W = x.shape
        dev = x.device
        st = _stream()
        arena = _conv_scratch(N, H, W, C, C, 3, 3, 1, 1, dev)
        wsb = Q.conv2d_fwd_workspace(N, H, W, C, C, 3, 3, 1, 1)

        def conv(src_key, planes, words, weight, bias, y):
            ws, hit, plan = _packed(weight, ('fwd', 1, 1, N, H, W), wsb)
            with _span('igemm_fwd_resblock'), _record(plan):
                L.conv2d_fwd_ex(src_key, C, None, 0, _p(weight), _p(bias), _p(y), N, H, W, C, 3, 3, 1, 1, PAD_REFLECT, ACT_NONE, 0.2,
                                _p(ws), wsb, hit, st, _extras(arena, words, None, planes))

        ready = _planes_of(x)
        xp0 = _xplanes_of(x)
        if ready is not None:
            x_words = ready[1]
            if xp0 is not None and xp0[1] is not ready[1]:
                xp0 = None
        else:
            x_words, xp0 = _absmax_word(x), None
        y1 = torch.empty_like(x)
        conv(_p(x), ready[0] if ready is not None else None, x_words, w1, b1, y1)
        stats1 = torch.empty((N * C, 2), dtype=torch.float32, device=dev)
        p1 = _chan_planes_buffer(N, C, H, W, dev)
        train = any(ctx.needs_input_grad[:5])
        xp1 = _x_planes_buffer(N, C, H, W, dev) if train else None
        scale1 = torch.empty(N, dtype=torch.int32, device=dev)
        seed = off = 0
        if drop_p > 0.0:
            _dropout_state["offset"] = (_dropout_state["offset"] + 1) & 0xFFFFFFFF
            seed, off = _dropout_state["seed"], _dropout_state["offset"]
        with _span('in_fwd_planes_resblock'):
            L.instnorm_fwd_planes(_p(y1), None, None, None, _p(stats1), N, C, H, W, eps, ACT_RELU, 0.2, drop_p, seed, off, _p(p1), _p(scale1),
                                  None, _p(xp1), st)
        y2 = torch.empty_like(x)
        conv(_p(p1), p1, scale1, w2, b2, y2)
        del p1
        out = torch.empty_like(x)
        stats2 = torch.empty((N * C, 2), dtype=torch.float32, device=dev)
        words = _max_words(N, dev)
        if feeds_block:
            pout = _chan_planes_buffer(N, C, H, W, dev)
            xpout = _x_planes_buffer(N, C, H, W, dev) if train else None
            scale_out = torch.empty(N, dtype=torch.int32, device=dev)
            with _span('in_fwd_planes_resblock'), _lazy_max():
                L.instnorm_fwd_planes(_p(y2), _p(x), _p(_absmax_word(x, lazy_ok=True)), _p(out), _p(stats2), N, C, H, W, eps, ACT_NONE, 0.2, 0.0, 0, 0,
                                      _p(pout), _p(scale_out), _p(words), _p(xpout), st)
            out._nemar_planes = (pout, scale_out, out._version)
            if xpout is not None:
                out._nemar_xplanes = (xpout, scale_out, out._version)
        else:
            L.instnorm_fwd_max(_p(y2), _p(x), _p(out), _p(stats2), N * C, H * W, eps, ACT_NONE, 0.2, _p(words), C, st)
        _tag_max(out, words, lazy=feeds_block and _LAZY_MAX)
        ctx.save_for_backward(y1, stats1, y2, stats2, w1, w2)
        ctx.x0 = None if xp0 is not None else x
        ctx.xp0 = xp0[0] if xp0 is not None else None
        ctx.x_words, ctx.xp1, ctx.scale1 = x_words, xp1, scale1
        ctx.params = (w1, b1, w2, b2)
        ctx.drop = (drop_p, seed, off)
        for prm in (w1, b1, w2, b2):
            if prm is not None:
                _note_use(prm)
        return out

    @staticmethod
    @once_differentiable
    def backward(ctx, g_out):
        y1, stats1, y2, stats2, w1v, w2v = ctx.saved_tensors
        w1, b1, w2, b2 = ctx.params
        g_out = _c(g_out)
        N, C, H, W = g_out.shape
        dev = g_out.device
        st = _stream()
        need_x = ctx.needs_input_grad[0]
        need = [ctx.needs_input_grad[1], ctx.needs_input_grad[2] and b1 is not None, ctx.needs_input_grad[3],
                ctx.needs_input_grad[4] and b2 is not None]
        drop_p, seed, off = ctx.drop
        gbytes = _gplanes_need.get((N, C, H, W, C, 3, 3, 1, 1, PAD_REFLECT))
        if gbytes is None:
            gbytes = _gplanes_need[(N, C, H, W, C, 3, 3, 1, 1, PAD_REFLECT)] = L.conv2d_gy_planes_bytes(N, C, H, W, C, 3, 3, 1, 1, PAD_REFLECT)
        arena = _conv_scratch(N, H, W, C, C, 3, 3, 1, 1, dev)
        dwsb = Q.conv2d_bwd_data_workspace(N, C, H, W, C, 3, 3, 1, 1, PAD_REFLECT)

        def norm_bwd(xin, stats, g, gwords, act, p, sd, of, want_d, want_g, want_bias):
            d = _chan_planes_buffer(N, C, H, W, dev) if want_d else None
            gp = torch.empty(int(gbytes), dtype=torch.uint8, device=dev) if want_g else None
            scale = torch.empty(N, dtype=torch.int32, device=dev)
            bsum = torch.empty((N, C), dtype=torch.float32, device=dev) if want_bias else None
            with _span('in_bwd_planes_resblock'):
                L.instnorm_bwd_planes(_p(xin), _p(stats), _p(g), _p(gwords), N, C, H, W, act, 0.2, p, sd, of, 1, None, _p(d), _p(gp), _p(scale),
                                      _p(bsum), st)
            return d, gp, scale, bsum

        def dgrad(d, scale, weight, dst, addend, out_words):
            ws, hit, plan = _packed(weight, ('dgrad', 1, 1, PAD_REFLECT, True, N, H, W), dwsb)
            with _record(plan), _span('dgrad_resblock'):
                L.conv2d_bwd_data_ex(_p(d), _p(weight), None, ACT_NONE, 0.0, _p(dst), C, None, 0, N, H, W, C, H, W, 3, 3, 1, 1, PAD_REFLECT,
                                     _p(ws), dwsb, hit, st, _extras(arena, scale, planes=d, addend=addend, out_max=out_words))

        def wgrad(x_t, xpl, x_words, gp, g_scale, weight, bias, bsum, want_w, want_b):
            if not (want_w or want_b):
                return
            gw = _grad_buffer(weight) if want_w else None
            gb = _grad_buffer(bias) if want_b else None
            if _side_on[0]:
                for buf in (gw, gb):
                    if buf is not None:
                        _side_touched.add(id(buf))
            else:
                for buf in (gw, gb):
                    if buf is not None:
                        _main_lane_grad(buf, dev)
            with _on_side(dev, x_t, xpl, x_words, gp, g_scale, bsum), _span('wgrad_resblock'):
                if want_w:
                    wsb = Q.conv2d_bwd_weight_workspace(N, C, H, W, C, H, W, 3, 3, 1, 1)
                    side_arena = _conv_scratch(N, H, W, C, C, 3, 3, 1, 1, dev)
                    key = x_t if x_t is not None else xpl
                    L.conv2d_bwd_weight_ex(_p(key), C, None, 0, _p(gp), _p(gw), _p(gb) if want_b else None, N, H, W, C, H, W, 3, 3, 1, 1, PAD_REFLECT,
                                           _p(_workspace(wsb, dev)), wsb, _stream(),
                                           _extras(side_arena, x_words, g_scale, planes=xpl, src2_planes=gp, bias_partials=bsum if want_b else None))
                    grad_ready(weight)
                    if want_b:
                        grad_ready(bias)
                elif want_b:
                    L.bias_from_partials(_p(bsum), N, C, _p(gb), _stream())
                    grad_ready(bias)

        gwords = _absmax_word(g_out, lazy_ok=True)
        d2, gp2, scale2, bsum2 = norm_bwd(y2, stats2, g_out, gwords, ACT_NONE, 0.0, 0, 0, True, need[2], need[3])
        gmid = torch.empty_like(g_out)
# ... 673 lines not shown
```

Before: 301.1.

## Fuse instance-norm statistics into split-16 conv forward epilogue

Adds an epilogue variant to the split-16 forward conv that writes per-tile channel partial sums (count, mean, centered sum of squares) via wave butterfly reductions. The instance-norm planes producer then merges these partials instead of making its own statistics pass over the conv output, both in the resblock and in standalone conv-then-norm paths. This removes a full read of the activation for stats, at the cost of extra epilogue registers and shuffles and a small partials buffer. It is on by default through NEMAR_CONV_STATS.

```diff
diff --git a/include/nemar_hip.h b/include/nemar_hip.h
--- a/include/nemar_hip.h
+++ b/include/nemar_hip.h
@@ -67,7 +67,9 @@
     const float* addend;
     void* out_max_words;
     const float* bias_partials;
+    float* stat_partials;
 } nemar_conv_extras;
+int nemar_conv2d_fwd_stat_tiles(int N, int H, int W, int K, int C, int R, int S, int stride, int pad, int pad_mode);
 int nemar_conv2d_bwd_data_fusable(int N, int C, int H, int W, int K, int R, int S, int stride, int pad, int pad_mode);
 int nemar_conv2d_bwd_data_addend_ok(int N, int C, int H, int W, int K, int R, int S, int stride, int pad, int pad_mode);
 size_t nemar_conv2d_x_planes_bytes(int N, int C, int H, int W, int KS);
@@ -117,6 +119,10 @@
                               int N, int C, int H, int W, float eps, int act, float slope, float dropout_p,
                               unsigned long long seed, unsigned offset, void* planes, void* scale_words, void* max_words,
                               void* wgrad_planes, void* stream);
+int nemar_instnorm_fwd_planes_stats(const float* x, const float* residual, const void* residual_max_words, float* y, float* stats,
+                                    int N, int C, int H, int W, float eps, int act, float slope, float dropout_p,
+                                    unsigned long long seed, unsigned offset, void* planes, void* scale_words, void* max_words,
+                                    void* wgrad_planes, const float* stat_partials, int stat_tiles, void* stream);
 int nemar_instnorm_bwd_planes(const float* x, const float* stats, const float* gy, const void* gy_max_words, int N, int C,
                               int H, int W, int act, float slope, float dropout_p, unsigned long long seed, unsigned offset,
                               int pad_mode, float* gx, void* dgrad_planes, void* wgrad_planes, void* scale_words,
diff --git a/nemar_amd/_lib.py b/nemar_amd/_lib.py
--- a/nemar_amd/_lib.py
+++ b/nemar_amd/_lib.py
@@ -52,6 +52,8 @@
     "nemar_instnorm_bwd": (_i, [_vp, _vp, _vp, _vp, _i, _i, _i, _fl, _vp]),
     "nemar_instnorm_fwd_max": (_i, [_vp, _vp, _vp, _vp, _i, _i, _fl, _i, _fl, _vp, _i, _vp]),
     "nemar_instnorm_fwd_planes": (_i, [_vp, _vp, _vp, _vp, _vp, _i, _i, _i, _i, _fl, _i, _fl, _fl, _u64, _u32, _vp, _vp, _vp, _vp, _vp]),
+    "nemar_instnorm_fwd_planes_stats": (_i, [_vp, _vp, _vp, _vp, _vp, _i, _i, _i, _i, _fl, _i, _fl, _fl, _u64, _u32, _vp, _vp, _vp, _vp, _vp, _i, _vp]),
+    "nemar_conv2d_fwd_stat_tiles": (_i, [_i] * 10),
     "nemar_instnorm_bwd_planes": (_i, [_vp, _vp, _vp, _vp, _i, _i, _i, _i, _i, _fl, _fl, _u64, _u32, _i, _vp, _vp, _vp, _vp, _vp, _vp]),
     "nemar_bias_from_partials": (_i, [_vp, _i, _i, _vp, _vp]),
     "nemar_conv2d_bwd_data_fusable": (_i, [_i] * 10),
@@ -120,7 +122,7 @@
     _fields_ = [("scratch", C.c_void_p), ("scratch_bytes", C.c_size_t), ("src_max_words", C.c_void_p), ("src_max_count", C.c_int),
                 ("src2_max_words", C.c_void_p), ("src2_max_count", C.c_int), ("src_planes", C.c_void_p),
                 ("gy_planes_out", C.c_void_p), ("gy_planes_bytes", C.c_size_t), ("src2_planes", C.c_void_p),
-                ("addend", C.c_void_p), ("out_max_words", C.c_void_p), ("bias_partials", C.c_void_p)]
+                ("addend", C.c_void_p), ("out_max_words", C.c_void_p), ("bias_partials", C.c_void_p), ("stat_partials", C.c_void_p)]
 
 
 class Library:
@@ -164,7 +166,7 @@
                                     "(libnemar_hip_ab.so; set NEMAR_AB_LIBRARY=1 before nemar_amd is imported)" % (self.__dict__.get("path"), full))
             raise AttributeError(name)
         fn = fns[full]
-        if {**SIGNATURES, **AB_SIGNATURES}[full][0] is not _i or full in ("nemar_version", "nemar_last_route", "nemar_last_gy_planes", "nemar_config_epoch", "nemar_set_max_words_lazy", "nemar_pack_plan_jobs", "nemar_pack_plan_dirty", "nemar_conv2d_bwd_data_fusable", "nemar_conv2d_bwd_data_addend_ok"):
+        if {**SIGNATURES, **AB_SIGNATURES}[full][0] is not _i or full in ("nemar_version", "nemar_last_route", "nemar_last_gy_planes", "nemar_config_epoch", "nemar_set_max_words_lazy", "nemar_pack_plan_jobs", "nemar_pack_plan_dirty", "nemar_conv2d_bwd_data_fusable", "nemar_conv2d_bwd_data_addend_ok", "nemar_conv2d_fwd_stat_tiles"):
             return fn
 
         if os.environ.get("NEMAR_DEBUG_SYNC"):
diff --git a/nemar_amd/csrc/common.h b/nemar_amd/csrc/common.h
--- a/nemar_amd/csrc/common.h
+++ b/nemar_amd/csrc/common.h
@@ -40,6 +40,7 @@
     const float* addend;
     void* out_max_words;
     const float* bias_partials;
+    float* stat_partials;
 };
 
 void nemar_set_error(const char* fmt, ...);
diff --git a/nemar_amd/csrc/conv.hip b/nemar_amd/csrc/conv.hip
--- a/nemar_amd/csrc/conv.hip
+++ b/nemar_amd/csrc/conv.hip
@@ -520,6 +520,9 @@
         nemar_set_error("conv2d_fwd: workspace %zu < %zu", ws_bytes, sizeof(float) * P.total);
         return NEMAR_EWORKSPACE;
     }
+    NEMAR_REQUIRE(!call.stat_partials || P.stat_tiles > 0,
+                  "conv2d_fwd: stat_partials on a call the wide forward epilogue does not serve (route %d; ask nemar_conv2d_fwd_stat_tiles)", P.route);
+    NEMAR_REQUIRE((((uintptr_t)call.stat_partials) & 15) == 0, "conv2d_fwd: stat_partials must be 16-byte aligned");
     hipStream_t st = (hipStream_t)stream;
     const char* what = "conv2d_fwd";
     g_last_route = P.route;
@@ -543,7 +546,7 @@
         const int mode = pad_mode == BORDER_REFLECT ? SPLIT16_REFLECT : SPLIT16_ZERO;
         if (!prepacked) nemar_split16_pack(w, workspace, K, C, R, 0, g_split16_variant, st);
         nemar_split16_conv(x0, workspace, bias, y, N, H, W, K, C, R, 1, H, W, OH, OW, mode, call.scratch, g_xcd_map, g_split16_variant,
-                           g_tl, nullptr, call.src_max, call.src_planes, call.src_planes_kind, nullptr, nullptr, st);
+                           g_tl, nullptr, call.src_max, call.src_planes, call.src_planes_kind, nullptr, nullptr, call.stat_partials, st);
         what = "conv2d_fwd (split-16)";
         break;
     }
@@ -646,7 +649,7 @@
         const Split16Done done = nemar_split16_conv(gy, workspace, nullptr, gx0, N, H, W, C, K, R, R - 1 - pad, OH, OW, H, W,
                                                     refl ? SPLIT16_DGRAD_REFLECT : SPLIT16_ZERO, call.scratch, g_xcd_map, g_split16_variant, g_tl,
                                                     L.want_gy_planes ? call.gy_planes_out : nullptr, call.src_max, call.src_planes,
-                                                    call.src_planes_kind, call.addend, call.out_max, st);
+                                                    call.src_planes_kind, call.addend, call.out_max, nullptr, st);
         call.gy_planes_written = done.dual_written;
         call.epilogue_fused = done.epilogue_fused;
         what = "conv2d_bwd_data (split-16)";
@@ -937,6 +940,11 @@
     return plan_arena_bytes({N, C, 0, H, W, K, R, S, stride, pad, BORDER_ZERO});
 }
 
+NEMAR_API int nemar_conv2d_fwd_stat_tiles(int N, int H, int W, int K, int C, int R, int S, int stride, int pad, int pad_mode) {
+    if (N <= 0 || H <= 0 || W <= 0 || K <= 0 || C <= 0 || R <= 0 || S <= 0 || stride < 1) return 0;
+    return plan_fwd({N, C, 0, H, W, K, R, S, stride, pad, pad_mode}, ConvFacts::canonical()).stat_tiles;
+}
+
 NEMAR_API size_t nemar_conv2d_gy_planes_bytes(int N, int C, int H, int W, int K, int R, int S, int stride, int pad, int pad_mode) {
     return usual_dgrad(N, C, H, W, K, R, S, stride, pad, pad_mode).gy_planes_need;
 }
@@ -976,6 +984,7 @@
                                   void* workspace, size_t ws_bytes, int prepacked, void* stream, const nemar_conv_extras* extras) {
     ConvCall call = call_from(extras);
     if (extras) { call.src_planes = extras->src_planes; call.src_planes_kind = SPLIT16_REFLECT; }
+    if (extras) call.stat_partials = extras->stat_partials;
     return conv2d_fwd(call, x0, C0, x1, C1, w, bias, y, N, H, W, K, R, S, stride, pad, pad_mode, act, slope, workspace, ws_bytes, prepacked, stream);
 }
 
diff --git a/nemar_amd/csrc/conv_call.h b/nemar_amd/csrc/conv_call.h
--- a/nemar_amd/csrc/conv_call.h
+++ b/nemar_amd/csrc/conv_call.h
@@ -20,6 +20,7 @@
     const float* addend = nullptr;
     void* out_max = nullptr;
     const float* bias_partials = nullptr;
+    float* stat_partials = nullptr;
     bool gy_planes_written = false;
     bool epilogue_fused = false;
     bool addend_done = false;
diff --git a/nemar_amd/csrc/conv_route.h b/nemar_amd/csrc/conv_route.h
--- a/nemar_amd/csrc/conv_route.h
+++ b/nemar_amd/csrc/conv_route.h
@@ -200,6 +200,7 @@
     enum Sub { PLAIN, K7_MANY_FEW, K7_FEW_MANY, SPLIT, SPLIT_ACT } sub;
     size_t pack, slab_off, total;
     int ksplit;
+    int stat_tiles;
     K7MfPlan k7;
     S16gProblem q; S16gPlan pl;
 };
@@ -237,6 +238,7 @@
         P.route = ROUTE_EXACT;
         if (P.ksplit > 1 && (f.act == ACT_NONE || split_act)) P.sub = split_act ? FwdPlan::SPLIT_ACT : FwdPlan::SPLIT;
     }
+    P.stat_tiles = P.route == ROUTE_SPLIT16 ? nemar_split16_stat_tiles(N, H, W, K, C, R, g_split16_variant) : 0;
     return P;
 }
 
diff --git a/nemar_amd/csrc/conv_split16.h b/nemar_amd/csrc/conv_split16.h
--- a/nemar_amd/csrc/conv_split16.h
+++ b/nemar_amd/csrc/conv_split16.h
@@ -18,7 +18,8 @@
 Split16Done nemar_split16_conv(const float* src, const void* packed, const float* bias, float* dst, int N, int H, int W, int M, int Cred,
                                int KS, int src_pad, int Hs, int Ws_src, int OH, int OW, int mode, void* scratch, int xcd_map, int variant,
                                long long* tl, void* dual_g_out, MaxWords src_max, const void* ready_planes, int ready_kind,
-                               const float* addend, void* out_max, hipStream_t st);
+                               const float* addend, void* out_max, float* stat_partials, hipStream_t st);
+int nemar_split16_stat_tiles(int N, int H, int W, int M, int Cred, int KS, int variant);
 
 bool nemar_split16_wgrad_eligible(int N, int C, int H, int W, int K, int R, int S, int stride, int pad);
 size_t nemar_split16_wgrad_scratch_bytes(int N, int C, int H, int W, int K, int KS);
diff --git a/nemar_amd/csrc/conv_split16.hip b/nemar_amd/csrc/conv_split16.hip
--- a/nemar_amd/csrc/conv_split16.hip
+++ b/nemar_amd/csrc/conv_split16.hip
@@ -232,7 +232,26 @@
     const float* addend;
     unsigned* maxw;
     int maxw_lazy;
+    float* statp;
+    int stat_tiles;
 };
+
+template <int HALF>
+__device__ __forceinline__ void stat_bfly_step(float (&a)[64], int lane) {
+    const bool up = (lane & (HALF >> 1)) != 0;
+#pragma unroll
+    for (int k = 0; k < HALF; ++k) {
+        const float keep = up ? a[k + HALF] : a[k], send = up ? a[k] : a[k + HALF];
+        a[k] = keep + __shfl_xor(send, HALF >> 1, 64);
+    }
+}
+__device__ __forceinline__ void stat_bfly(float (&a)[64], int lane) {
+    stat_bfly_step<32>(a, lane);
+    stat_bfly_step<16>(a, lane);
+    stat_bfly_step<8>(a, lane);
+    stat_bfly_step<4>(a, lane);
+    stat_bfly_step<2>(a, lane);
+}
 
 __device__ __forceinline__ void glds16(const u32x4* g, u32x4* lds) {
     __builtin_amdgcn_global_load_lds((const __attribute__((address_space(1))) void*)g,
@@ -496,6 +515,76 @@
 
     const size_t HW = (size_t)p.OH * p.OW;
     const float unscale = NPL == 2 ? 1.f / (pow2_scale(p.xmax[n * p.xstride]) * pow2_scale(*p.wmax)) : 1.f;
+    if (EPI == 3) {
+        float* d0[2];
+#pragma unroll
+        for (int nt = 0; nt < 2; ++nt)
+            d0[nt] = p.dst + (size_t)n * p.M * HW + (size_t)(y0 + row[nt]) * p.OW + col[nt] + (size_t)(mblk * 128 + 4 * lhi) * HW;
+        auto bias16 = [&](int mt, float* bv) {
+#pragma unroll
+            for (int q = 0; q < 4; ++q) {
+                float4 b4 = make_float4(0.f, 0.f, 0.f, 0.f);
+                if (p.bias) {
+                    const float* const bp = p.bias + mblk * 128 + 4 * lhi + mt * 32 + 8 * q;
+                    b4 = p.bias_al ? *reinterpret_cast<const float4*>(bp) : make_float4(bp[0], bp[1], bp[2], bp[3]);
+                }
+                bv[4 * q] = b4.x; bv[4 * q + 1] = b4.y; bv[4 * q + 2] = b4.z; bv[4 * q + 3] = b4.w;
+            }
+        };
+        float s[64];
+#pragma unroll
+        for (int mt = 0; mt < 4; ++mt) {
+            float bv[16];
+            bias16(mt, bv);
+#pragma unroll
+            for (int r = 0; r < 16; ++r) {
+                float v[2];
+#pragma unroll
+                for (int nt = 0; nt < 2; ++nt) {
+                    v[nt] = acc[mt][nt][r];
+                    if (NPL == 2) v[nt] *= unscale;
+                    v[nt] += bv[r];
+                    d0[nt][(size_t)(mt * 32 + (r & 3) + 8 * (r >> 2)) * HW] = v[nt];
+                }
+                s[mt * 16 + r] = v[0] + v[1];
+            }
+            __builtin_amdgcn_sched_barrier(0);
+        }
+        stat_bfly(s, lane);
+        const float tm0 = s[0] * 0.015625f, tm1 = s[1] * 0.015625f;
+        float s1[64], q2[64];
+#pragma unroll
+        for (int mt = 0; mt < 4; ++mt) {
+            float bv[16];
+            bias16(mt, bv);
+#pragma unroll
+            for (int r = 0; r < 16; ++r) {
+                const int i = mt * 16 + r;
+                const float m = __shfl((i & 1) ? tm1 : tm0, (lane & 32) + (i >> 1), 64);
+                float d[2];
+#pragma unroll
+                for (int nt = 0; nt < 2; ++nt) {
+                    float v = acc[mt][nt][r];
+                    if (NPL == 2) v *= unscale;
+                    v += bv[r];
+                    d[nt] = v - m;
+                }
+                s1[i] = d[0] + d[1];
+                q2[i] = d[0] * d[0] + d[1] * d[1];
+            }
+        }
+        stat_bfly(s1, lane);
+        stat_bfly(q2, lane);
+        const int tile = (ptile - n * p.tiles_per_img) * 4 + wid;
+#pragma unroll
+        for (int k = 0; k < 2; ++k) {
+            const int i = 2 * l31 + k, r = i & 15;
+            const int c = mblk * 128 + 4 * lhi + 32 * (i >> 4) + (r & 3) + 8 * (r >> 2);
+            const float lo = s1[k] * 0.015625f;
+            *reinterpret_cast<float4*>(p.statp + (((size_t)n * p.M + c) * p.stat_tiles + tile) * 4) = make_float4(64.f, k ? tm1 : tm0, lo, q2[k] - s1[k] * lo);
+        }
+        return;
+    }
     if (!EPI) {
         const bool with_bias = p.bias != nullptr && zsplit == 0;
         float* d0[2];
@@ -600,6 +689,11 @@
     int ks = 1;
     while (tiles * ks * 2 <= 256 && nchunks % (ks * 2) == 0 && nchunks / (ks * 2) >= 4 && ks < g_split16_ksplit_cap) ks *= 2;
     return ks;
+}
+
+int nemar_split16_stat_tiles(int N, int H, int W, int M, int Cred, int KS, int variant) {
+    if (KS != 3 || variant != 4 || nemar_split16_ksplit(N, H, W, M, Cred) != 1) return 0;
+    return H * W / 64;
 }
 
 size_t nemar_split16_scratch_total(int N, int H, int W, int M, int Cred, int OH, int OW) {
@@ -714,7 +808,7 @@
 Split16Done nemar_split16_conv(const float* src, const void* packed, const float* bias, float* dst, int N, int H, int W, int M, int Cred,
                                int KS, int src_pad, int Hs, int Ws_src, int OH, int OW, int mode, void* scratch, int xcd_map, int variant,
                                long long* tl, void* dual_g_out, MaxWords src_max, const void* ready_planes, int ready_kind,
-                               const float* addend, void* out_max, hipStream_t st) {
+                               const float* addend, void* out_max, float* stat_partials, hipStream_t st) {
     bool dual_written = false;
     const long long total = (long long)N * (Cred / 8) * (H + 4) * (W + 4);
     unsigned* const xmw = scratch_max_word(scratch, N, Cred, H, W);
@@ -767,6 +861,8 @@
     p.addend = fuse ? addend : nullptr;
     p.maxw = fuse ? (unsigned*)out_max : nullptr;
     p.maxw_lazy = (p.maxw && nemar_max_words_lazy() && p.tiles_per_img * p.mblks <= 0xFFFF) ? 1 : 0;
+    p.stat_tiles = nemar_split16_stat_tiles(N, H, W, M, Cred, KS, variant);
+    p.statp = p.stat_tiles && !fuse ? stat_partials : nullptr;
     float* const final_dst = dst;
     if (p.ksplit > 1) p.dst = (float*)((char*)scratch + nemar_split16_scratch_bytes(N, Cred, H, W));
     const int grid = tiles * p.ksplit;
@@ -805,6 +901,9 @@
             else if (fuse && nbw <= 1) S16_GO_(1, 2, 3, 4, 1)
             else if (fuse && nbw == 2) S16_GO_(2, 2, 3, 4, 1)
             else if (fuse) S16_GO_(3, 2, 3, 4, 1)
+            else if (p.statp && nbw <= 1) S16_GO_(1, 2, 3, 4, 3)
+            else if (p.statp && nbw == 2) S16_GO_(2, 2, 3, 4, 3)
+            else if (p.statp) S16_GO_(3, 2, 3, 4, 3)
             else if (nbw <= 1) S16_GO(1, 2, 3, 4)
             else if (nbw == 2) S16_GO(2, 2, 3, 4)
             else S16_GO(3, 2, 3, 4))
diff --git a/nemar_amd/csrc/core.hip b/nemar_amd/csrc/core.hip
--- a/nemar_amd/csrc/core.hip
+++ b/nemar_amd/csrc/core.hip
@@ -45,7 +45,7 @@
 #endif
 }
 
-#define NEMAR_HIP_VERSION 607
+#define NEMAR_HIP_VERSION 608
 
 static thread_local char g_err[512] = "";
 static thread_local int g_max_words_lazy = 0;
diff --git a/nemar_amd/csrc/norm_planes.hip b/nemar_amd/csrc/norm_planes.hip
--- a/nemar_amd/csrc/norm_planes.hip
+++ b/nemar_amd/csrc/norm_planes.hip
@@ -68,6 +68,8 @@
     u32x4* xw;
     long long xplane16;
     int CPR, Hx;
+    const float* statp;
+    int stat_tiles;
 };
 
 constexpr int XT_MAX = 64 * 72;
@@ -292,6 +294,207 @@
             for (int i = 1; i < 16; ++i) m = max(m, mred[i]);
             p.maxw[p.N + unit] = m;
             if (p.lazy && cg == 0) p.maxw[n] = NEMAR_MAX_LAZY_MARK | (unsigned)CG;
+        }
+    }
+}
+
+constexpr int NS_THREADS = 256, NS_PIX = 4 * NS_THREADS;
+constexpr int NS_XT = 32 * 40;
+constexpr int NS_LDS_BYTES = 8 * (NS_XT + 8) * 2 > 4 * 256 * 16 ? 8 * (NS_XT + 8) * 2 : 4 * 256 * 16;
+
+__global__ __launch_bounds__(NS_THREADS) void instnorm_planes_stream_kernel(NormPlanesParams p) {
+    __shared__ float sm[24];
+    __shared__ unsigned mred[4];
+    __shared__ __attribute__((aligned(16))) unsigned char np_lds[NS_LDS_BYTES];
+    u32x4 (*const xpose)[256] = reinterpret_cast<u32x4 (*)[256]>(np_lds);
+    const int CG = p.C >> 3;
+    const int HW = p.H * p.W, W = p.W, H = p.H;
+    const int bands = (HW + NS_PIX - 1) / NS_PIX;
+    int n, cg, band;
+    {
+        const int v = np_unit_of_block((int)blockIdx.x, (int)gridDim.x);
+        if ((p.C & 63) == 0) {
+            int rest = v >> 3;
+            band = rest % bands; rest /= bands;
+            const int CB = CG >> 3;
+            n = rest / CB;
+            cg = (rest - n * CB) * 8 + (v & 7);
+        } else {
+            band = v % bands;
+            const int unit = v / bands;
+            n = unit / CG; cg = unit - n * CG;
+        }
+    }
+    const int t = threadIdx.x;
+    const int t4 = band * NS_THREADS + t;
+    const bool active = 4 * t4 < HW;
+    const size_t cbase = ((size_t)n * p.C + (size_t)cg * 8) * HW;
+    const float inv = 1.f / (float)HW;
+    if (t < 8) {
+        const float4* const pp = reinterpret_cast<const float4*>(p.statp) + ((size_t)n * p.C + (size_t)cg * 8 + t) * p.stat_tiles;
+        const float m0 = pp[0].y;
+        float a = 0.f;
+        for (int i = 0; i < p.stat_tiles; ++i) a += pp[i].x * ((pp[i].y - m0) + pp[i].z);
+        const float delta = a * inv;
+        float m2 = 0.f;
+        for (int i = 0; i < p.stat_tiles; ++i) {
+            const float d = ((pp[i].y - m0) - delta) + pp[i].z;
+            m2 += pp[i].w + pp[i].x * (d * d);
+        }
+        const float rs = 1.f / sqrtf(m2 * inv + p.eps);
+        sm[t] = m0; sm[8 + t] = delta; sm[16 + t] = rs;
+        if (band == 0) {
+            const size_t pl = (size_t)n * p.C + (size_t)cg * 8 + t;
+            p.stats[2 * pl] = m0 + delta;
+            p.stats[2 * pl + 1] = rs;
+        }
+    }
+    __syncthreads();
+    float bound = p.bound0;
+    if (p.residual) bound += __builtin_bit_cast(float, sample_max_word(p.resmax, n, p.N));
+    const unsigned bound_bits = __builtin_bit_cast(unsigned, bound);
+    if (cg == 0 && band == 0 && t == 0) p.scale_words[n] = bound_bits;
+    const float scale = np_pow2_scale(bound_bits);
+    unsigned omax = 0;
+    float v[8][4];
+#pragma unroll
+    for (int j = 0; j < 8; ++j) {
+        float4 q = make_float4(0.f, 0.f, 0.f, 0.f);
+        if (active) q = *reinterpret_cast<const float4*>(p.x + cbase + (size_t)j * HW + 4 * t4);
+        v[j][0] = q.x; v[j][1] = q.y; v[j][2] = q.z; v[j][3] = q.w;
+    }
+#pragma unroll
+    for (int j = 0; j < 8; ++j) {
+        const float m0 = uniform_f(sm[j]), delta = uniform_f(sm[8 + j]), rstd = uniform_f(sm[16 + j]);
+        float o[4];
+#pragma unroll
+        for (int e = 0; e < 4; ++e) {
+            const float d = active ? (v[j][e] - m0) - delta : 0.f;
+            o[e] = np_act(d * rstd, p.act, p.slope);
+        }
+        if (p.dropout) {
+            const unsigned long long q = ((unsigned long long)n * p.C + (unsigned long long)cg * 8 + j) * (unsigned long long)(HW >> 2) + t4;
+            unsigned r[4];
+            np_philox((unsigned)q, (unsigned)(q >> 32), p.offset + (p.obase ? *p.obase : 0u), 0u, p.seed_lo, p.seed_hi, r);
+#pragma unroll
+            for (int e = 0; e < 4; ++e) o[e] = r[e] >= p.thresh ? o[e] * p.dscale : 0.f;
+        }
+        if (p.residual && active) {
+            const float4 q = *reinterpret_cast<const float4*>(p.residual + cbase + (size_t)j * HW + 4 * t4);
+            o[0] += q.x; o[1] += q.y; o[2] += q.z; o[3] += q.w;
+        }
+        if (p.y && active) *reinterpret_cast<float4*>(p.y + cbase + (size_t)j * HW + 4 * t4) = make_float4(o[0], o[1], o[2], o[3]);
+#pragma unroll
+        for (int e = 0; e < 4; ++e) {
+            omax = max(omax, np_finite_mag(o[e]));
+            v[j][e] = o[e];
+        }
+    }
+    u32x4 hw[4], lw[4];
+#pragma unroll
+    for (int e = 0; e < 4; ++e) {
+#pragma unroll
+        for (int k = 0; k < 4; ++k) {
+            f16x2 h, l;
+            h[0] = (_Float16)(v[2 * k][e] * scale);
+            h[1] = (_Float16)(v[2 * k + 1][e] * scale);
+            l[0] = (_Float16)__builtin_fmaf(v[2 * k][e], scale, -(float)h[0]);
+            l[1] = (_Float16)__builtin_fmaf(v[2 * k + 1][e], scale, -(float)h[1]);
+            hw[e][k] = __builtin_bit_cast(unsigned, h);
+            lw[e][k] = __builtin_bit_cast(unsigned, l);
+        }
+    }
+    {
+        const int Ws = W + 4;
+        u32x4* const hp = p.planes + ((size_t)n * CG + cg) * (size_t)(H + 4) * Ws;
+        const u32x4 z = u32x4{0u, 0u, 0u, 0u};
+        const int wid = t >> 6, lane = t & 63;
+#pragma unroll
+        for (int pl = 0; pl < 2; ++pl) {
+            __syncthreads();
+#pragma unroll
+            for (int e = 0; e < 4; ++e) xpose[wid][lane * 4 + e] = pl ? lw[e] : hw[e];
+            __syncthreads();
+            u32x4* const dst = hp + (pl ? p.plane16 : 0);
+#pragma unroll
+            for (int e = 0; e < 4; ++e) {
+                const int P = band * NS_PIX + wid * 256 + e * 64 + lane;
+                if (P >= HW) continue;
+                const u32x4 word = xpose[wid][e * 64 + lane];
+                const int row = P / W, col = P - row * W;
+                auto put = [&](int prow) {
+                    u32x4* const r = dst + (size_t)prow * Ws;
+                    r[col + 1] = word;
+                    if (col == 1) r[0] = word;
+                    if (col == W - 2) r[W + 1] = word;
+                    if (col == W - 1) { r[W + 2] = z; r[W + 3] = z; }
+                };
+                put(row + 1);
+                if (row == 1) put(0);
+                if (row == H - 2) put(H + 1);
+                if (row == 0 || row == H - 1) {
+                    u32x4* const r = dst + (size_t)(row == 0 ? H + 2 : H + 3) * Ws;
+                    r[col + 1] = z;
+                    if (col == 0) r[0] = z;
+                    if (col == W - 1) { r[W + 1] = z; r[W + 2] = z; r[W + 3] = z; }
+                }
+            }
+        }
+    }
+    if (p.xw) {
+        unsigned short* const xt = reinterpret_cast<unsigned short*>(np_lds);
+        const int RB = NS_PIX / W;
+        const int r0 = band * RB, rows = min(RB, H - r0);
+        const int RS = p.CPR * 8, CS = RB * RS + 8;
+        const int row = (4 * t) / W, c0 = 4 * t - row * W;
+        const int CBLK = p.C >> 6, FX = p.Hx * p.CPR;
+        const int nwords = 8 * rows * p.CPR;
+#pragma unroll
+        for (int pl = 0; pl < 2; ++pl) {
+            __syncthreads();
+            if (active) {
+#pragma unroll
+                for (int j = 0; j < 8; ++j) {
+                    unsigned short u[4];
+#pragma unroll
+                    for (int e = 0; e < 4; ++e) u[e] = (unsigned short)(((pl ? lw[e][j >> 1] : hw[e][j >> 1]) >> (16 * (j & 1))) & 0xffffu);
+                    unsigned short* const r = xt + j * CS + row * RS + c0 + 1;
+                    r[0] = u[0];
+                    *reinterpret_cast<unsigned*>(r + 1) = (unsigned)u[1] | ((unsigned)u[2] << 16);
+                    r[3] = u[3];
+                    if (c0 == 0) r[-1] = u[1];
+                    if (c0 == W - 4) {
+                        r[4] = u[2];
+                        for (int z = W + 2; z < RS; ++z) xt[j * CS + row * RS + z] = 0;
+                    }
+                }
+            }
+            __syncthreads();
+            u32x4* const dst = p.xw + (pl ? p.xplane16 : 0) + (((size_t)n * CBLK + (cg >> 3)) * FX) * 64 + (cg & 7) * 8;
+            for (int i = t; i < nwords; i += NS_THREADS) {
+                const int cc = i & 7, f = i >> 3;
+                const int lr = f / p.CPR, q = f - lr * p.CPR;
+                const int sr = r0 + lr;
+                const u32x4 word = *reinterpret_cast<const u32x4*>(xt + cc * CS + lr * RS + q * 8);
+                dst[((size_t)(sr + 1) * p.CPR + q) * 64 + cc] = word;
+                if (sr == 1) dst[(size_t)q * 64 + cc] = word;
+                if (sr == H - 2) dst[((size_t)(H + 1) * p.CPR + q) * 64 + cc] = word;
+            }
+            if (r0 + rows == H) {
+                const u32x4 z = u32x4{0u, 0u, 0u, 0u};
+                for (int i = t + 8 * (H + 2) * p.CPR; i < 8 * FX; i += NS_THREADS) dst[(size_t)(i >> 3) * 64 + (i & 7)] = z;
+            }
+        }
+    }
+    if (p.maxw) {
+#pragma unroll
+        for (int o = 32; o > 0; o >>= 1) omax = max(omax, (unsigned)__shfl_xor((int)omax, o, 64));
+        if ((t & 63) == 0) mred[t >> 6] = omax;
+        __syncthreads();
+        if (t == 0) {
+            const int parts = CG * bands;
+            p.maxw[p.N + (size_t)n * parts + cg * bands + band] = max(max(mred[0], mred[1]), max(mred[2], mred[3]));
+            if (p.lazy && cg == 0 && band == 0) p.maxw[n] = NEMAR_MAX_LAZY_MARK | (unsigned)parts;
         }
     }
 }
@@ -587,10 +790,10 @@
     return (size_t)2 * N * C * (Hg + 2) * CPR * 16;
 }
 
-NEMAR_API int nemar_instnorm_fwd_planes(const float* x, const float* residual, const void* residual_max_words, float* y, float* stats,
-                                        int N, int C, int H, int W, float eps, int act, float slope, float dropout_p,
-                                        unsigned long long seed, unsigned offset, void* planes, void* scale_words, void* max_words,
-                                        void* wgrad_planes, void* stream) {
+static int instnorm_fwd_planes(const float* x, const float* residual, const void* residual_max_words, float* y, float* stats,
+                               int N, int C, int H, int W, float eps, int act, float slope, float dropout_p,
+                               unsigned long long seed, unsigned offset, void* planes, void* scale_words, void* max_words,
+                               void* wgrad_planes, const float* stat_partials, int stat_tiles, void* stream) {
     NEMAR_CLEAR_HIP_ERROR();
     NEMAR_REQUIRE(x && stats && planes && scale_words, "instnorm_fwd_planes: null pointer");
     NEMAR_REQUIRE(N > 0 && N <= 256 && C > 0 && C % 8 == 0 && C / 8 <= NEMAR_MAX_PARTIALS, "instnorm_fwd_planes: bad N=%d C=%d", N, C);
@@ -612,6 +815,7 @@
     p.dscale = dropout_p > 0.f ? 1.f / (1.f - dropout_p) : 1.f;
     p.dbg = g_norm_planes_dbg;
     p.lazy = (max_words && nemar_max_words_lazy() && C / 8 <= 0xFFFF) ? 1 : 0;
+    p.statp = stat_partials; p.stat_tiles = stat_tiles;
     p.obase = g_dropout_base;
     p.seed_lo = (unsigned)(seed & 0xffffffffu); p.seed_hi = (unsigned)(seed >> 32); p.offset = offset;
     p.xw = (u32x4*)wgrad_planes;
@@ -621,10 +825,40 @@
     NEMAR_REQUIRE(!wgrad_planes || (nemar_conv2d_x_planes_bytes(N, C, H, W, 3) > 0 && ((uintptr_t)wgrad_planes & 15) == 0),
                   "instnorm_fwd_planes: this shape has no weight-gradient planes (N=%d C=%d %dx%d)", N, C, H, W);
     hipStream_t st = (hipStream_t)stream;
+    if (stat_partials) {
+        NEMAR_REQUIRE(W == 32 || W == 64, "instnorm_fwd_planes_stats: W = %d (a wide forward call writes 32- or 64-wide planes)", W);
+        NEMAR_REQUIRE(stat_tiles > 0 && stat_tiles == H * W / 64 && (H * W) % 64 == 0,
+                      "instnorm_fwd_planes_stats: %d tiles per plane, a %dx%d plane has %d", stat_tiles, H, W, H * W / 64);
+        NEMAR_REQUIRE((((uintptr_t)stat_partials) & 15) == 0, "instnorm_fwd_planes_stats: stat_partials must be 16-byte aligned");
+        const int bands = (H * W + NS_PIX - 1) / NS_PIX;
+        NEMAR_REQUIRE((C / 8) * bands <= NEMAR_MAX_PARTIALS, "instnorm_fwd_planes_stats: too many partial maxima");
+        static_assert(NS_XT >= 16 * 72, "band tile of a 64-wide plane");
+        hipLaunchKernelGGL(instnorm_planes_stream_kernel, dim3(N * (C / 8) * bands), dim3(NS_THREADS), 0, st, p);
+        if (max_words && !p.lazy) max_words_finalize((unsigned*)max_words, N, (C / 8) * bands, st);
+        NEMAR_CHECK_LAUNCH("instnorm_fwd_planes_stats");
+        return NEMAR_OK;
+    }
     hipLaunchKernelGGL(instnorm_planes_kernel, dim3(N * (C / 8)), dim3(1024), 0, st, p);
     if (max_words && !p.lazy) max_words_finalize((unsigned*)max_words, N, C / 8, st);
     NEMAR_CHECK_LAUNCH("instnorm_fwd_planes");
     return NEMAR_OK;
+}
+
+NEMAR_API int nemar_instnorm_fwd_planes(const float* x, const float* residual, const void* residual_max_words, float* y, float* stats,
+                                        int N, int C, int H, int W, float eps, int act, float slope, float dropout_p,
+                                        unsigned long long seed, unsigned offset, void* planes, void* scale_words, void* max_words,
+                                        void* wgrad_planes, void* stream) {
+    return instnorm_fwd_planes(x, residual, residual_max_words, y, stats, N, C, H, W, eps, act, slope, dropout_p, seed, offset, planes,
+                               scale_words, max_words, wgrad_planes, nullptr, 0, stream);
+}
+
+NEMAR_API int nemar_instnorm_fwd_planes_stats(const float* x, const float* residual, const void* residual_max_words, float* y, float* stats,
+                                              int N, int C, int H, int W, float eps, int act, float slope, float dropout_p,
+                                              unsigned long long seed, unsigned offset, void* planes, void* scale_words, void* max_words,
+                                              void* wgrad_planes, const float* stat_partials, int stat_tiles, void* stream) {
+    NEMAR_REQUIRE(stat_partials, "instnorm_fwd_planes_stats: null stat_partials (nemar_instnorm_fwd_planes computes the statistics itself)");
+    return instnorm_fwd_planes(x, residual, residual_max_words, y, stats, N, C, H, W, eps, act, slope, dropout_p, seed, offset, planes,
+                               scale_words, max_words, wgrad_planes, stat_partials, stat_tiles, stream);
 }
 
 NEMAR_API int nemar_instnorm_bwd_planes(const float* x, const float* stats, const float* gy, const void* gy_max_words, int N, int C,
diff --git a/nemar_amd/ops.py b/nemar_amd/ops.py
--- a/nemar_amd/ops.py
+++ b/nemar_amd/ops.py
@@ -223,6 +223,44 @@
     return buf
 
 
+_conv_stats_on = [os.environ.get("NEMAR_CONV_STATS", "1") != "0"]
+_stat_tiles = {}
+_stat_arena = {}
+
+
+def conv_stats(on=None):
+    prev = _conv_stats_on[0]
+    if on is not None:
+        _conv_stats_on[0] = bool(on)
+    return prev
+
+
+def _fwd_stat_tiles(N, H, W, K, C, R, S, stride, pad, pad_mode):
+    if not _conv_stats_on[0]:
+        return 0
+    key = (N, H, W, K, C, R, S, stride, pad, pad_mode, L.config_epoch())
+    t = _stat_tiles.get(key)
+    if t is None:
+        t = _stat_tiles[key] = L.conv2d_fwd_stat_tiles(N, H, W, K, C, R, S, stride, pad, pad_mode)
+    return t
+
+
+def _stat_buffer(N, C, tiles, device):
+    need = N * C * tiles * 4
+    akey = (device, _lane[0])
+    buf = _stat_arena.get(akey)
+    if buf is None or buf.numel() < need:
+        _retire(buf)
+        buf = torch.empty(need, dtype=torch.float32, device=device)
+        _stat_arena[akey] = buf
+    return buf
+
+
+def _stats_of(t):
+    have = getattr(t, '_nemar_stat_partials', None)
+    return have if have is not None and have[2] == t._version else None
+
+
 _garena = {}
 _garena_next = {}
 _gplanes_need = {}
@@ -252,10 +290,13 @@
     return slot[0], slot
 
 
-def _extras(arena=None, src_max=None, src2_max=None, planes=None, gy_out=None, src2_planes=None, addend=None, out_max=None, bias_partials=None):
+def _extras(arena=None, src_max=None, src2_max=None, planes=None, gy_out=None, src2_planes=None, addend=None, out_max=None, bias_partials=None,
+            stats_out=None):
     if arena is None and src_max is None and src2_max is None and planes is None and addend is None:
         return None
     e = _lib.ConvExtras()
+    if stats_out is not None:
+        e.stat_partials = stats_out.data_ptr()
     if addend is not None:
         e.addend = addend.data_ptr()
     if bias_partials is not None:
@@ -500,9 +541,14 @@
             if arena is not None:
                 ready = _planes_of(x) if (pad_mode == PAD_REFLECT and R == 3 and S == 3 and stride == 1 and pad == 1) else None
                 xmax = ready[1] if ready is not None else _absmax_word(x)
+            tiles = _fwd_stat_tiles(N, H, W, K, C, R, S, stride, pad, pad_mode) if (arena is not None and act == ACT_NONE and _planes_on[0]) else 0
+            sbuf = torch.empty(N * K * tiles * 4, dtype=torch.float32, device=x.device) if tiles else None
             with _record(plan):
                 L.conv2d_fwd_ex(_p(x), C0, _p(x2), C1, _p(w), _p(b), _p(y), N, H, W, K, R, S, stride, pad, pad_mode, act,
-                                slope, _p(ws), wsb, hit, _stream(), _extras(arena, xmax, None, ready[0] if ready is not None else None))
+                                slope, _p(ws), wsb, hit, _stream(),
+                                _extras(arena, xmax, None, ready[0] if ready is not None else None, stats_out=sbuf))
+            if sbuf is not None:
+                y._nemar_stat_partials = (sbuf, tiles, y._version)
         ctx.xmax = xmax
         xp = _xplanes_of(x) if ready is not None else None
         ctx.xplanes = xp[0] if (xp is not None and xp[1] is ready[1]) else None
@@ -790,8 +836,14 @@
                 seed, off = _dropout_state["seed"], _dropout_state["offset"]
                 ctx.drop = (drop_p, seed, off)
             xbuf = _x_planes_buffer(N, C, H, W, x.device) if any(ctx.needs_input_grad[:2]) else None
-            L.instnorm_fwd_planes(_p(x), _p(residual), _p(_absmax_word(residual)) if residual is not None else None, _p(y), _p(stats),
-                                  N, C, H, W, eps, act, slope, drop_p, seed, off, _p(buf), _p(scale_words), _p(words), _p(xbuf), _stream())
+            part = _stats_of(x) if _conv_stats_on[0] else None
+            if part is not None:
+                L.instnorm_fwd_planes_stats(_p(x), _p(residual), _p(_absmax_word(residual)) if residual is not None else None, _p(y), _p(stats),
+                                            N, C, H, W, eps, act, slope, drop_p, seed, off, _p(buf), _p(scale_words), _p(words), _p(xbuf),
+                                            _p(part[0]), part[1], _stream())
+            else:
+                L.instnorm_fwd_planes(_p(x), _p(residual), _p(_absmax_word(residual)) if residual is not None else None, _p(y), _p(stats),
+                                      N, C, H, W, eps, act, slope, drop_p, seed, off, _p(buf), _p(scale_words), _p(words), _p(xbuf), _stream())
             _tag_max(y, words)
             y._nemar_planes = (buf, scale_words, y._version)
             if xbuf is not None:
@@ -973,11 +1025,20 @@
         arena = _conv_scratch(N, H, W, C, C, 3, 3, 1, 1, dev)
         wsb = Q.conv2d_fwd_workspace(N, H, W, C, C, 3, 3, 1, 1)
 
-        def conv(src_key, planes, words, weight, bias, y):
+        tiles = _fwd_stat_tiles(N, H, W, C, C, 3, 3, 1, 1, PAD_REFLECT) if arena is not None else 0
+        part = _stat_buffer(N, C, tiles, dev) if tiles else None
+
+        def conv(src_key, planes, words, weight, bias, y, stats_out=None):
             ws, hit, plan = _packed(weight, ('fwd', 1, 1, N, H, W), wsb)
             with _span('igemm_fwd_resblock'), _record(plan):
                 L.conv2d_fwd_ex(src_key, C, None, 0, _p(weight), _p(bias), _p(y), N, H, W, C, 3, 3, 1, 1, PAD_REFLECT, ACT_NONE, 0.2,
-                                _p(ws), wsb, hit, st, _extras(arena, words, None, planes))
+                                _p(ws), wsb, hit, st, _extras(arena, words, None, planes, stats_out=stats_out))
+
+        def producer(*a):
+            if part is not None:
+                L.instnorm_fwd_planes_stats(*a, _p(part), tiles, st)
+            else:
+                L.instnorm_fwd_planes(*a, st)
 
         ready = _planes_of(x)
         xp0 = _xplanes_of(x)
@@ -988,7 +1049,7 @@
         else:
             x_words, xp0 = _absmax_word(x), None
         y1 = torch.empty_like(x)
-        conv(_p(x), ready[0] if ready is not None else None, x_words, w1, b1, y1)
+        conv(_p(x), ready[0] if ready is not None else None, x_words, w1, b1, y1, part)
         stats1 = torch.empty((N * C, 2), dtype=torch.float32, device=dev)
         p1 = _chan_planes_buffer(N, C, H, W, dev)
         train = any(ctx.needs_input_grad[:5])
@@ -999,10 +1060,9 @@
             _dropout_state["offset"] = (_dropout_state["offset"] + 1) & 0xFFFFFFFF
             seed, off = _dropout_state["seed"], _dropout_state["offset"]
         with _span('in_fwd_planes_resblock'):
-            L.instnorm_fwd_planes(_p(y1), None, None, None, _p(stats1), N, C, H, W, eps, ACT_RELU, 0.2, drop_p, seed, off, _p(p1), _p(scale1),
-                                  None, _p(xp1), st)
+            producer(_p(y1), None, None, None, _p(stats1), N, C, H, W, eps, ACT_RELU, 0.2, drop_p, seed, off, _p(p1), _p(scale1), None, _p(xp1))
         y2 = torch.empty_like(x)
-        conv(_p(p1), p1, scale1, w2, b2, y2)
+        conv(_p(p1), p1, scale1, w2, b2, y2, part if feeds_block else None)
         del p1
         out = torch.empty_like(x)
         stats2 = torch.empty((N * C, 2), dtype=torch.float32, device=dev)
@@ -1012,8 +1072,8 @@
             xpout = _x_planes_buffer(N, C, H, W, dev) if train else None
             scale_out = torch.empty(N, dtype=torch.int32, device=dev)
             with _span('in_fwd_planes_resblock'), _lazy_max():
-                L.instnorm_fwd_planes(_p(y2), _p(x), _p(_absmax_word(x, lazy_ok=True)), _p(out), _p(stats2), N, C, H, W, eps, ACT_NONE, 0.2, 0.0, 0, 0,
-                                      _p(pout), _p(scale_out), _p(words), _p(xpout), st)
+                producer(_p(y2), _p(x), _p(_absmax_word(x, lazy_ok=True)), _p(out), _p(stats2), N, C, H, W, eps, ACT_NONE, 0.2, 0.0, 0, 0,
+                         _p(pout), _p(scale_out), _p(words), _p(xpout))
             out._nemar_planes = (pout, scale_out, out._version)
             if xpout is not None:
                 out._nemar_xplanes = (xpout, scale_out, out._version)
```

Measured after the change: 298.2. About the same (-1.0%).
